# tkkiran/Robust-Conditional-GAN

Hardware: AMD Instinct MI355X
Metric: images/sec G+D train step (CIFAR-10 RCGAN bs=64) (higher is better)
Workload: dtype bf16

## Files before the change

### include/rcgan_hip.h

```cpp
#ifndef RCGAN_HIP_H
#define RCGAN_HIP_H

#include <stddef.h>
#include <stdint.h>

#ifdef __cplusplus
extern "C" {
#endif

#define RCGAN_OK 0
#define RCGAN_EINVALID_ARG (-1)
#define RCGAN_EUNSUPPORTED_SHAPE (-2)
#define RCGAN_EWORKSPACE_TOO_SMALL (-3)
#define RCGAN_EHIP (-4)
#define RCGAN_ERCCL (-5)

#define RCGAN_F32 0
#define RCGAN_BF16 1
#define RCGAN_F16 2

#define RCGAN_ACT_NONE 0
#define RCGAN_ACT_RELU 1
#define RCGAN_ACT_LRELU 2
#define RCGAN_ACT_TANH 3
// ... 24 lines not shown
int rcgan_prof_begin(rcgan_ctx* ctx, int which);
int rcgan_prof_end(rcgan_ctx* ctx, int* launches, double* total_ms, double* total_flops);
int rcgan_prof_executed_flops(rcgan_ctx* ctx, double* executed_flops);
int rcgan_prof_bn_in_launches(rcgan_ctx* ctx, int* launches);
int rcgan_debug_stamps(rcgan_ctx* ctx, void* stamps);
int rcgan_graph_begin(rcgan_ctx* ctx);
int rcgan_graph_end(rcgan_ctx* ctx, int* graph_id);
int rcgan_reserve_scratch(rcgan_ctx* ctx, size_t bytes);
int rcgan_scratch_bytes(rcgan_ctx* ctx, size_t* split_reduction_bytes, size_t* narrow_bytes);
int rcgan_graph_abort(rcgan_ctx* ctx);
int rcgan_graph_launch(rcgan_ctx* ctx, int graph_id);
int rcgan_graph_destroy(rcgan_ctx* ctx, int graph_id);

#define RCGAN_CONV_IN_UPSAMPLE2X 1
#define RCGAN_CONV_IN_RELU 2
#define RCGAN_CONV_ACCUMULATE 4
#define RCGAN_CONV_FORCE_DIRECT 8
#define RCGAN_CONV_OUT_MEANPOOL2 16

#define RCGAN_CONV_RESID_UPSAMPLE2X 32

typedef struct rcgan_conv_desc {
  int n, h, w, cin;
  int cout, kh, kw, stride;
  int dtype;
  int flags;
} rcgan_conv_desc;

size_t rcgan_conv_prepared_bytes(const rcgan_conv_desc* d);
int rcgan_conv_prepare(rcgan_ctx* ctx, const rcgan_conv_desc* d, const float* w_hwio,
                       const float* sigma , void* prepared);

typedef struct rcgan_prepare_item {
  rcgan_conv_desc desc;
  const float* w;
  const float* sigma;
  void* prepared;
} rcgan_prepare_item;
int rcgan_conv_prepare_batch(rcgan_ctx* ctx, const rcgan_prepare_item* items, int n_items);
typedef struct rcgan_embed_desc {
  int v, e_dim, d;
  const float *table, *w_e, *sigma_e , *b_e ;
  float* E;
} rcgan_embed_desc;
int rcgan_conv_prepare_batch_embed(rcgan_ctx* ctx, const rcgan_prepare_item* items, int n_items, const rcgan_embed_desc* e);
typedef struct rcgan_step_inputs_desc {
  int n, dtype;
  const int32_t* images;
  void* x; void* pooled;
  float noise_lo, noise_hi;
  uint64_t seed; void* rng_state;
  float* fill; size_t fill_count;
  const void* fakes; void* fake_slice; int n_slices;
} rcgan_step_inputs_desc;
int rcgan_conv_prepare_batch_riders(rcgan_ctx* ctx, const rcgan_prepare_item* items, int n_items, const rcgan_embed_desc* e,
                                    const rcgan_step_inputs_desc* si);
typedef struct rcgan_frag_item { int item; int ctn, ss; void* fwd; void* bwd; } rcgan_frag_item;
int rcgan_conv_prepare_batch_frags(rcgan_ctx* ctx, const rcgan_prepare_item* items, int n_items, const rcgan_embed_desc* e,
                                   const rcgan_step_inputs_desc* si, const rcgan_frag_item* frags, int n_frags);

size_t rcgan_conv_workspace_bytes(const rcgan_conv_desc* d);
int rcgan_conv_fused_pool_ok(const rcgan_conv_desc* d);
int rcgan_conv_resid_up_ok(const rcgan_conv_desc* d);
int rcgan_conv2d_fwd(rcgan_ctx* ctx, const rcgan_conv_desc* d, const void* x, const void* prepared,
                     const float* bias , void* y);
int rcgan_conv_bn_in_ok(const rcgan_conv_desc* d);
int rcgan_conv2d_fwd_bn(rcgan_ctx* ctx, const rcgan_conv_desc* d, const void* x, const void* prepared, const float* bias, void* y,
                        int segments, const int32_t* labels, const float* gamma, const float* beta, const float* mean, const float* rstd,
                        int act);
int rcgan_conv2d_fwd_bn_residual(rcgan_ctx* ctx, const rcgan_conv_desc* d, const void* x, const void* prepared, const float* bias,
                                 const void* residual, void* y, int segments, const int32_t* labels, const float* gamma, const float* beta,
                                 const float* mean, const float* rstd, int act);
int rcgan_conv2d_fwd_residual(rcgan_ctx* ctx, const rcgan_conv_desc* d, const void* x, const void* prepared,
                              const float* bias , const void* residual , void* y);
int rcgan_conv2d_bwd_data(rcgan_ctx* ctx, const rcgan_conv_desc* d, const void* dy, const void* prepared,
                          const void* x , void* dx, void* ws, size_t ws_bytes);
int rcgan_conv2d_bwd_data_residual(rcgan_ctx* ctx, const rcgan_conv_desc* d, const void* dy, const void* prepared,
                                   const void* x , const void* residual, void* dx, void* ws, size_t ws_bytes);
int rcgan_conv_wgrad_pool_ok(const rcgan_conv_desc* d);
int rcgan_conv2d_bwd_weight(rcgan_ctx* ctx, const rcgan_conv_desc* d, const void* x, const void* dy,
                            float* dw, float* dbias, int accumulate, void* ws, size_t ws_bytes);
int rcgan_conv2d_bwd_weight_group(rcgan_ctx* ctx, int n, const rcgan_conv_desc* descs, const void* const* xs, const void* const* dys,
                                  float* const* dws, float* const* dbiases, int accumulate, void* ws, size_t ws_bytes);

int rcgan_deconv2d_fwd(rcgan_ctx* ctx, const rcgan_conv_desc* d, const void* x, const float* w,
                       const float* bias, void* y);
int rcgan_deconv2d_bwd_data(rcgan_ctx* ctx, const rcgan_conv_desc* d, const void* dy, const float* w, void* dx);
int rcgan_deconv2d_bwd_data_cols(rcgan_ctx* ctx, const rcgan_conv_desc* d, const void* dy, const float* w, void* dx, int n_cols);
int rcgan_deconv2d_bwd_weight(rcgan_ctx* ctx, const rcgan_conv_desc* d, const void* x, const void* dy,
                              float* dw, float* dbias, int accumulate, void* ws, size_t ws_bytes);
size_t rcgan_deconv2d_bwd_weight_concat_bytes(const rcgan_conv_desc* d, int n_cols);
int rcgan_deconv2d_bwd_weight_concat(rcgan_ctx* ctx, const rcgan_conv_desc* d, const void* x, const void* dy, int n_cols, const float* yb,
                                     float* dw, float* dbias, int accumulate, void* ws, size_t ws_bytes);

int rcgan_linear_fwd(rcgan_ctx* ctx, int m, int k, int n, int dtype, const void* x, const float* w,
                     const float* sigma, const float* bias, void* y);
int rcgan_linear_bwd_data(rcgan_ctx* ctx, int m, int k, int n, int dtype, const void* dy, const float* w,
                          const float* sigma, void* dx, int accumulate);
int rcgan_linear_bwd_weight(rcgan_ctx* ctx, int m, int k, int n, int dtype, const void* x, const void* dy,
                            float* dw, float* dbias, int accumulate, void* ws, size_t ws_bytes);
size_t rcgan_linear_workspace_bytes(int m, int k, int n);

size_t rcgan_bn_workspace_bytes(int rows, int c);
size_t rcgan_bn_workspace_bytes_labels(int rows, int c, int n_labels);
int rcgan_bn_stats(rcgan_ctx* ctx, int rows, int c, int dtype, const void* x, float eps,
                   float* mean, float* rstd, float* moving_mean, float* moving_var, float decay,
                   void* ws, size_t ws_bytes);
int rcgan_bn_apply_fwd(rcgan_ctx* ctx, int n, int rows_per_sample, int c, int n_labels, int dtype, const void* x,
                       const int32_t* labels, const float* gamma, const float* beta,
                       const float* mean, const float* rstd, int act, void* y, void* ws, size_t ws_bytes);
int rcgan_bn_fwd_segments(rcgan_ctx* ctx, int nseg, int n_per_seg, int rows_per_sample, int c, int n_labels, int dtype,
                          const void* x, const int32_t* labels, const float* gamma, const float* beta, float eps, int act,
                          float* mean, float* rstd, void* y, void* ws, size_t ws_bytes);
int rcgan_bn_bwd(rcgan_ctx* ctx, int n, int rows_per_sample, int c, int n_labels, int dtype,
                 const void* x, const void* y, const void* dy, const int32_t* labels,
                 const float* gamma, const float* mean, const float* rstd, int act,
                 void* dx, int accumulate_dx, float* dgamma, float* dbeta, int accumulate, void* ws, size_t ws_bytes);
int rcgan_bn_bwd2(rcgan_ctx* ctx, int n, int rows_per_sample, int c, int n_labels, int dtype, const void* x, const void* y,
                  const void* dy, const int32_t* labels, const float* gamma, const float* beta, const float* mean, const float* rstd,
                  int act, void* dx, int accumulate_dx, float* dgamma, float* dbeta, int accumulate, void* ws, size_t ws_bytes);
int rcgan_bn_infer(rcgan_ctx* ctx, int rows, int c, int dtype, const void* x, const float* gamma,
                   const float* beta, const float* moving_mean, const float* moving_var, float eps,
                   int act, void* y);
int rcgan_bn_infer_bwd(rcgan_ctx* ctx, int rows, int c, int dtype, const void* y, const void* dy, const float* gamma,
                       const float* moving_var, float eps, int act, void* dx, int accumulate);

typedef struct rcgan_sn_item {
  const float* w;
  float* u;
  float* sigma;
  float* save;
  int k, c, update;
} rcgan_sn_item;
size_t rcgan_sn_save_floats(int k, int c);
int rcgan_sn_power_iter(rcgan_ctx* ctx, const rcgan_sn_item* items, int n_items);
typedef struct rcgan_sn_bwd_item {
  const float* w; const float* dwbar; float* dw; float* save ; int k, c, accumulate;
} rcgan_sn_bwd_item;
int rcgan_sn_bwd(rcgan_ctx* ctx, const rcgan_sn_bwd_item* items, int n_items);
typedef struct rcgan_sn_adam {
  float* w; float* g; float* m; float* v; size_t count;
  float* hyper;
  float beta1, beta2, eps, clip, grad_scale;
  int n_ranges; const size_t* ranges;
} rcgan_sn_adam;
int rcgan_sn_bwd_adam(rcgan_ctx* ctx, const rcgan_sn_bwd_item* items, int n_items, const rcgan_sn_adam* opt);

int rcgan_act_fwd(rcgan_ctx* ctx, size_t count, int dtype, int act, const void* x, void* y);
int rcgan_act_bwd(rcgan_ctx* ctx, size_t count, int dtype, int act, const void* x_or_y, const void* dy,
                  void* dx, int accumulate);
int rcgan_add(rcgan_ctx* ctx, size_t count, int dtype, const void* a, const void* b, void* y);
int rcgan_axpby(rcgan_ctx* ctx, size_t count, int dtype, float alpha, const void* a, float beta, void* y);
int rcgan_cast(rcgan_ctx* ctx, size_t count, int src_dtype, const void* src, int dst_dtype, void* dst);
int rcgan_meanpool2_fwd(rcgan_ctx* ctx, int n, int h, int w, int c, int dtype, const void* x, void* y);
int rcgan_meanpool2_bwd(rcgan_ctx* ctx, int n, int h, int w, int c, int dtype, const void* dy, void* dx, int accumulate);
int rcgan_upsample2_fwd(rcgan_ctx* ctx, int n, int h, int w, int c, int dtype, const void* x, void* y);
int rcgan_upsample2_bwd(rcgan_ctx* ctx, int n, int h, int w, int c, int dtype, const void* dy, void* dx, int accumulate);
int rcgan_pad_channels(rcgan_ctx* ctx, size_t rows, int c, int before, int after, int dtype, const void* x, void* y);
int rcgan_concat_channels_fwd(rcgan_ctx* ctx, int n, int hw, int c1, int c2, int dtype, const void* x,
                              const float* yb, void* y);
int rcgan_concat_channels_bwd(rcgan_ctx* ctx, int n, int hw, int c1, int c2, int dtype, const void* dy, void* dx);
int rcgan_tile_rows_fwd(rcgan_ctx* ctx, size_t count, int reps, int dtype, const void* x, void* y);
int rcgan_tile_rows_bwd(rcgan_ctx* ctx, size_t count, int reps, int dtype, const void* dy, void* dx, int accumulate);
int rcgan_transpose_f32(rcgan_ctx* ctx, int rows, int cols, const float* x, float* y, int accumulate);
int rcgan_preprocess_cifar(rcgan_ctx* ctx, int n, const int32_t* images_chw, const float* noise_chw,
                           int dtype, void* y_nhwc);
// ... 34 lines not shown
int rcgan_conv_rf_prepare(rcgan_ctx* ctx, int n, const rcgan_conv_desc* descs, const void* const* prepared, void* const* frags);
int rcgan_fragments_prepare(rcgan_ctx* ctx, const void* const* trunk_prepared, void* trunk_frag, int n, const rcgan_conv_desc* descs,
                            const void* const* prepared, void* const* frags);
int rcgan_conv2d_rf(rcgan_ctx* ctx, const rcgan_conv_desc* d, int backward, const void* x, const void* frag, const float* bias,
                    const void* mask_x, const void* residual, void* y);
typedef struct {
  int n, d, v, e_dim;
  int rows_a, kind_a, kind_b;
  float weight;
  const int32_t* labels_a; const float* wts_a; float* dwts_a;
  const int32_t* labels_b; const float* wts_b; float* dwts_b;
  const void* x; void* dx;
  int x_dtype, hw, act;
  const float* E_pre;
  void* defer_ws;
  size_t defer_ws_bytes;
} rcgan_head_desc;
int rcgan_proj_head_fwd_bwd(rcgan_ctx* ctx, const rcgan_head_desc* hd, const float* feat, const float* w_out, const float* sigma_out,
                            const float* b_out, const float* table, const float* w_e, const float* sigma_e, const float* b_e,
                            float* loss_acc, float* logits, float* dfeat, float* dw_out, float* db_out, float* dtable, float* dw_e,
                            float* db_e, void* ws, size_t ws_bytes);
int rcgan_head_flush(rcgan_ctx* ctx);
int rcgan_bce_onehot_fwd_bwd(rcgan_ctx* ctx, int rows, int cols, const float* x, const int32_t* labels,
                             float weight, float* loss_acc, float* dx);
int rcgan_recover_mse_fwd_bwd(rcgan_ctx* ctx, int r, int ydim, int pix, int dtype, const void* gen, const void* actual,
                              const float* yrec, float* loss, void* dgen, float* dyrec, void* ws, size_t ws_bytes);
int rcgan_softmax_rows_fwd(rcgan_ctx* ctx, int rows, int cols, const float* logits, float* p);
int rcgan_softmax_rows_bwd(rcgan_ctx* ctx, int rows, int cols, const float* p, const float* dp, float* dlogits,
                           int accumulate);

size_t rcgan_softmax_xent_workspace_bytes(int rows);
int rcgan_softmax_xent_fwd_bwd(rcgan_ctx* ctx, int rows, int cols, const float* logits, const int32_t* labels, float weight,
                               float* loss_acc, float* n_correct_acc, float* dlogits, void* ws, size_t ws_bytes);
int rcgan_shortcut_a_fwd(rcgan_ctx* ctx, int n, int h, int w, int c, int dtype, const void* x, void* y);
int rcgan_shortcut_a_bwd(rcgan_ctx* ctx, int n, int h, int w, int c, int dtype, const void* dy, void* dx, int accumulate);
int rcgan_sgd_momentum(rcgan_ctx* ctx, size_t count, size_t decay_count, float* w, const float* g, float* accum, const float* hyper,
                       float momentum, float weight_decay, int nesterov, float grad_scale);
int rcgan_augment_cifar(rcgan_ctx* ctx, int n, int n_images, const uint8_t* images_chw_u8, const int32_t* labels_all,
                        const int32_t* index, const int32_t* shift_flip, int pad, int dtype, void* y_nhwc, int32_t* labels_out);

int rcgan_adam_tf(rcgan_ctx* ctx, size_t count, float* w, const float* g, float* m, float* v,
                  const float* hyper, float beta1, float beta2, float eps, float clip, float grad_scale);
int rcgan_adam_tf_host(rcgan_ctx* ctx, size_t count, float* w, const float* g, float* m, float* v,
                       float lr, float t, float beta1, float beta2, float eps, float clip, float grad_scale);
int rcgan_fill_f32(rcgan_ctx* ctx, size_t count, float* p, float value);
int rcgan_copy_words(rcgan_ctx* ctx, size_t count, const void* src, void* dst);

int rcgan_conv_stats_ok(const rcgan_conv_desc* d);
size_t rcgan_conv_stats_bytes(const rcgan_conv_desc* d);
int rcgan_conv2d_fwd_stats(rcgan_ctx* ctx, const rcgan_conv_desc* d, const void* x, const void* prepared, const float* bias,
                           const void* residual, void* y, float* tile_sums);
int rcgan_bn_stats_from_tiles(rcgan_ctx* ctx, const rcgan_conv_desc* d, int nseg, float eps, const float* tile_sums, float* mean, float* rstd);
int rcgan_bn_apply_segments(rcgan_ctx* ctx, int nseg, int n_per_seg, int rows_per_sample, int c, int n_labels, int dtype, const void* x,
                            const int32_t* labels, const float* gamma, const float* beta, const float* mean, const float* rstd, int act,
                            void* y, void* ws, size_t ws_bytes);

int rcgan_set_grad_scale(rcgan_ctx* ctx, float host_scale, const float* dev_scale);

#define RCGAN_F32_PRECISION_HIGHEST 0
#define RCGAN_F32_PRECISION_HIGH 1
int rcgan_set_f32_matmul_precision(rcgan_ctx* ctx, int precision);
int rcgan_grad_finite_check(rcgan_ctx* ctx, size_t count, const float* g, float* ls_state);
int rcgan_adam_tf_dyn(rcgan_ctx* ctx, size_t count, float* w, const float* g, float* m, float* v, float lr, const float* t_dev,
                      float beta1, float beta2, float eps, float clip, float grad_scale, const float* ls_state);
int rcgan_loss_scale_update(rcgan_ctx* ctx, float* ls_state, float* t_dev0, float* t_dev1, float growth_interval, float min_scale,
                            float max_scale);

#define RCGAN_COMM_ID_BYTES 128
int rcgan_comm_unique_id(void* id_out);
int rcgan_comm_init(rcgan_ctx* ctx, const void* id, int world, int rank);
int rcgan_comm_init_stub(rcgan_ctx* ctx, int world);
int rcgan_comm_destroy(rcgan_ctx* ctx);
int rcgan_comm_world(rcgan_ctx* ctx);
int rcgan_allreduce_sum(rcgan_ctx* ctx, float* buf, size_t count);
int rcgan_allreduce_sum_buckets(rcgan_ctx* ctx, int n, float* const* bufs, const size_t* counts);
int rcgan_allreduce_sum_async(rcgan_ctx* ctx, float* buf, size_t count);
int rcgan_allreduce_join(rcgan_ctx* ctx);
int rcgan_comm_count(rcgan_ctx* ctx, int* ranks);
size_t rcgan_allreduce_bf16_scratch_bytes(int n, const size_t* counts);
int rcgan_allreduce_sum_bf16_buckets(rcgan_ctx* ctx, int n, float* const* bufs, const size_t* counts, void* scratch16, size_t scratch_bytes);
int rcgan_comm_stub_model(rcgan_ctx* ctx, double bus_gbps, double latency_us);
const char* rcgan_comm_load_error(void);
int rcgan_set2_f32(rcgan_ctx* ctx, float* p, float a, float b);

int rcgan_selftest(rcgan_ctx* ctx);
#define RCGAN_QUERY_TR_READ 0
int rcgan_query(rcgan_ctx* ctx, int what);

#ifdef __cplusplus
}
#endif
#endif
```

### robust-conditional-gan_amd/_lib.py

```python
import ctypes as C
import os

_HERE = os.path.dirname(os.path.abspath(__file__))
LIB_PATH = os.environ.get("RCGAN_LIB_PATH") or os.path.join(_HERE, "librcgan_hip.so")
LIB_PATH_F16 = os.environ.get("RCGAN_LIB_PATH_F16") or os.path.join(_HERE, "librcgan_hip_f16.so")

F32, BF16, F16 = 0, 1, 2
ACT_NONE, ACT_RELU, ACT_LRELU, ACT_TANH, ACT_SIGMOID = 0, 1, 2, 3, 4
CONV_IN_UPSAMPLE2X, CONV_IN_RELU, CONV_ACCUMULATE, CONV_FORCE_DIRECT, CONV_OUT_MEANPOOL2, CONV_RESID_UPSAMPLE2X = 1, 2, 4, 8, 16, 32
LOSS_HINGE_REAL, LOSS_HINGE_FAKE, LOSS_NEG_MEAN, LOSS_CE_ONES, LOSS_CE_ZEROS = 0, 1, 2, 3, 4
QUERY_TR_READ = 0
F32_PRECISION_HIGHEST, F32_PRECISION_HIGH = 0, 1
F32_PRECISIONS = {"highest": F32_PRECISION_HIGHEST, "high": F32_PRECISION_HIGH}

RCGAN_EHIP, RCGAN_ERCCL = -4, -5
EINVALID_ARG, EUNSUPPORTED_SHAPE = -1, -2
ERRORS = {-1: "RCGAN_EINVALID_ARG", -2: "RCGAN_EUNSUPPORTED_SHAPE", -3: "RCGAN_EWORKSPACE_TOO_SMALL",
          -4: "RCGAN_EHIP", -5: "RCGAN_ERCCL"}


def source_hash():
    import glob
    import hashlib
    h = hashlib.sha256()
    files = sorted(glob.glob(os.path.join(_HERE, "csrc", "*.hip")) + glob.glob(os.path.join(_HERE, "csrc", "*.h")) +
                   glob.glob(os.path.join(os.path.dirname(_HERE), "include", "*.h")))
    for f in files:
        h.update(os.path.basename(f).encode())
        with open(f, "rb") as fh:
            h.update(fh.read())
    return h.hexdigest()[:16]


class RcganError(RuntimeError):
    def __init__(self, code, msg):
        super().__init__("%s (%d): %s" % (ERRORS.get(code, "RCGAN_E?"), code, msg))
        self.code = code


class ConvDesc(C.Structure):
    _fields_ = [("n", C.c_int), ("h", C.c_int), ("w", C.c_int), ("cin", C.c_int),
                ("cout", C.c_int), ("kh", C.c_int), ("kw", C.c_int), ("stride", C.c_int),
                ("dtype", C.c_int), ("flags", C.c_int)]


class PrepareItem(C.Structure):
    _fields_ = [("desc", ConvDesc), ("w", C.c_void_p), ("sigma", C.c_void_p), ("prepared", C.c_void_p)]


class FragItem(C.Structure):
    _fields_ = [("item", C.c_int), ("ctn", C.c_int), ("ss", C.c_int), ("fwd", C.c_void_p), ("bwd", C.c_void_p)]


class HeadDesc(C.Structure):
    _fields_ = [("n", C.c_int), ("d", C.c_int), ("v", C.c_int), ("e_dim", C.c_int),
                ("rows_a", C.c_int), ("kind_a", C.c_int), ("kind_b", C.c_int), ("weight", C.c_float),
                ("labels_a", C.c_void_p), ("wts_a", C.c_void_p), ("dwts_a", C.c_void_p),
                ("labels_b", C.c_void_p), ("wts_b", C.c_void_p), ("dwts_b", C.c_void_p),
                ("x", C.c_void_p), ("dx", C.c_void_p), ("x_dtype", C.c_int), ("hw", C.c_int), ("act", C.c_int),
                ("E_pre", C.c_void_p), ("defer_ws", C.c_void_p), ("defer_ws_bytes", C.c_size_t)]


class EmbedDesc(C.Structure):
    _fields_ = [("v", C.c_int), ("e_dim", C.c_int), ("d", C.c_int),
                ("table", C.c_void_p), ("w_e", C.c_void_p), ("sigma_e", C.c_void_p), ("b_e", C.c_void_p), ("E", C.c_void_p)]


class StepInputsDesc(C.Structure):
    _fields_ = [("n", C.c_int), ("dtype", C.c_int), ("images", C.c_void_p), ("x", C.c_void_p), ("pooled", C.c_void_p),
                ("noise_lo", C.c_float), ("noise_hi", C.c_float), ("seed", C.c_uint64), ("rng_state", C.c_void_p),
                ("fill", C.c_void_p), ("fill_count", C.c_size_t),
                ("fakes", C.c_void_p), ("fake_slice", C.c_void_p), ("n_slices", C.c_int)]


class SnItem(C.Structure):
    _fields_ = [("w", C.c_void_p), ("u", C.c_void_p), ("sigma", C.c_void_p), ("save", C.c_void_p),
                ("k", C.c_int), ("c", C.c_int), ("update", C.c_int)]


class SnBwdItem(C.Structure):
    _fields_ = [("w", C.c_void_p), ("dwbar", C.c_void_p), ("dw", C.c_void_p), ("save", C.c_void_p),
                ("k", C.c_int), ("c", C.c_int), ("accumulate", C.c_int)]


LABELS_NARROW = 16
MAX_CLASSES = 1024
SN_MAX_RANGES = 48


class SnAdam(C.Structure):
    _fields_ = [("w", C.c_void_p), ("g", C.c_void_p), ("m", C.c_void_p), ("v", C.c_void_p), ("count", C.c_size_t),
                ("hyper", C.c_void_p), ("beta1", C.c_float), ("beta2", C.c_float), ("eps", C.c_float), ("clip", C.c_float),
                ("grad_scale", C.c_float), ("n_ranges", C.c_int), ("ranges", C.POINTER(C.c_size_t))]


P, I, F, SZ = C.c_void_p, C.c_int, C.c_float, C.c_size_t
DP = C.POINTER(ConvDesc)

SIGNATURES = {
    "rcgan_create": (I, [C.POINTER(P), I, P]),
    "rcgan_destroy": (I, [P]),
    "rcgan_last_error": (C.c_char_p, [P]),
    "rcgan_version": (C.c_char_p, []),
    "rcgan_half_dtype": (I, []),
    "rcgan_crc32c": (C.c_uint, [C.c_uint, P, SZ]),
    "rcgan_set_stream": (I, [P, P]),
    "rcgan_side_begin": (I, [P]),
    "rcgan_side_end": (I, [P]),
    "rcgan_side_join": (I, [P]),
    "rcgan_stream_sync": (I, [P]),
    "rcgan_event_record": (I, [P, I]),
    "rcgan_event_elapsed_ms": (I, [P, I, I, C.POINTER(F)]),
    "rcgan_debug_stamps": (I, [P, P]),
    "rcgan_prof_begin": (I, [P, I]),
    "rcgan_prof_end": (I, [P, C.POINTER(I), C.POINTER(C.c_double), C.POINTER(C.c_double)]),
    "rcgan_prof_executed_flops": (I, [P, C.POINTER(C.c_double)]),
    "rcgan_prof_bn_in_launches": (I, [P, C.POINTER(I)]),
    "rcgan_graph_begin": (I, [P]),
    "rcgan_reserve_scratch": (I, [P, C.c_size_t]),
    "rcgan_scratch_bytes": (I, [P, C.POINTER(C.c_size_t), C.POINTER(C.c_size_t)]),
    "rcgan_graph_end": (I, [P, C.POINTER(I)]),
    "rcgan_graph_abort": (I, [P]),
    "rcgan_graph_launch": (I, [P, I]),
    "rcgan_graph_destroy": (I, [P, I]),
    "rcgan_conv_prepared_bytes": (SZ, [DP]),
    "rcgan_conv_prepare": (I, [P, DP, P, P, P]),
    "rcgan_conv_prepare_batch": (I, [P, C.POINTER(PrepareItem), I]),
    "rcgan_conv_prepare_batch_embed": (I, [P, C.POINTER(PrepareItem), I, C.POINTER(EmbedDesc)]),
    "rcgan_conv_prepare_batch_riders": (I, [P, C.POINTER(PrepareItem), I, C.POINTER(EmbedDesc), C.POINTER(StepInputsDesc)]),
    "rcgan_conv_prepare_batch_frags": (I, [P, C.POINTER(PrepareItem), I, C.POINTER(EmbedDesc), C.POINTER(StepInputsDesc), C.POINTER(FragItem), I]),
    "rcgan_conv_workspace_bytes": (SZ, [DP]),
    "rcgan_conv2d_fwd": (I, [P, DP, P, P, P, P]),
    "rcgan_conv_bn_in_ok": (I, [DP]),
    "rcgan_conv2d_fwd_bn": (I, [P, DP, P, P, P, P, I, P, P, P, P, P, I]),
    "rcgan_conv2d_fwd_bn_residual": (I, [P, DP, P, P, P, P, P, I, P, P, P, P, P, I]),
    "rcgan_conv_fused_pool_ok": (I, [DP]),
    "rcgan_conv_resid_up_ok": (I, [DP]),
    "rcgan_conv_wgrad_pool_ok": (I, [DP]),
    "rcgan_conv2d_fwd_residual": (I, [P, DP, P, P, P, P, P]),
    "rcgan_conv2d_bwd_data": (I, [P, DP, P, P, P, P, P, SZ]),
    "rcgan_conv2d_bwd_data_residual": (I, [P, DP, P, P, P, P, P, P, SZ]),
    "rcgan_conv2d_bwd_weight": (I, [P, DP, P, P, P, P, I, P, SZ]),
    "rcgan_conv2d_bwd_weight_group": (I, [P, I, P, P, P, P, P, I, P, SZ]),
    "rcgan_deconv2d_fwd": (I, [P, DP, P, P, P, P]),
    "rcgan_deconv2d_bwd_data": (I, [P, DP, P, P, P]),
    "rcgan_deconv2d_bwd_data_cols": (I, [P, DP, P, P, P, I]),
    "rcgan_deconv2d_bwd_weight": (I, [P, DP, P, P, P, P, I, P, SZ]),
    "rcgan_deconv2d_bwd_weight_concat_bytes": (SZ, [DP, I]),
    "rcgan_deconv2d_bwd_weight_concat": (I, [P, DP, P, P, I, P, P, P, I, P, SZ]),
    "rcgan_linear_fwd": (I, [P, I, I, I, I, P, P, P, P, P]),
    "rcgan_linear_bwd_data": (I, [P, I, I, I, I, P, P, P, P, I]),
    "rcgan_linear_bwd_weight": (I, [P, I, I, I, I, P, P, P, P, I, P, SZ]),
    "rcgan_linear_workspace_bytes": (SZ, [I, I, I]),
    "rcgan_bn_workspace_bytes": (SZ, [I, I]),
    "rcgan_bn_workspace_bytes_labels": (SZ, [I, I, I]),
    "rcgan_bn_stats": (I, [P, I, I, I, P, F, P, P, P, P, F, P, SZ]),
    "rcgan_bn_apply_fwd": (I, [P, I, I, I, I, I, P, P, P, P, P, P, I, P, P, SZ]),
    "rcgan_bn_fwd_segments": (I, [P, I, I, I, I, I, I, P, P, P, P, F, I, P, P, P, P, SZ]),
    "rcgan_bn_bwd": (I, [P, I, I, I, I, I, P, P, P, P, P, P, P, I, P, I, P, P, I, P, SZ]),
    "rcgan_bn_bwd2": (I, [P, I, I, I, I, I, P, P, P, P, P, P, P, P, I, P, I, P, P, I, P, SZ]),
    "rcgan_bn_infer": (I, [P, I, I, I, P, P, P, P, P, F, I, P]),
    "rcgan_bn_infer_bwd": (I, [P, I, I, I, P, P, P, P, F, I, P, I]),
    "rcgan_sn_save_floats": (SZ, [I, I]),
    "rcgan_sn_power_iter": (I, [P, C.POINTER(SnItem), I]),
    "rcgan_sn_bwd": (I, [P, C.POINTER(SnBwdItem), I]),
    "rcgan_sn_bwd_adam": (I, [P, C.POINTER(SnBwdItem), I, C.POINTER(SnAdam)]),
    "rcgan_act_fwd": (I, [P, SZ, I, I, P, P]),
    "rcgan_act_bwd": (I, [P, SZ, I, I, P, P, P, I]),
    "rcgan_add": (I, [P, SZ, I, P, P, P]),
    "rcgan_axpby": (I, [P, SZ, I, F, P, F, P]),
    "rcgan_cast": (I, [P, SZ, I, P, I, P]),
    "rcgan_meanpool2_fwd": (I, [P, I, I, I, I, I, P, P]),
    "rcgan_meanpool2_bwd": (I, [P, I, I, I, I, I, P, P, I]),
    "rcgan_upsample2_fwd": (I, [P, I, I, I, I, I, P, P]),
    "rcgan_upsample2_bwd": (I, [P, I, I, I, I, I, P, P, I]),
    "rcgan_pad_channels": (I, [P, SZ, I, I, I, I, P, P]),
    "rcgan_concat_channels_fwd": (I, [P, I, I, I, I, I, P, P, P]),
    "rcgan_concat_channels_bwd": (I, [P, I, I, I, I, I, P, P]),
    "rcgan_tile_rows_fwd": (I, [P, SZ, I, I, P, P]),
    "rcgan_tile_rows_bwd": (I, [P, SZ, I, I, P, P, I]),
    "rcgan_transpose_f32": (I, [P, I, I, P, P, I]),
    "rcgan_preprocess_cifar": (I, [P, I, P, P, I, P]),
    "rcgan_rng_fill": (I, [P, SZ, I, I, F, F, C.c_uint64, P, P]),
    "rcgan_act_meanhw_fwd": (I, [P, I, I, I, I, I, P, P]),
    "rcgan_act_meanhw_bwd": (I, [P, I, I, I, I, I, P, P, P]),
    "rcgan_gather_rows": (I, [P, I, I, P, P, P]),
    "rcgan_scatter_add_rows": (I, [P, I, I, I, P, P, P, I]),
    "rcgan_proj_logit_fwd": (I, [P, I, I, P, P, P, P]),
    "rcgan_proj_logit_bwd": (I, [P, I, I, P, P, P, P, P, P, I]),
    "rcgan_proj_logit_all_fwd": (I, [P, I, I, I, P, P, P, P]),
    "rcgan_proj_logit_all_bwd": (I, [P, I, I, I, P, P, P, P, P, P, I]),
    "rcgan_loss_fwd_bwd": (I, [P, I, I, I, P, P, F, P, P, P]),
    "rcgan_bce_onehot_fwd_bwd": (I, [P, I, I, P, P, F, P, P]),
    "rcgan_dtrunk": (I, [P, I, I, P, P, P, P, P]),
    "rcgan_dtrunk_pooled": (I, [P, I, I, P, P, P, P, P, P, P, P]),
    "rcgan_dtrunk_prepare": (I, [P, P, P]),
    "rcgan_conv_rf_ok": (I, [C.POINTER(ConvDesc)]),
    "rcgan_conv_rf_fragment_bytes": (SZ, [C.POINTER(ConvDesc)]),
    "rcgan_conv_rf_prepare": (I, [P, I, C.POINTER(ConvDesc), P, P]),
    "rcgan_fragments_prepare": (I, [P, P, P, I, C.POINTER(ConvDesc), P, P]),
    "rcgan_conv2d_rf": (I, [P, C.POINTER(ConvDesc), I, P, P, P, P, P, P]),
    "rcgan_dtrunk_fragment_bytes": (SZ, []),
    "rcgan_head_flush": (I, [P]),
    "rcgan_proj_head_fwd_bwd": (I, [P, C.POINTER(HeadDesc)] + [P] * 16 + [P, SZ]),
    "rcgan_recover_mse_fwd_bwd": (I, [P, I, I, I, I, P, P, P, P, P, P, P, SZ]),
    "rcgan_softmax_rows_fwd": (I, [P, I, I, P, P]),
    "rcgan_softmax_rows_bwd": (I, [P, I, I, P, P, P, I]),
    "rcgan_softmax_xent_workspace_bytes": (SZ, [I]),
    "rcgan_softmax_xent_fwd_bwd": (I, [P, I, I, P, P, F, P, P, P, P, SZ]),
    "rcgan_shortcut_a_fwd": (I, [P, I, I, I, I, I, P, P]),
    "rcgan_shortcut_a_bwd": (I, [P, I, I, I, I, I, P, P, I]),
    "rcgan_sgd_momentum": (I, [P, SZ, SZ, P, P, P, P, F, F, I, F]),
    "rcgan_augment_cifar": (I, [P, I, I, P, P, P, P, I, I, P, P]),
    "rcgan_adam_tf": (I, [P, SZ, P, P, P, P, P, F, F, F, F, F]),
    "rcgan_adam_tf_host": (I, [P, SZ, P, P, P, P, F, F, F, F, F, F, F]),
    "rcgan_fill_f32": (I, [P, SZ, P, F]),
    "rcgan_copy_words": (I, [P, SZ, P, P]),
    "rcgan_conv_stats_ok": (I, [DP]),
    "rcgan_conv_stats_bytes": (SZ, [DP]),
    "rcgan_conv2d_fwd_stats": (I, [P, DP, P, P, P, P, P, P]),
    "rcgan_bn_stats_from_tiles": (I, [P, DP, I, F, P, P, P]),
    "rcgan_bn_apply_segments": (I, [P, I, I, I, I, I, I, P, P, P, P, P, P, I, P, P, SZ]),
    "rcgan_comm_unique_id": (I, [P]),
    "rcgan_comm_init": (I, [P, P, I, I]),
    "rcgan_comm_init_stub": (I, [P, I]),
    "rcgan_comm_destroy": (I, [P]),
    "rcgan_comm_world": (I, [P]),
    "rcgan_allreduce_sum": (I, [P, P, SZ]),
    "rcgan_allreduce_sum_buckets": (I, [P, I, P, P]),
    "rcgan_allreduce_sum_async": (I, [P, P, SZ]),
    "rcgan_allreduce_join": (I, [P]),
    "rcgan_comm_count": (I, [P, P]),
    "rcgan_allreduce_bf16_scratch_bytes": (SZ, [I, P]),
    "rcgan_allreduce_sum_bf16_buckets": (I, [P, I, P, P, P, SZ]),
    "rcgan_comm_stub_model": (I, [P, C.c_double, C.c_double]),
    "rcgan_comm_load_error": (C.c_char_p, []),
    "rcgan_set2_f32": (I, [P, P, F, F]),
    "rcgan_set_grad_scale": (I, [P, F, P]),
    "rcgan_set_f32_matmul_precision": (I, [P, I]),
    "rcgan_grad_finite_check": (I, [P, SZ, P, P]),
    "rcgan_adam_tf_dyn": (I, [P, SZ, P, P, P, P, F, P, F, F, F, F, F, P]),
    "rcgan_loss_scale_update": (I, [P, P, P, P, F, F, F]),
    "rcgan_selftest": (I, [P]),
    "rcgan_query": (I, [P, I]),
}

_libs = {}


def load(half="bf16"):
    if half in _libs:
        return _libs[half]
    path = LIB_PATH_F16 if half == "f16" else LIB_PATH
    if not os.path.exists(path):
        raise RuntimeError(
            "%s is missing (%s): build it with robust-conditional-gan_amd/csrc/build.sh "
            "or __graft_entry__.build(); there is no CPU fallback" % (os.path.basename(path), path))
    import torch
    lib = C.CDLL(path)
    for name, (res, args) in SIGNATURES.items():
        fn = getattr(lib, name)
        fn.restype = res
        fn.argtypes = args
    want = F16 if half == "f16" else BF16
    if lib.rcgan_half_dtype() != want:
        raise RuntimeError("%s was built for 16-bit dtype %d, expected %d" % (path, lib.rcgan_half_dtype(), want))
    _libs[half] = lib
    return lib
```

### robust-conditional-gan_amd/cifar.py

```python
import ctypes as C
import os

import warnings

import numpy as np
import torch

from . import _lib as L
from . import ops as O
from .ops_cifar import NO_OPS, Conv2D, Linear, cond_batchnorm, embed_y, spectral_normed_weight
from .runtime import DT, Context, ParamGroup, check_f32_matmul_precision
from .variables import Graph, scoped, variable_scope

Z_DIM = 128
DIM_G = 128
DIM_D = 128
VOCAB_SIZE = 10
EMBEDDING_DIM = 300
IMG_SIZE = 32
IMG_DIM = 3
OUTPUT_DIM = 3072
N_CRITIC = 5
GEN_BS_MULTIPLE = 2
ALGORITHMS = ("rcgan", "rcgan-u", "biased", "unbiased")
# ... 286 lines not shown
    O.proj_head(g.ctx, features, w_out, b_out, table, w_e, b_e, parts, weight, loss_acc, logits=logits, E_pre=getattr(g, "head_E", None))


def perm_classifier(x, perm_type='linear'):
    ctx = _ctx()
    with variable_scope("Discriminator"):
        x = O.cast(ctx, O.reshape(ctx, x, (-1, OUTPUT_DIM)), L.F32)
        if perm_type == 'linear':
            return Linear(x, OUTPUT_DIM, _n_classes(), 'D.d_perm_classifier_h1', spectral_normed=True, biases=True)
        elif perm_type == '2layer':
            h = Linear(x, OUTPUT_DIM, 128, 'D.d_perm_classifier_h1', spectral_normed=True, biases=True)
            return Linear(h, 128, _n_classes(), 'D.d_perm_classifier_h2', spectral_normed=True, biases=True)
        raise ValueError('Unknown perm_type {}'.format(perm_type))


class CifarRCGAN:

    def __init__(self, algorithm="rcgan", alpha=0.6, batch_size=64, lr=2e-4, dtype="bf16", seed=0,
                 perm_classifier=False, perm_multiplier=1.0, perm_type="linear",
                 confuse_init=False, confuse_init_diag=0.2, confuse_multiplier=1.0, confuse_lr_decay=False,
                 device=0, use_graphs=True, device_rng=True, arena_bytes=None, world_size=1, rank=0,
                 variables=None, loss_scale=None, dynamic_loss_scale=None, loss_scale_growth_interval=2000, comm=None,
                 grad_bucket_dtype=None, stub_model=None, f32_matmul_precision="highest", n_classes=VOCAB_SIZE):
        if algorithm not in ALGORITHMS:
            raise ValueError("Unknown algorithm %s" % algorithm)
        self.K = check_n_classes(n_classes)
        self.f32_matmul_precision = check_f32_matmul_precision(f32_matmul_precision, dtype)
        self.alg, self.alpha, self.B, self.lr = algorithm, alpha, int(batch_size), lr
        self.perm, self.perm_mult, self.perm_type = perm_classifier, perm_multiplier, perm_type
        self.confuse_multiplier, self.confuse_lr_decay = confuse_multiplier, confuse_lr_decay
        self.world, self.rank = world_size, rank
        self.use_graphs, self.device_rng = use_graphs, device_rng
        self.fused_head = os.environ.get("RCGAN_FUSED_HEAD", "1") == "1" and 2 * int(batch_size) <= O.HEAD_MAX_N
        self.ride_inputs = os.environ.get("RCGAN_RIDE_INPUTS", "1") == "1"
        if arena_bytes is None:
            arena_bytes = int(2.5e6 * 4 * self.B * (4 if dtype == "f32" else 2)) + (1 << 30)
        self.ctx = Context(device, dtype, arena_bytes=arena_bytes)
        ctx = self.ctx
        ctx.set_f32_matmul_precision(self.f32_matmul_precision)
        self.loss_scale = float(loss_scale) if loss_scale is not None else (1024.0 if ctx.act_dtype == L.F16 else 1.0)
        self.dynamic_ls = (ctx.act_dtype == L.F16) if dynamic_loss_scale is None else bool(dynamic_loss_scale)
        self.ls_growth_interval = float(loss_scale_growth_interval)
        if self.dynamic_ls:
            self.ls_state = torch.tensor([self.loss_scale, 0.0, 0.0, 0.0], dtype=torch.float32, device=ctx.device)
            ctx.check(ctx.lib.rcgan_set_grad_scale(ctx.h, 1.0, C.c_void_p(self.ls_state.data_ptr())))
        else:
            self.ls_state = None
            ctx.check(ctx.lib.rcgan_set_grad_scale(ctx.h, self.loss_scale, None))
        if variables is None:
            variables = create_variables(seed, algorithm, perm_classifier, perm_type, confuse_init, confuse_init_diag, self.K)
        gs, ds, cs, U = variables
        self.PG, self.PD = ParamGroup(ctx, gs), ParamGroup(ctx, ds, sn_scratch=True)
        self.PC = ParamGroup(ctx, cs) if cs else None
        self.groups = [self.PG, self.PD] + ([self.PC] if self.PC else [])
        self.state = {}
        for k, v in U.items():
            t = ctx.persistent((v.size,), L.F32)
            ctx.view(t).copy_(torch.from_numpy(np.ascontiguousarray(v.reshape(-1))))
            self.state[k] = t
        self.graph = Graph(ctx, self.groups, self.state)
        self.graph.n_classes = self.K
        self.comm_kind = None
        self.dp_active = self.world > 1 or comm == "rccl-self"
        if self.dp_active:
            from . import dp
            self.comm_kind = comm or "rccl"
            if self.comm_kind not in ("rccl", "stub", "rccl-self") or (self.comm_kind == "rccl-self" and self.world != 1):
                raise ValueError("Unknown comm %s for world_size %d" % (comm, self.world))
            dp.init_comm(ctx, self.world, self.rank, stub=(self.comm_kind == "stub"))
            if stub_model is not None:
                ctx.check(ctx.lib.rcgan_comm_stub_model(ctx.h, float(stub_model[0]), float(stub_model[1])))
        self.grad_bucket_dtype = grad_bucket_dtype or os.environ.get("RCGAN_DP_BUCKET_DTYPE", "f32")
        if self.grad_bucket_dtype not in ("f32", "bf16"):
            raise ValueError("Unknown gradient bucket dtype %s" % self.grad_bucket_dtype)
        self._bucket16 = None
        self.dp_overlap = self.dp_active and self.grad_bucket_dtype == "f32" and os.environ.get("RCGAN_DP_OVERLAP", "0") == "1"
        self._early_lo = {id(self.PD): self.PD.offsets["Discriminator/D.Block.3.Conv1/Filters"],
                          id(self.PG): self.PG.offsets["Generator/G.Block.2.Shortcut/Filters"]}
        self.dp_adam_in_graph = self.dp_active and not self.dynamic_ls and os.environ.get("RCGAN_DP_GRAPH_ADAM", "1") == "1"
        self.graph_adam = self.dp_adam_in_graph or (not self.dp_active and not self.dynamic_ls and
                                                    os.environ.get("RCGAN_GRAPH_ADAM", "0") == "1")
        self.fused_tail = (not self.dp_active and not self.dynamic_ls and not self.graph_adam
                           and os.environ.get("RCGAN_SN_ADAM", "1") == "1")
        self._tail_fused = {}
        B = self.B
        f32, i32, act = L.F32, "i32", ctx.act_dtype
        P = ctx.persistent
        self.feed_layout = {
            "d": [("images", (B, OUTPUT_DIM), i32), ("labels", (B,), i32), ("labels_random", (B,), i32), ("labels_biased", (B,), i32),
                  ("inv_weights", (B, self.K), f32), ("labels_all", (2 * B,), i32)],
            "g": [("labels_random_G", (2 * B,), i32), ("labels_biased_G", (2 * B,), i32)],
            "gf": [("labels_random_all", (N_CRITIC * B,), i32)]}
        self.feed, self.inp = {}, {}
        self._feed_ring = {}
        for key, fields in self.feed_layout.items():
            words = sum(int(np.prod(shp)) for _, shp, _ in fields)
            slab = torch.zeros(words, dtype=torch.int32, device=ctx.device)
            self.feed[key] = slab
            off = 0
            for name, shp, dt in fields:
                self.inp[name] = DT(slab.data_ptr() + 4 * off, shp, dt, slab, name)
                off += int(np.prod(shp))
        words_d = self.feed["d"].numel()
        self.feed["d5"] = torch.zeros(N_CRITIC * words_d, dtype=torch.int32, device=ctx.device)
        self._d_slot_views = []
        for k in range(N_CRITIC):
            off, views = k * words_d, {}
            for name, shp, dt in self.feed_layout["d"]:
                views[name] = DT(self.feed["d5"].data_ptr() + 4 * off, shp, dt, self.feed["d5"], name)
                off += int(np.prod(shp))
            self._d_slot_views.append(views)
        self.critic_graph = os.environ.get("RCGAN_CRITIC_GRAPH", "1") == "1"
        self.inp.update(noise=P((B, OUTPUT_DIM), f32), z=P((B, Z_DIM), act), z_G=P((2 * B, Z_DIM), act),
                        z_all=P((N_CRITIC * B, Z_DIM), act),
                        arange=P((self.K,), i32), C_const=P((self.K, self.K), f32))
        ctx.view(self.inp["arange"]).copy_(torch.arange(self.K, dtype=torch.int32))
        ctx.view(self.inp["C_const"]).copy_(torch.from_numpy(C_ALPHA(alpha, self.K).astype(np.float32)))
        self.fakes_all = P((N_CRITIC * B, OUTPUT_DIM), act)
        self.x_all = P((2 * B, OUTPUT_DIM), act)
        self._fakes_left = 0
        self.loss_d = self.PD.scalar(0)
        self.loss_g = self.PG.scalar(0)
        self.rng_state = torch.zeros(2, dtype=torch.int64, device=ctx.device)
        self.overlap_gf = os.environ.get("RCGAN_OVERLAP_GF", "0") == "1"
        self.ctx2 = None
        if self.overlap_gf:
            self.ctx2 = Context(device, dtype, arena_bytes=int(2.5e6 * self.B * (4 if dtype == "f32" else 2)) + (256 << 20), ws_bytes=256 << 20)
            ctx.also_close = [self.ctx2]
            ctx.check(self.ctx2.lib.rcgan_set_grad_scale(self.ctx2.h, 1.0, None))
            self.ctx2.set_f32_matmul_precision(self.f32_matmul_precision)
            self.graph2 = Graph(self.ctx2, [ParamGroup.alias(self.ctx2, self.PG)], {})
            self.graph2.persist = self.graph.persist
            self.rng_state_gf = torch.zeros(2, dtype=torch.int64, device=ctx.device)
            self._gf_done = [torch.cuda.Event() for _ in range(N_CRITIC)]
            self._gf_pending = [False] * N_CRITIC
            torch.cuda.set_device(ctx.device)
        self.slice_ctr = torch.zeros(4, dtype=torch.int32, device=ctx.device)
        self._slice_mirror = 0
        self.seed = seed
        self._graphs = {}
        self.head_logits = None
        self.iteration = 0
        self._pg_prepared_version = -1
        torch.cuda.synchronize()

    def set_inputs(self, **arrays):
        ctx = self.ctx
        with torch.cuda.stream(ctx.stream):
            for k, a in arrays.items():
                dst = ctx.view(self.inp[k])
                src = torch.from_numpy(np.ascontiguousarray(np.asarray(a)))
                dst.copy_(src.reshape(dst.shape).to(dst.dtype).pin_memory(), non_blocking=True)

    def pack_feed(self, key, **arrays):
        parts = []
        for name, shp, dt in self.feed_layout[key]:
            a = np.ascontiguousarray(np.asarray(arrays[name]).reshape(shp))
            parts.append(a.astype(np.float32).view(np.int32).reshape(-1) if dt == L.F32 else a.astype(np.int32).reshape(-1))
        return np.concatenate(parts)

    def feed_host(self, key, **arrays):
        steps = arrays.pop("_steps", None)
        ring = self._feed_ring.setdefault(key, {"slots": [], "events": [], "next": 0})
        words = self.feed[key].numel()
        if not ring["slots"]:
            ring["slots"] = [torch.empty(words, dtype=torch.int32).pin_memory() for _ in range(8)]
# ... 145 lines not shown
        else:
            fake = Generator(B, inp["labels_random"], inp["z"], out=fake_dst)
        w = 1.0
        if self.fused_head:
            feat = Discriminator(x_all, None, update_collection=None, _head=False)
            lab_r, lab_f = inp["labels_all"].rows(0, B), inp["labels_all"].rows(B, 2 * B)
            if self.alg == "rcgan-u":
                y_conf = O.gather_rows(ctx, self.confusion_matrix(), inp["labels_random"], B)
                parts = [(B, L.LOSS_HINGE_REAL, inp["labels"], None), (B, L.LOSS_HINGE_FAKE, None, y_conf)]
            elif self.alg == "unbiased":
                parts = [(B, L.LOSS_HINGE_REAL, None, inp["inv_weights"]), (B, L.LOSS_HINGE_FAKE, inp["labels_random"], None)]
            else:
                parts = [(B, L.LOSS_HINGE_REAL, lab_r, None), (B, L.LOSS_HINGE_FAKE, lab_f, None)]
            Discriminator_head(feat, parts, w, self.loss_d, update_collection=None, logits=self.head_logits)
        elif self.alg == "rcgan-u":
            feat_a, wgan_a = Discriminator(x_all, None, update_collection=None)
            feat, wgan = O.rows(ctx, feat_a, 0, B), O.rows(ctx, wgan_a, 0, B)
            feat_f, wgan_f = O.rows(ctx, feat_a, B, 2 * B), O.rows(ctx, wgan_a, B, 2 * B)
            emb = Discriminator_projection(inp["labels"], update_collection=None)
            disc_real = O.proj_logit(ctx, feat, wgan, emb)
            E = Discriminator_projection(inp["arange"], update_collection=None)
            disc_fake = O.proj_logit_all(ctx, feat_f, wgan_f, E)
            y_conf = O.gather_rows(ctx, self.confusion_matrix(), inp["labels_random"], B)
            O.loss_term(ctx, L.LOSS_HINGE_FAKE, disc_fake, w, self.loss_d, wts=y_conf)
            O.loss_term(ctx, L.LOSS_HINGE_REAL, disc_real, w, self.loss_d)
        else:
            feat, wgan = Discriminator(x_all, None, update_collection=None)
            if self.alg in ("biased", "rcgan"):
                emb = Discriminator_projection(inp["labels_all"], update_collection=None)
                disc_all = O.proj_logit(ctx, feat, wgan, emb)
                O.loss_term(ctx, L.LOSS_HINGE_REAL, O.rows(ctx, disc_all, 0, B), w, self.loss_d)
                O.loss_term(ctx, L.LOSS_HINGE_FAKE, O.rows(ctx, disc_all, B, 2 * B), w, self.loss_d)
            else:
                E = Discriminator_projection(inp["arange"], update_collection=None)
                feat_r, wgan_r = O.rows(ctx, feat, 0, B), O.rows(ctx, wgan, 0, B)
                feat_f, wgan_f = O.rows(ctx, feat, B, 2 * B), O.rows(ctx, wgan, B, 2 * B)
                disc_real_all = O.proj_logit_all(ctx, feat_r, wgan_r, E)
                O.loss_term(ctx, L.LOSS_HINGE_REAL, disc_real_all, w, self.loss_d, wts=inp["inv_weights"])
                emb_f = Discriminator_projection(inp["labels_random"], update_collection=None)
                disc_fake = O.proj_logit(ctx, feat_f, wgan_f, emb_f)
                O.loss_term(ctx, L.LOSS_HINGE_FAKE, disc_fake, w, self.loss_d)
        if self.perm:
            logits = perm_classifier(real, self.perm_type)
            O.bce_onehot_term(ctx, logits, inp["labels"], 1.0, self.loss_d)
        ctx.backward()
        fused = bool(ctx.sn_adam and ctx.sn_adam.get("done"))
        ctx.sn_adam = None
        self._dp_finish([self.PD])
        return fused

    def _d_step_body(self, fakes_ready):
        self._tail_fused[fakes_ready] = self._d_body(fakes_ready)

    def _g_body(self):
        ctx, g, B, inp = self.ctx, self.graph, self.B, self.inp
        n = GEN_BS_MULTIPLE * B
        self._refresh_generator_filters()
        ctx.new_step()
        g.begin_step({0, 2} if self.PC is not None else {0})
        ctx.sn_adam = None
        g.early_g = self._dp_early(self.PG) if (self.dp_overlap and ctx.recording) else None
        self.PG.zero_grad()
        if self.PC is not None:
            self.PC.zero_grad()
        if self.device_rng:
            self._rng(inp["z_G"], 1, 0.0, 1.0)
        g.prefetch_sn(self._sn_entries(False, True))
        self._prepare_all((self.PG, self.PD), head_update=NO_OPS)
        fake = Generator(n, inp["labels_random_G"], inp["z_G"])
        lab = inp["labels_random_G"] if self.alg in ("biased", "unbiased") else inp["labels_biased_G"]
        if self.fused_head:
            feat = Discriminator(fake, lab, update_collection=NO_OPS, _head=False)
            if self.alg == "rcgan-u":
                y_conf = O.gather_rows(ctx, self.confusion_matrix(), inp["labels_random_G"], n)
                parts = [(n, L.LOSS_NEG_MEAN, None, y_conf)]
            else:
                parts = [(n, L.LOSS_NEG_MEAN, lab, None)]
            Discriminator_head(feat, parts, 1.0, self.loss_g, update_collection=NO_OPS, logits=self.head_logits)
        else:
            self._g_head_unfused(fake, lab, n)
        if self.perm:
            logits = perm_classifier(fake, self.perm_type)
            O.bce_onehot_term(ctx, logits, inp["labels_random_G"], self.perm_mult, self.loss_g)
        ctx.backward()
        self._dp_finish([self.PG] + ([self.PC] if self.PC is not None else []))

    def _g_head_unfused(self, fake, lab, n):
        ctx, inp = self.ctx, self.inp
        feat, wgan = Discriminator(fake, lab, update_collection=NO_OPS)
        if self.alg == "rcgan-u":
            E = Discriminator_projection(inp["arange"], update_collection=None)
            disc_fake = O.proj_logit_all(ctx, feat, wgan, E)
            y_conf = O.gather_rows(ctx, self.confusion_matrix(), inp["labels_random_G"], n)
            O.loss_term(ctx, L.LOSS_NEG_MEAN, disc_fake, 1.0, self.loss_g, wts=y_conf)
        else:
            emb = Discriminator_projection(lab, update_collection=None)
            disc_fake = O.proj_logit(ctx, feat, wgan, emb)
            O.loss_term(ctx, L.LOSS_NEG_MEAN, disc_fake, 1.0, self.loss_g)

    def _run(self, key, body, ctx=None):
        ctx = ctx or self.ctx
        if not self.use_graphs:
            body()
            return
        if key not in self._graphs:
            body()
            ctx.sync()
            ctx.graph_begin()
            try:
                body()
                gid = ctx.graph_end()
            except L.RcganError as e:
                ctx.graph_abort()
                if not (self.dp_active and e.code == L.RCGAN_ERCCL):
                    raise
                warnings.warn("step %r: the all-reduce could not be captured (%s); running it uncaptured" % (key, e))
                gid = None
            except BaseException:
                ctx.graph_abort()
                raise
            self._graphs[key] = gid
            return
        if self._graphs[key] is None:
            body()
            return
        ctx.graph_launch(self._graphs[key])

    def _dp_early(self, grp):
        ctx, lo = self.ctx, self._early_lo[id(grp)]
        state = {"sent": False}
        grp._dp_early_state = state

        def fire():
            ctx.flush_wgrads()
            for bw in ctx.sn_partial:
                bw(lambda name: name in grp.offsets and grp.offsets[name] >= lo)
            ctx.check(ctx.lib.rcgan_allreduce_sum_async(ctx.h, C.c_void_p(grp.grad.data_ptr() + 4 * lo), grp.count - lo))
            state["sent"] = True
        return fire

    def _dp_finish(self, groups):
        ctx = self.ctx
        if not ctx.recording:
            return
        if not self.dp_active:
            if self.graph_adam:
                for grp in groups:
                    grp.adam_captured(0.0, 0.9, grad_scale=1.0 / (self.world * self.loss_scale))
            return
        ptrs, counts = [], []
        for grp in groups:
            st = getattr(grp, "_dp_early_state", None)
            hi = self._early_lo[id(grp)] if (st is not None and st["sent"]) else grp.count
            grp._dp_early_state = None
            if hi > 0:
                ptrs.append(grp.grad.data_ptr())
                counts.append(hi)
        n = len(ptrs)
        if self.grad_bucket_dtype == "bf16":
            cnt = (C.c_size_t * n)(*counts)
            need = ctx.lib.rcgan_allreduce_bf16_scratch_bytes(n, cnt)
            if self._bucket16 is None:
                allc = [g.count for g in self.groups]
                self._bucket16 = torch.empty(ctx.lib.rcgan_allreduce_bf16_scratch_bytes(len(allc), (C.c_size_t * len(allc))(*allc)),
                                             dtype=torch.uint8, device=ctx.device)
            assert need <= self._bucket16.numel()
            ctx.check(ctx.lib.rcgan_allreduce_sum_bf16_buckets(ctx.h, n, (C.c_void_p * n)(*ptrs), cnt, C.c_void_p(self._bucket16.data_ptr()),
                                                               self._bucket16.numel()))
        else:
            ctx.check(ctx.lib.rcgan_allreduce_sum_buckets(ctx.h, n, (C.c_void_p * n)(*ptrs), (C.c_size_t * n)(*counts)))
        if self.dp_overlap:
            ctx.check(ctx.lib.rcgan_allreduce_join(ctx.h))
        if self.dp_adam_in_graph:
            for grp in groups:
                grp.adam_captured(0.0, 0.9, grad_scale=1.0 / (self.world * self.loss_scale))

    def _optimise_or_publish(self, steps):
        if self.graph_adam:
            for grp, _ in steps:
                grp.version += 1
            return
        self._optimise(steps)

    def _pre_step(self, steps):
        if self.fused_tail:
            for grp, lr in steps:
                if grp is self.PD and (grp.hyper is None or getattr(grp, "_dev_hyper", None) != (float(lr), grp.t)):
                    grp.set_hyper_device(lr, grp.t)
                    grp._dev_hyper = (float(lr), grp.t)
        if self.graph_adam:
            for grp, lr in steps:
                grp.t += 1
                grp.set_hyper_device(lr, grp.t)

    def _gf_body(self):
        ctx, g, B, inp = self.ctx, self.graph, self.B, self.inp
        self._refresh_generator_filters()
        ctx.new_step()
        g.begin_step(set())
        rec, ctx.recording = ctx.recording, False
        try:
            if self.device_rng:
                self._rng(inp["z_all"], 1, 0.0, 1.0)
            self._prepare_all((self.PG,))
            Generator(N_CRITIC * B, inp["labels_random_all"], inp["z_all"], out=self.fakes_all, segments=N_CRITIC)
        finally:
            ctx.recording = rec

    def _gf_chunk_body(self, k):
        ctx2, g2, B, inp = self.ctx2, self.graph2, self.B, self.inp
        ctx2.new_step()
        g2.begin_step(set())
        rec, ctx2.recording = ctx2.recording, False
        try:
            z = inp["z_all"].rows(k * B, (k + 1) * B)
            if self.device_rng:
                ctx2.check(ctx2.lib.rcgan_rng_fill(ctx2.h, z.size, z.dtype, 1, 0.0, 1.0, self.seed * 1000003 + self.rank + 500009,
                                                   C.c_void_p(self.rng_state_gf.data_ptr()), C.c_void_p(z.ptr)))
            Generator(B, inp["labels_random_all"].rows(k * B, (k + 1) * B), z, out=self.fakes_all.rows(k * B, (k + 1) * B))
        finally:
            ctx2.recording = rec

    def _join_gf(self):
        if self.overlap_gf:
            for k in range(N_CRITIC):
                if self._gf_pending[k]:
                    self.ctx.stream.wait_event(self._gf_done[k])
                    self._gf_pending[k] = False

    def _prepare_critic_fakes_overlapped(self):
        s1, s2 = self.ctx.stream, self.ctx2.stream
        self._refresh_generator_filters()
        ev = torch.cuda.Event()
        ev.record(s1)
        s2.wait_event(ev)
        for k in range(N_CRITIC):
            self._run("gf%d" % k, lambda k=k: self._gf_chunk_body(k), ctx=self.ctx2)
            self._gf_done[k].record(s2)
            self._gf_pending[k] = True

    def prepare_critic_fakes(self):
        if self.overlap_gf:
            self._prepare_critic_fakes_overlapped()
        else:
            self._run("gf", self._gf_body)
        self._fakes_left = N_CRITIC
        if self._slice_mirror != 0:
            with torch.cuda.stream(self.ctx.stream):
                self.slice_ctr.zero_()
            self._slice_mirror = 0

    def d_step(self, iteration=None):
        it = self.iteration if iteration is None else iteration
        self._refresh_generator_filters()
        steps = [(self.PD, self.lr * lr_decay(it))]
        self._pre_step(steps)
        if self._fakes_left > 0:
            k = N_CRITIC - self._fakes_left
            self._fakes_left -= 1
            ctx = self.ctx
            if self.overlap_gf and self._gf_pending[k]:
                ctx.stream.wait_event(self._gf_done[k])
                self._gf_pending[k] = False
            if self._rides_inputs():
                assert self._slice_mirror == k, (self._slice_mirror, k)
                self._slice_mirror = (k + 1) % N_CRITIC
            else:
                with torch.cuda.stream(ctx.stream):
                    ctx.view(self.x_all.rows(self.B, 2 * self.B)).copy_(ctx.view(self.fakes_all.rows(k * self.B, (k + 1) * self.B)), non_blocking=True)
            key, fakes_ready = "d_fakes", True
        else:
            key, fakes_ready = "d", False
        self._run(key, lambda: self._d_step_body(fakes_ready))
        if self._tail_fused.get(fakes_ready, False):
            lr = steps[0][1]
            self.PD.t += 1
            self.PD._dev_hyper = (float(lr), self.PD.t)
            self.PD.version += 1
            return
        self._optimise_or_publish(steps)

    def _critic_graph_ok(self):
        return (self.critic_graph and self.fused_tail and self._fakes_left == N_CRITIC and self._rides_inputs() and self._slice_mirror == 0)

    def critic_steps(self, batches, iteration=None):
        it = self.iteration if iteration is None else iteration
        packed = isinstance(batches, torch.Tensor)
        assert (batches.shape[0] if packed else len(batches)) == N_CRITIC
        if not self._critic_graph_ok():
            for k in range(N_CRITIC):
                if packed:
                    self.set_feed("d", batches[k])
                else:
                    self.feed_host("d", **batches[k])
                self.d_step(iteration=it)
            return
        ctx = self.ctx
        if packed:
            src = batches.reshape(-1)
            assert src.is_cuda and src.dtype == torch.int32 and src.is_contiguous() and src.numel() == self.feed["d5"].numel()
            ctx.check(ctx.lib.rcgan_copy_words(ctx.h, src.numel(), C.c_void_p(src.data_ptr()), C.c_void_p(self.feed["d5"].data_ptr())))
        else:
            self.feed_host("d5", _steps=batches)
        self._refresh_generator_filters()
        lr = self.lr * lr_decay(it)
        self._pre_step([(self.PD, lr)])
        self._join_gf()

        def body():
            fused = True
            for k in range(N_CRITIC):
                saved = {n: self.inp[n] for n in self._d_slot_views[k]}
                self.inp.update(self._d_slot_views[k])
                try:
                    fused = self._d_body(True) and fused
                finally:
                    self.inp.update(saved)
            self._tail_fused["d5"] = fused
        self._run("d5", body)
        assert self._tail_fused.get("d5", False), "critic_steps: a step's last launch did not apply the update"
        self._fakes_left = 0
        self.PD.t += N_CRITIC
        self.PD._dev_hyper = (float(lr), self.PD.t)
        self.PD.version += 1

    def g_step(self, iteration=None):
        it = self.iteration if iteration is None else iteration
        self._fakes_left = 0
        self._join_gf()
        self._refresh_generator_filters()
        steps = [(self.PG, self.lr * lr_decay(it))]
        if self.PC is not None:
            steps.append((self.PC, self.lr * self.confuse_multiplier * (lr_decay(it) if self.confuse_lr_decay else 1.0)))
        self._pre_step(steps)
        self._run("g", self._g_body)
        self._optimise_or_publish(steps)
        self._refresh_generator_filters()

    def _optimise(self, steps):
        ctx = self.ctx
        if not self.dynamic_ls:
            for grp, lr in steps:
                grp.t += 1
                grp.set_hyper(lr, grp.t)
                grp.adam(0.0, 0.9, grad_scale=1.0 / (self.world * self.loss_scale))
            return
        for grp, lr in steps:
            grp.t += 1
            grp.finite_check(self.ls_state)
        for grp, lr in steps:
            grp.set_hyper(lr, grp.t)
            grp.adam_dyn(self.ls_state, 0.0, 0.9, grad_scale=1.0 / self.world)
        tds = [C.c_void_p(g.t_dev.data_ptr()) for g, _ in steps] + [None]
        ctx.check(ctx.lib.rcgan_loss_scale_update(ctx.h, C.c_void_p(self.ls_state.data_ptr()), tds[0], tds[1], self.ls_growth_interval,
                                                  1.0, float(1 << 24)))

    def loss_scale_state(self):
        if self.ls_state is None:
            return dict(scale=self.loss_scale, good_steps=None, skipped_steps=0)
        self.ctx.sync()
        s = self.ls_state.cpu().numpy()
        return dict(scale=float(s[0]), good_steps=int(s[1]), skipped_steps=int(s[3]))

    def losses(self):
        ctx = self.ctx
        return float(ctx.download(self.loss_d)[0]), float(ctx.download(self.loss_g)[0])

    def enqueue_losses(self):
        if not hasattr(self, "_loss_ring"):
            self._loss_ring = torch.zeros(1024, 2, dtype=torch.float32).pin_memory()
            self._loss_tickets = 0
        i = self._loss_tickets % 1024
        self._loss_tickets += 1
        ctx = self.ctx
        with torch.cuda.stream(ctx.stream):
            self._loss_ring[i, 0:1].copy_(ctx.view(self.loss_d), non_blocking=True)
            self._loss_ring[i, 1:2].copy_(ctx.view(self.loss_g), non_blocking=True)
        return self._loss_tickets - 1

    def fetch_losses(self, tickets):
        if not tickets:
            return []
        assert self._loss_tickets - min(tickets) <= 1024, "loss ring overrun: fetch at least every 1024 tickets"
        self.ctx.sync()
        return [(float(self._loss_ring[t % 1024, 0]), float(self._loss_ring[t % 1024, 1])) for t in tickets]

    def eval_d_cost(self):
        ctx = self.ctx
        left, self._fakes_left = self._fakes_left, 0
        rec, ctx.recording = ctx.recording, False
        try:
            self._d_body(False)
        finally:
            ctx.recording = rec
            self._fakes_left = left
        return float(ctx.download(self.loss_d)[0])

    def get_params(self):
        out = {}
        for grp in self.groups:
            for n in grp.names:
                out[n] = grp.get(n)
        return out

    def get_grads(self, group):
        scale = self.loss_scale_state()["scale"] * (self.world if self.dp_active else 1)
        return {n: group.get(n, "grad") / np.float32(scale) for n in group.names}

    def get_state(self):
        return {k: self.ctx.download(v).reshape(1, -1) for k, v in self.state.items()}

    def state_dict(self):
        out = {}
        for gname, grp in zip(("Generator", "Discriminator", "confusion"), self.groups):
            for n in grp.names:
                out[n] = grp.get(n)
                out[n + "/Adam"] = grp.get(n, "m")
                out[n + "/Adam_1"] = grp.get(n, "v")
            out["_opt/%s/step" % gname] = np.array([grp.steps_applied()], np.int64)
# ... 72 lines not shown
```

### robust-conditional-gan_amd/csrc/api.hip

```cpp
#include "conv_mfma.h"
#include "small_gemm.h"
#include "step_inputs.h"
#include "conv_image.h"


size_t direct_wgrad_ws_bytes(const rcgan_conv_desc* d);
template <typename T> int direct_fwd(rcgan_ctx*, const rcgan_conv_desc*, const T*, const float*, const float*, const float*, T*, int n_cols = 0);
template <typename T> int direct_dgrad(rcgan_ctx*, const rcgan_conv_desc*, const T*, const float*, const float*, const float*, const T*, T*, int);
template <typename T> int direct_wgrad(rcgan_ctx*, const rcgan_conv_desc*, const T*, const T*, float*, float*, int, void*, size_t);
template <typename T> int direct_wgrad_cols(rcgan_ctx*, const rcgan_conv_desc*, const T*, const T*, int, const float*, float*, int, void*, size_t);
size_t direct_wgrad_cols_ws_bytes(const rcgan_conv_desc* d, int c1);
template <typename T> int colsum_launch(rcgan_ctx*, const T*, long, int, float*, int, float*);
template <typename T> int linear_fwd(rcgan_ctx*, long, long, long, const T*, const float*, const float*, const float*, T*);
template <typename T> int linear_dgrad(rcgan_ctx*, long, long, long, const T*, const float*, const float*, T*, int);
template <typename T> int linear_wgrad(rcgan_ctx*, long, long, long, const T*, const T*, float*, float*, int, void*, size_t);
size_t linear_wgrad_ws_bytes(long m, long k, long n);
template <typename T> int sumpool2_masked_launch(rcgan_ctx*, int, int, int, int, const T*, const T*, T*, int);
int small_fwd_kind(const rcgan_conv_desc* d);
int small_dgrad_kind(const rcgan_conv_desc* d);
int small_wgrad_kind(const rcgan_conv_desc* d);
size_t small_wgrad_ws_bytes(const rcgan_conv_desc* d);
template <typename T> int small_fwd(rcgan_ctx*, const rcgan_conv_desc*, int, const T*, const float*, const float*, T*);
template <typename T> int small_dgrad(rcgan_ctx*, const rcgan_conv_desc*, int, const T*, const float*, T*, int);
template <typename T> int small_wgrad(rcgan_ctx*, const rcgan_conv_desc*, int, const T*, const T*, float*, float*, int, void*, size_t);

__global__ void slab_reduce2_kernel(const float* slab, long stride, float* out, long count, float* bias_out, int nbias, int nz,
                                    int accumulate) {
  long i = (long)blockIdx.x * blockDim.x + threadIdx.x;
  if (i >= count + nbias) return;
  float s = 0.f;
#pragma unroll 4
  for (int z = 0; z < nz; ++z) s += slab[(long)z * stride + i];
  float* o = i < count ? out + i : bias_out + (i - count);
  if (accumulate) s += *o;
  *o = s;
}

#define REDUCE_GROUP_MAX 16
struct SlabReduceGroup {
  struct Item {
    const float* slab; long stride; float* out; long count; float* bias_out; int nbias, nz, accumulate;
    long bias_off;
    int orient, Cb, Cs;
    int sub;
    long cc;
    int bias_parts;
    int vec4;
  } it[REDUCE_GROUP_MAX];
};
__device__ __forceinline__ float4 f4add(float4 a, float4 b) { return make_float4(a.x + b.x, a.y + b.y, a.z + b.z, a.w + b.w); }
__global__ void slab_reduce2_group_kernel(SlabReduceGroup g) {
  const SlabReduceGroup::Item& r = g.it[blockIdx.y];
  long i = (long)blockIdx.x * blockDim.x + threadIdx.x;
  if (r.vec4) {
    const long nv = r.count >> 2;
    if (i < nv) {
      const long e = i << 2;
      float4 s = make_float4(0.f, 0.f, 0.f, 0.f);
      if (r.sub) {
        const int tap = (int)(e / r.cc), kh = tap / 3, kw = tap - kh * 3;
        const long rem = e - (long)tap * r.cc;
        long c4[4];
#pragma unroll
        for (int q = 0; q < 4; ++q) {
          const int pa = q >> 1, pb = q & 1;
          const int sa = ((r.sub == 1) == (pa == 0)) ? (kh >= 1) : (kh >= 2);
          const int sb = ((r.sub == 1) == (pb == 0)) ? (kw >= 1) : (kw >= 2);
          c4[q] = (long)(q * 4 + sa * 2 + sb) * r.cc + rem;
        }
        int z = 0;
        for (; z + 2 <= r.nz; z += 2) {
          float4 v[2][4];
#pragma unroll
          for (int u = 0; u < 2; ++u)
#pragma unroll
            for (int q = 0; q < 4; ++q) v[u][q] = *(const float4*)(r.slab + (long)(z + u) * r.stride + c4[q]);
#pragma unroll
          for (int u = 0; u < 2; ++u) s = f4add(s, f4add(f4add(v[u][0], v[u][1]), f4add(v[u][2], v[u][3])));
        }
        for (; z < r.nz; ++z) {
          const float* sl = r.slab + (long)z * r.stride;
          s = f4add(s, f4add(f4add(*(const float4*)(sl + c4[0]), *(const float4*)(sl + c4[1])), f4add(*(const float4*)(sl + c4[2]), *(const float4*)(sl + c4[3]))));
        }
        if (r.sub == 2) { s.x *= 0.25f; s.y *= 0.25f; s.z *= 0.25f; s.w *= 0.25f; }
      } else {
        int z = 0;
        for (; z + 8 <= r.nz; z += 8) {
          float4 v[8];
#pragma unroll
          for (int u = 0; u < 8; ++u) v[u] = *(const float4*)(r.slab + (long)(z + u) * r.stride + e);
#pragma unroll
          for (int u = 0; u < 8; ++u) s = f4add(s, v[u]);
        }
#pragma unroll 4
        for (; z < r.nz; ++z) s = f4add(s, *(const float4*)(r.slab + (long)z * r.stride + e));
      }
      float4* o = (float4*)(r.out + e);
      if (r.accumulate) s = f4add(s, *o);
      *o = s;
      return;
    }
    i = r.count + (i - nv);
  }
  if (i >= r.count + r.nbias) return;
  const long si = i < r.count ? i : r.bias_off + (i - r.count);
  float s = 0.f;
  if (r.sub && i < r.count) {
    const int tap = (int)(i / r.cc), kh = tap / 3, kw = tap - kh * 3;
    const long rem = i - (long)tap * r.cc;
    long c4[4];
#pragma unroll
    for (int q = 0; q < 4; ++q) {
      const int pa = q >> 1, pb = q & 1;
      const int sa = ((r.sub == 1) == (pa == 0)) ? (kh >= 1) : (kh >= 2);
      const int sb = ((r.sub == 1) == (pb == 0)) ? (kw >= 1) : (kw >= 2);
      c4[q] = (long)(q * 4 + sa * 2 + sb) * r.cc + rem;
    }
    int z = 0;
    for (; z + 4 <= r.nz; z += 4) {
      float v[4][4];
#pragma unroll
      for (int u = 0; u < 4; ++u)
#pragma unroll
        for (int q = 0; q < 4; ++q) v[u][q] = r.slab[(long)(z + u) * r.stride + c4[q]];
#pragma unroll
      for (int u = 0; u < 4; ++u) s += (v[u][0] + v[u][1]) + (v[u][2] + v[u][3]);
    }
    for (; z < r.nz; ++z) {
      const float* sl = r.slab + (long)z * r.stride;
      s += (sl[c4[0]] + sl[c4[1]]) + (sl[c4[2]] + sl[c4[3]]);
    }
    if (r.sub == 2) s *= 0.25f;
  } else {
    int z = 0;
    for (; z + 16 <= r.nz; z += 16) {
      float v[16];
#pragma unroll
      for (int u = 0; u < 16; ++u) v[u] = r.slab[(long)(z + u) * r.stride + si];
#pragma unroll
      for (int u = 0; u < 16; ++u) s += v[u];
    }
#pragma unroll 4
    for (; z < r.nz; ++z) s += r.slab[(long)z * r.stride + si];
    if (i >= r.count && r.bias_parts == 2) {
#pragma unroll 4
      for (z = 0; z < r.nz; ++z) s += r.slab[(long)z * r.stride + si + r.nbias];
    }
  }
  float* o;
  if (i >= r.count) o = r.bias_out + (i - r.count);
  else if (r.orient == 0) o = r.out + i;
  else {
    const int k = (int)(i / r.Cb), n = (int)(i - (long)k * r.Cb);
    const int t = k / r.Cs, c = k - t * r.Cs;
    o = r.out + ((long)t * r.Cb + n) * r.Cs + c;
  }
  if (r.accumulate) s += *o;
  *o = s;
}

struct AdamDyn { const float* ls; const float* tdev; };

__global__ void adam_tf_kernel(size_t count, float* w, const float* g, float* m, float* v, const float* hyper, float lr_v, float t_v,
                               float beta1, float beta2, float eps, float clip, float grad_scale, AdamDyn dyn) {
  if (dyn.ls) {
    if (dyn.ls[2] != 0.f) return;
    grad_scale /= dyn.ls[0];
    t_v = dyn.tdev[0] + 1.f;
  }
  const float lr = hyper ? hyper[0] : lr_v, t = hyper ? hyper[1] : t_v;
  const float alpha = lr * sqrtf(1.f - powf(beta2, t)) / (1.f - powf(beta1, t));
  const float omb1 = 1.f - beta1, omb2 = 1.f - beta2;
  for (size_t i = (size_t)blockIdx.x * blockDim.x + threadIdx.x; i < count; i += (size_t)gridDim.x * blockDim.x) {
    float gi = g[i] * grad_scale;
    float mi = m[i] + (gi - m[i]) * omb1;
    float vi = v[i] + (gi * gi - v[i]) * omb2;
    float wi = w[i] - (mi * alpha) / (sqrtf(vi) + eps);
    if (clip > 0.f) wi = fminf(fmaxf(wi, -clip), clip);
    m[i] = mi; v[i] = vi; w[i] = wi;
  }
}

__global__ void adam_tf_vec4_kernel(size_t count4, float4* w, const float4* g, float4* m, float4* v, const float* hyper, float lr_v, float t_v,
                                    float beta1, float beta2, float eps, float clip, float grad_scale, AdamDyn dyn) {
  if (dyn.ls) {
    if (dyn.ls[2] != 0.f) return;
    grad_scale /= dyn.ls[0];
    t_v = dyn.tdev[0] + 1.f;
  }
  const float lr = hyper ? hyper[0] : lr_v, t = hyper ? hyper[1] : t_v;
  const float alpha = lr * sqrtf(1.f - powf(beta2, t)) / (1.f - powf(beta1, t));
  const float omb1 = 1.f - beta1, omb2 = 1.f - beta2;
  for (size_t i = (size_t)blockIdx.x * blockDim.x + threadIdx.x; i < count4; i += (size_t)gridDim.x * blockDim.x) {
    const float4 g4 = g[i], m4 = m[i], v4 = v[i], w4 = w[i];
    const float gs[4] = {g4.x, g4.y, g4.z, g4.w}, ms[4] = {m4.x, m4.y, m4.z, m4.w}, vs[4] = {v4.x, v4.y, v4.z, v4.w}, ws[4] = {w4.x, w4.y, w4.z, w4.w};
    float mo[4], vo[4], wo[4];
#pragma unroll
    for (int q = 0; q < 4; ++q) {
      const float gi = gs[q] * grad_scale;
      mo[q] = ms[q] + (gi - ms[q]) * omb1;
      vo[q] = vs[q] + (gi * gi - vs[q]) * omb2;
      wo[q] = ws[q] - (mo[q] * alpha) / (sqrtf(vo[q]) + eps);
      if (clip > 0.f) wo[q] = fminf(fmaxf(wo[q], -clip), clip);
    }
    m[i] = make_float4(mo[0], mo[1], mo[2], mo[3]);
    v[i] = make_float4(vo[0], vo[1], vo[2], vo[3]);
    w[i] = make_float4(wo[0], wo[1], wo[2], wo[3]);
  }
}

__global__ void set2_kernel(float* p, float a, float b) { p[0] = a; p[1] = b; }

__global__ void grad_finite_check_kernel(size_t count, const float* g, float* ls) {
  bool bad = false;
  const size_t n4 = count / 4, stride = (size_t)gridDim.x * blockDim.x, tid = (size_t)blockIdx.x * blockDim.x + threadIdx.x;
  for (size_t i = tid; i < n4; i += stride) {
    const float4 q = ((const float4*)g)[i];
    const float z = (q.x - q.x) + (q.y - q.y) + (q.z - q.z) + (q.w - q.w);
    bad |= !(z == 0.f);
  }
  for (size_t i = n4 * 4 + tid; i < count; i += stride) bad |= !((g[i] - g[i]) == 0.f);
  if (bad) ls[2] = 1.f;
}

__global__ void loss_scale_update_kernel(float* ls, float* t0, float* t1, float interval, float min_scale, float max_scale) {
  if (ls[2] != 0.f) {
    ls[0] = fmaxf(ls[0] * 0.5f, min_scale);
    ls[1] = 0.f; ls[2] = 0.f; ls[3] += 1.f;
  } else {
    if (t0) t0[0] += 1.f;
    if (t1) t1[0] += 1.f;
    ls[1] += 1.f;
    if (ls[1] >= interval) { if (ls[0] < max_scale) ls[0] = fminf(ls[0] * 2.f, max_scale); ls[1] = 0.f; }
  }
}

static void adam_launch(rcgan_ctx* ctx, size_t count, float* w, const float* g, float* m, float* v, const float* hyper, float lr, float t,
                        float beta1, float beta2, float eps, float clip, float grad_scale, AdamDyn dyn = {nullptr, nullptr}) {
  const bool vec = count % 4 == 0 && (((size_t)w | (size_t)g | (size_t)m | (size_t)v) & 15) == 0;
  if (vec) {
    size_t blocks = (count / 4 + 255) / 256;
    if (blocks > 8192) blocks = 8192;
    hipLaunchKernelGGL(adam_tf_vec4_kernel, dim3((int)blocks), dim3(256), 0, ctx->stream, count / 4, (float4*)w, (const float4*)g, (float4*)m,
                       (float4*)v, hyper, lr, t, beta1, beta2, eps, clip, grad_scale, dyn);
  } else {
    size_t blocks = (count + 255) / 256;
    if (blocks > 4096) blocks = 4096;
    hipLaunchKernelGGL(adam_tf_kernel, dim3((int)blocks), dim3(256), 0, ctx->stream, count, w, g, m, v, hyper, lr, t, beta1, beta2, eps, clip,
                       grad_scale, dyn);
  }
}

static int g_use_tr = -1;

static int ensure_selftest(rcgan_ctx* ctx) {
  if (g_use_tr >= 0) return RCGAN_OK;
  hipStreamCaptureStatus st = hipStreamCaptureStatusNone;
  (void)hipStreamIsCapturing(ctx->stream, &st);
  if (st != hipStreamCaptureStatusNone) RC_FAIL(ctx, RCGAN_EINVALID_ARG, "first MFMA wgrad call must happen outside graph capture");
  int res[2] = {0, 0};
  int rc = mfma_selftest(ctx, res);
  if (rc) return rc;
  if (res[0] != 0) RC_FAIL(ctx, RCGAN_EHIP, "MFMA 16x16x32 bf16 fragment layout probe failed (%d mismatches)", res[0]);
  g_use_tr = (res[1] == 0) ? 1 : 0;
  const char* e = getenv("RCGAN_NO_TR");
  if (e && e[0] == '1') g_use_tr = 0;
  return RCGAN_OK;
}

extern "C" {

const char* rcgan_version(void) { return RCGAN_HALF_FP16 ? "rcgan_hip 0.1 (gfx950, fp16 build)" : "rcgan_hip 0.1 (gfx950, bf16 build)"; }

int rcgan_create(rcgan_ctx** out, int device, void* stream) {
  if (!out) return RCGAN_EINVALID_ARG;
  int ndev = 0;
  if (hipGetDeviceCount(&ndev) != hipSuccess || ndev <= 0 || device < 0 || device >= ndev) return RCGAN_EHIP;
  if (hipSetDevice(device) != hipSuccess) return RCGAN_EHIP;
  rcgan_ctx* c = new rcgan_ctx();
  c->device = device;
  c->stream = (hipStream_t)stream;
  c->capturing = false;
  c->devtmp = nullptr;
  c->devtmp_bytes = 0;
  c->prof_which = 0;
  c->prof_flops = 0.0; c->prof_flops_exec = 0.0;
  c->main_stream = c->stream; c->side_stream = nullptr; c->fork_ev = nullptr; c->join_ev = nullptr; c->on_side = false;
  if (hipStreamCreateWithFlags(&c->side_stream, hipStreamNonBlocking) != hipSuccess ||
      hipEventCreateWithFlags(&c->fork_ev, hipEventDisableTiming) != hipSuccess ||
      hipEventCreateWithFlags(&c->join_ev, hipEventDisableTiming) != hipSuccess) {
    delete c;
    return RCGAN_EHIP;
  }
  {
// ... 631 lines not shown
  a.M = (long)d->n * a.H * a.W;
  a.lw = ilog2_exact(a.W); a.lh = ilog2_exact(a.H);
  if (a.lw < 0 || a.lh < 0) { a.lw = -1; a.lh = -1; }
  a.slab_stride = (long)a.cells * d->cin * d->cout + d->cout;
  a.want_bias = want_bias ? 1 : 0;
  a.m_chunk = 0;
  *nz = a.sub ? mfma_wgrad_sub_splits(d, a.M) : mfma_wgrad_splits(d, a.M);
  return RCGAN_OK;
}

static SlabReduceGroup::Item wgrad_reduce_item(const rcgan_conv_desc* d, const MfmaWgradArgs& a, float* dw, float* dbias, int nbias, int nz, int accumulate) {
  SlabReduceGroup::Item it = {};
  it.slab = a.slab; it.stride = a.slab_stride; it.out = dw; it.count = (long)d->kh * d->kw * d->cin * d->cout;
  it.bias_out = dbias; it.nbias = nbias; it.nz = nz; it.accumulate = accumulate;
  it.bias_off = (long)a.cells * d->cin * d->cout;
  it.sub = a.sub == 3 ? 0 : a.sub; it.cc = (long)d->cin * d->cout;
  it.bias_parts = a.slab_stride == it.bias_off + 2L * d->cout ? 2 : 1;
  static const int vec4_on = [] { const char* e = getenv("RCGAN_SLAB_REDUCE_VEC4"); return e ? atoi(e) : 1; }();
  it.vec4 = vec4_on && it.count % 4 == 0 && it.cc % 4 == 0 && a.slab_stride % 4 == 0 && ((size_t)a.slab & 15) == 0 && ((size_t)dw & 15) == 0;
  return it;
}

int rcgan_conv_wgrad_pool_ok(const rcgan_conv_desc* d) {
  return d && (d->flags & RCGAN_CONV_OUT_MEANPOOL2) && mfma_wgrad_sub_kind(d, g_use_tr < 0 ? 1 : g_use_tr) == 2 ? 1 : 0;
}

int rcgan_conv2d_bwd_weight(rcgan_ctx* ctx, const rcgan_conv_desc* d, const void* x, const void* dy, float* dw, float* dbias,
                            int accumulate, void* ws, size_t ws_bytes) {
  int rc = check_desc(ctx, d);
  if (rc) return rc;
  if (mfma_wgrad_eligible(d)) {
    rc = ensure_selftest(ctx);
    if (rc) return rc;
    MfmaWgradArgs a;
    int nz = 0;
    rc = wgrad_pose(ctx, d, x, dy, dbias != nullptr, a, &nz);
    if (rc) return rc;
    a.slab = (float*)ws;
    long cnt = (long)d->kh * d->kw * d->cin * d->cout;
    size_t need = (size_t)nz * a.slab_stride * sizeof(float) + (size_t)(cdiv(a.M, 2048) + 1024) * d->cout * sizeof(float);
    if (ws_bytes < need) RC_FAIL(ctx, RCGAN_EWORKSPACE_TOO_SMALL, "need %zu have %zu", need, ws_bytes);
    bool bias_done = false;
    int nzz = mfma_wgrad_launch(ctx, a, nz, &bias_done, ws_bytes);
    if (nzz < 0) return nzz;
    const int nb = bias_done ? d->cout : 0;
    if (a.sub == 1 || a.sub == 2) {
      SlabReduceGroup g;
      for (int q = 0; q < REDUCE_GROUP_MAX; ++q) g.it[q] = wgrad_reduce_item(d, a, dw, dbias, nb, nzz, accumulate);
      hipLaunchKernelGGL(slab_reduce2_group_kernel, dim3(cdiv(cnt + nb, 256), 1), dim3(256), 0, ctx->stream, g);
    } else {
      hipLaunchKernelGGL(slab_reduce2_kernel, dim3(cdiv(cnt + nb, 256)), dim3(256), 0, ctx->stream, (const float*)a.slab, a.slab_stride, dw, cnt,
                         dbias, nb, nzz, accumulate);
    }
    RC_LAUNCH_CHECK(ctx);
    if (dbias && !bias_done) {
      float* part = (float*)((char*)ws + (size_t)nz * a.slab_stride * sizeof(float));
      rc = colsum_launch<bf16_t>(ctx, (const bf16_t*)dy, a.M, d->cout, dbias, accumulate, part);
      if (rc) return rc;
    }
    return RCGAN_OK;
  }
  if (img_side(d)) return img_wgrad(ctx, d, x, dy, dw, dbias, accumulate, ws, ws_bytes);
  if (int kind = small_wgrad_kind(d)) {
    RC_DISPATCH_DTYPE(ctx, d->dtype, return small_wgrad<T>(ctx, d, kind, (const T*)x, (const T*)dy, dw, dbias, accumulate, ws, ws_bytes));
  }
  RC_DISPATCH_DTYPE(ctx, d->dtype, return direct_wgrad<T>(ctx, d, (const T*)x, (const T*)dy, dw, dbias, accumulate, ws, ws_bytes));
  return RCGAN_OK;
}

static int wgrad_busiest_family(const std::vector<MfmaWgradPlanned>* fam, int nfam, size_t counted, bool skip_empty, bool later_wins_ties) {
  int best_f = -1;
  unsigned best = 0;
  for (int f = 0; f < nfam; ++f) {
    if (skip_empty && fam[f].empty()) continue;
    unsigned tot = 0;
    for (size_t q = 0; q < fam[f].size() && q < counted; ++q) tot += fam[f][q].gx * fam[f][q].gy;
    if (best_f < 0 || (later_wins_ties ? tot >= best : tot > best)) { best = tot; best_f = f; }
  }
  return best_f;
}

int rcgan_conv2d_bwd_weight_group(rcgan_ctx* ctx, int n, const rcgan_conv_desc* descs, const void* const* xs, const void* const* dys,
                                  float* const* dws, float* const* dbiases, int accumulate, void* ws, size_t ws_bytes) {
  RC_REQUIRE(ctx, n >= 0 && (n == 0 || (descs && xs && dys && dws && dbiases)), "null argument");
  static const int target_blocks = [] { const char* e = getenv("RCGAN_WGRAD_GROUP_BLOCKS"); return e ? atoi(e) : 448; }();
  struct Cand { MfmaWgradArgs a; int nz; int takes; };
  std::vector<Cand> cand(n);
  const long w9_minwork = [] { const char* e = getenv("RCGAN_WGRAD9_GROUP_MINWORK"); return e ? atol(e) : 1000000L; }();
  bool wgrad9_group_on = false;
  {
    double w9 = 0;
    for (int i = 0; i < n; ++i) {
      const rcgan_conv_desc* d = descs + i;
      if (check_desc(ctx, d) || !mfma_wgrad_eligible(d) || d->kh != 3) continue;
      w9 += (double)d->n * d->h * d->w * (d->cin / 64) * (d->cout / 128);
    }
    wgrad9_group_on = w9 >= (double)w9_minwork;
  }
  double work = 0, work9[2] = {0, 0};
  for (int i = 0; i < n; ++i) {
    const rcgan_conv_desc* d = descs + i;
    int rc = check_desc(ctx, d);
    if (rc) return rc;
    if (!mfma_wgrad_eligible(d)) continue;
    rc = ensure_selftest(ctx);
    if (rc) return rc;
    MfmaWgradArgs& a = cand[i].a;
    rc = wgrad_pose(ctx, d, xs[i], dys[i], dbiases[i] != nullptr, a, &cand[i].nz);
    if (rc) return rc;
    if (mfma_wgrad9_takes(a) && wgrad9_group_on) {
      cand[i].takes = a.sub ? 3 : 2;
      work9[a.sub ? 1 : 0] += (double)a.M * (a.Cin / 64) * (a.Cout / 128) * (a.sub ? 2 : 1);
    } else if (mfma_wgrad3_takes(a)) {
      cand[i].takes = 1;
      work += (double)a.M * (a.sub == 3 ? 1.0 / 3.0 : (a.sub ? 8 * 2.0 / 3.0 : a.KH)) * (a.Cin / 64) * (a.Cout / 128);
    }
  }
  static const int px_max = [] { const char* e = getenv("RCGAN_WGRAD_GROUP_PXMAX"); return e ? atoi(e) : 6144; }();
  long px = (long)(work / target_blocks);
  px = (px + 63) / 64 * 64;
  if (px < 256) px = 256;
  if (px > px_max) px = px_max;
  static const int target9 = [] { const char* e = getenv("RCGAN_WGRAD9_BLOCKS"); return e ? atoi(e) : 256; }();
  long px9[2] = {0, 0};
  for (int f = 0; f < 2; ++f) {
    px9[f] = ((long)(work9[f] / target9) + 127) / 128 * 128;
    if (px9[f] < 512) px9[f] = 512;
    for (int it = 0; it < 4096 && work9[f] > 0; ++it, px9[f] += 128) {
      long tot = 0;
      for (int i = 0; i < n; ++i)
        if (cand[i].takes == 2 + f) {
          MfmaWgradArgs b = cand[i].a;
          unsigned bgx = 0, bgy = 0;
          if (mfma_wgrad9_plan(b, 1 << 20, &bgx, &bgy, px9[f])) tot += (long)bgx * bgy;
        }
      if (tot <= target9) break;
    }
  }
  std::vector<MfmaWgradPlanned> fam9[4];
  std::vector<MfmaWgradPlanned> fam[3];
  std::vector<MfmaWgradPlanned> late;
  std::vector<SlabReduceGroup::Item> red;
  size_t used = 0;
  ImgWGroup img;
  img.n = 0;
  for (int q = 0; q <= IMG_GROUP_MAX; ++q) img.first[q] = 0;
  static const int img_group = [] { const char* e = getenv("RCGAN_WGRAD_GROUP_IMG"); return e ? atoi(e) : 1; }();
  bool any_group = false;
  for (int i = 0; i < n && img_group; ++i) any_group = any_group || cand[i].takes == 1;
  for (int i = 0; i < n; ++i) {
    const rcgan_conv_desc* d = descs + i;
    bool grouped = false;
    if (any_group && img.n < IMG_GROUP_MAX && img_side(d) && (d->cin <= 3 ? d->cout : d->cin) == 128) {
      ImgWArgs ia;
      int cb = 0, nwg = 0;
      static const int img_wgs = [] { const char* e = getenv("RCGAN_WGRAD_IMG_WGS"); return e ? atoi(e) : 128; }();
      int rc = img_wgrad_plan(ctx, d, xs[i], dys[i], img_wgs, &ia, &cb, &nwg);
      if (rc) return rc;
      const long per = 32L * cb + 32;
      const size_t need = ((size_t)nwg * per * sizeof(float) + 255) / 256 * 256;
      if (used + need <= ws_bytes / 2) {
        ia.slab = (float*)((char*)ws + used);
        used += need;
        const int q = img.n++;
        img.a[q] = ia;
        for (int r = q + 1; r <= IMG_GROUP_MAX; ++r) img.first[r] = img.first[q] + (unsigned)nwg;
        const int side = img_side(d), cs = side == 1 ? d->cin : d->cout, T = d->kh * d->kw;
        SlabReduceGroup::Item it = {};
        it.slab = ia.slab; it.stride = per; it.out = dws[i]; it.count = (long)T * cs * cb; it.nz = nwg; it.accumulate = accumulate;
        it.Cb = cb; it.Cs = cs;
        if (side == 1) {
          it.orient = 0; it.bias_out = dbiases[i]; it.nbias = dbiases[i] ? cb : 0; it.bias_off = 31L * cb;
        } else {
          it.orient = 1; it.bias_out = dbiases[i]; it.nbias = dbiases[i] ? cs : 0; it.bias_off = 32L * cb + (T == 9 ? 4 : 0) * cs;
        }
        red.push_back(it);
        grouped = true;
      }
    }
    if (!grouped && mfma_wgrad_eligible(d)) {
      MfmaWgradPlanned p = {cand[i].a, 0, 0};
      MfmaWgradArgs& a = p.a;
      const int nz = cand[i].nz, takes = cand[i].takes;
      const bool nine = takes >= 2 && mfma_wgrad9_plan(a, 1 << 20, &p.gx, &p.gy, px9[takes - 2]);
      const bool three = !nine && takes && mfma_wgrad3_plan(a, nz, &p.gx, &p.gy, px);
      if (a.sub && !three && !nine) RC_FAIL(ctx, RCGAN_EUNSUPPORTED_SHAPE, "sub-pixel filter gradient needs the three-tap kernel");
      if (nine || three || mfma_wgrad_tap_plan(a, nz, &p.gx, &p.gy)) {
        const size_t need = ((size_t)p.gy * a.slab_stride * sizeof(float) + 255) / 256 * 256;
        if (used + need <= ws_bytes / 2) {
          a.slab = (float*)((char*)ws + used);
          used += need;
          if (nine) fam9[(a.sub ? 2 : 0) + (a.relu_in ? 1 : 0)].push_back(p);
          else if (three && a.sub == 3 && !a.relu_in) late.push_back(p);
          else fam[three ? (a.relu_in ? 1 : 0) : 2].push_back(p);
          red.push_back(wgrad_reduce_item(d, a, dws[i], dbiases[i], dbiases[i] ? d->cout : 0, (int)p.gy, accumulate));
          grouped = true;
        }
      }
    }
    if (!grouped) {
      int rc = rcgan_conv2d_bwd_weight(ctx, d, xs[i], dys[i], dws[i], dbiases[i], accumulate, (char*)ws + ws_bytes / 2, ws_bytes - ws_bytes / 2);
      if (rc) return rc;
    }
  }
  if (!late.empty()) {
    const int f = wgrad_busiest_family(fam, 2, (size_t)-1, false, false);
    fam[f].insert(fam[f].end(), late.begin(), late.end());
  }
  int img_f = -1;
  if (img.n) {
    img_f = wgrad_busiest_family(fam, 3, WGRAD_GROUP_MAX_HOST, true, true);
    RC_REQUIRE(ctx, img_f >= 0, "image-end filter gradients planned without a grouped launch");
  }
  int head_f = -1;
  if (ctx->head_stage == 2) head_f = (img_f == 0 || img_f == 1) ? img_f : wgrad_busiest_family(fam, 2, WGRAD_GROUP_MAX_HOST, true, true);
  for (int f = 0; f < 4; ++f)
    if (!fam9[f].empty()) {
      int rc = mfma_wgrad9_group_launch(ctx, (int)fam9[f].size(), fam9[f].data());
      if (rc) return rc;
    }
  for (int f = 0; f < 3; ++f)
    if (!fam[f].empty()) {
      int rc = mfma_wgrad3_group_launch(ctx, (int)fam[f].size(), fam[f].data(), f == 2 ? 1 : 0, f == img_f ? &img : nullptr, f == head_f);
      if (rc) return rc;
    }
  for (size_t i0 = 0; i0 < red.size(); i0 += REDUCE_GROUP_MAX) {
    SlabReduceGroup g;
    const int m = (int)((red.size() - i0 < REDUCE_GROUP_MAX) ? red.size() - i0 : REDUCE_GROUP_MAX);
    long maxc = 0;
    for (int q = 0; q < m; ++q) {
      g.it[q] = red[i0 + q];
      const long threads = (g.it[q].vec4 ? g.it[q].count / 4 : g.it[q].count) + g.it[q].nbias;
      if (threads > maxc) maxc = threads;
    }
    for (int q = m; q < REDUCE_GROUP_MAX; ++q) g.it[q] = red[i0];
    hipLaunchKernelGGL(slab_reduce2_group_kernel, dim3(cdiv(maxc, 256), m), dim3(256), 0, ctx->stream, g);
    RC_LAUNCH_CHECK(ctx);
  }
  return RCGAN_OK;
}

int rcgan_deconv2d_fwd(rcgan_ctx* ctx, const rcgan_conv_desc* d, const void* x, const float* w, const float* bias, void* y) {
  int rc = check_desc(ctx, d);
  if (rc) return rc;
  RC_DISPATCH_DTYPE(ctx, d->dtype, return direct_dgrad<T>(ctx, d, (const T*)x, w, nullptr, bias, (const T*)nullptr, (T*)y, 0));
  return RCGAN_OK;
}

int rcgan_deconv2d_bwd_data(rcgan_ctx* ctx, const rcgan_conv_desc* d, const void* dy, const float* w, void* dx) {
  return rcgan_deconv2d_bwd_data_cols(ctx, d, dy, w, dx, 0);
}

int rcgan_deconv2d_bwd_data_cols(rcgan_ctx* ctx, const rcgan_conv_desc* d, const void* dy, const float* w, void* dx, int n_cols) {
  int rc = check_desc(ctx, d);
  if (rc) return rc;
  RC_REQUIRE(ctx, n_cols >= 0 && n_cols <= d->cout, "n_cols %d of %d input channels", n_cols, d->cout);
  RC_DISPATCH_DTYPE(ctx, d->dtype, return direct_fwd<T>(ctx, d, (const T*)dy, w, nullptr, nullptr, (T*)dx, n_cols));
  return RCGAN_OK;
}

int rcgan_deconv2d_bwd_weight(rcgan_ctx* ctx, const rcgan_conv_desc* d, const void* x, const void* dy, float* dw, float* dbias,
                              int accumulate, void* ws, size_t ws_bytes) {
  int rc = check_desc(ctx, d);
  if (rc) return rc;
  RC_DISPATCH_DTYPE(ctx, d->dtype, rc = direct_wgrad<T>(ctx, d, (const T*)dy, (const T*)x, dw, nullptr, accumulate, ws, ws_bytes));
  if (rc) return rc;
  if (dbias) {
    int oh, ow, p;
    same_pad(d->h, d->kh, d->stride, &oh, &p);
    same_pad(d->w, d->kw, d->stride, &ow, &p);
    (void)oh; (void)ow;
    long rows = (long)d->n * d->h * d->w;
    size_t need = ((size_t)(cdiv(rows, 2048) + 1024) * d->cin * sizeof(float) + 255) / 256 * 256;
    float* part = (ws != nullptr && ws_bytes >= direct_wgrad_ws_bytes(d) + need) ? (float*)((char*)ws + (ws_bytes - need) / 256 * 256) : nullptr;
    RC_DISPATCH_DTYPE(ctx, d->dtype, rc = colsum_launch<T>(ctx, (const T*)dy, rows, d->cin, dbias, accumulate, part));
    if (rc) return rc;
  }
  return RCGAN_OK;
}

size_t rcgan_deconv2d_bwd_weight_concat_bytes(const rcgan_conv_desc* d, int n_cols) {
  if (!d || n_cols <= 0 || n_cols >= d->cout) return 0;
  const long rows = (long)d->n * d->h * d->w;
  return direct_wgrad_cols_ws_bytes(d, n_cols) + ((size_t)(cdiv(rows, 2048) + 1024) * d->cin * sizeof(float) + 255) / 256 * 256 + 256;
}

int rcgan_deconv2d_bwd_weight_concat(rcgan_ctx* ctx, const rcgan_conv_desc* d, const void* x, const void* dy, int n_cols, const float* yb,
                                     float* dw, float* dbias, int accumulate, void* ws, size_t ws_bytes) {
  int rc = check_desc(ctx, d);
  if (rc) return rc;
  RC_REQUIRE(ctx, n_cols > 0 && n_cols < d->cout && yb != nullptr, "%d real columns of %d, yb %p", n_cols, d->cout, (const void*)yb);
  const size_t need = rcgan_deconv2d_bwd_weight_concat_bytes(d, n_cols);
  if (ws == nullptr || ws_bytes < need) RC_FAIL(ctx, RCGAN_EWORKSPACE_TOO_SMALL, "need %zu have %zu", need, ws_bytes);
  RC_DISPATCH_DTYPE(ctx, d->dtype, rc = direct_wgrad_cols<T>(ctx, d, (const T*)dy, (const T*)x, n_cols, yb, dw, accumulate, ws, ws_bytes));
  if (rc) return rc;
  if (dbias) {
    const long rows = (long)d->n * d->h * d->w;
    const size_t tail = ((size_t)(cdiv(rows, 2048) + 1024) * d->cin * sizeof(float) + 255) / 256 * 256;
    float* part = (float*)((char*)ws + (ws_bytes - tail) / 256 * 256);
    RC_DISPATCH_DTYPE(ctx, d->dtype, rc = colsum_launch<T>(ctx, (const T*)dy, rows, d->cin, dbias, accumulate, part));
    if (rc) return rc;
  }
  return RCGAN_OK;
}

static int check_lin(rcgan_ctx* ctx, int m, int k, int n, int dtype) {
  RC_REQUIRE(ctx, m > 0 && k > 0 && n > 0, "bad linear shape [%d,%d]x[%d,%d]", m, k, k, n);
  RC_REQUIRE(ctx, dtype == RCGAN_F32 || dtype == RCGAN_H16, "bad dtype %d", dtype);
  return RCGAN_OK;
}

size_t rcgan_linear_workspace_bytes(int m, int k, int n) { return linear_wgrad_ws_bytes(m, k, n); }

int rcgan_linear_fwd(rcgan_ctx* ctx, int m, int k, int n, int dtype, const void* x, const float* w, const float* sigma,
                     const float* bias, void* y) {
  int rc = check_lin(ctx, m, k, n, dtype);
  if (rc) return rc;
  RC_DISPATCH_DTYPE(ctx, dtype, return linear_fwd<T>(ctx, m, k, n, (const T*)x, w, sigma, bias, (T*)y));
  return RCGAN_OK;
}

int rcgan_linear_bwd_data(rcgan_ctx* ctx, int m, int k, int n, int dtype, const void* dy, const float* w, const float* sigma,
                          void* dx, int accumulate) {
  int rc = check_lin(ctx, m, k, n, dtype);
  if (rc) return rc;
  RC_DISPATCH_DTYPE(ctx, dtype, return linear_dgrad<T>(ctx, m, k, n, (const T*)dy, w, sigma, (T*)dx, accumulate));
  return RCGAN_OK;
}

int rcgan_linear_bwd_weight(rcgan_ctx* ctx, int m, int k, int n, int dtype, const void* x, const void* dy, float* dw, float* dbias,
                            int accumulate, void* ws, size_t ws_bytes) {
  int rc = check_lin(ctx, m, k, n, dtype);
  if (rc) return rc;
  RC_DISPATCH_DTYPE(ctx, dtype, return linear_wgrad<T>(ctx, m, k, n, (const T*)x, (const T*)dy, dw, dbias, accumulate, ws, ws_bytes));
  return RCGAN_OK;
}

int rcgan_adam_tf(rcgan_ctx* ctx, size_t count, float* w, const float* g, float* m, float* v, const float* hyper, float beta1,
                  float beta2, float eps, float clip, float grad_scale) {
  if (count == 0) return RCGAN_OK;
  RC_REQUIRE(ctx, hyper != nullptr, "null hyper (rcgan_adam_tf_host takes {lr, t} by value)");
  adam_launch(ctx, count, w, g, m, v, hyper, 0.f, 0.f, beta1, beta2, eps, clip, grad_scale);
  RC_LAUNCH_CHECK(ctx);
  return RCGAN_OK;
}

int rcgan_adam_tf_host(rcgan_ctx* ctx, size_t count, float* w, const float* g, float* m, float* v, float lr, float t, float beta1,
                       float beta2, float eps, float clip, float grad_scale) {
  if (count == 0) return RCGAN_OK;
  adam_launch(ctx, count, w, g, m, v, nullptr, lr, t, beta1, beta2, eps, clip, grad_scale);
  RC_LAUNCH_CHECK(ctx);
  return RCGAN_OK;
}

int rcgan_set2_f32(rcgan_ctx* ctx, float* p, float a, float b) {
  RC_REQUIRE(ctx, p != nullptr, "null pointer");
  hipLaunchKernelGGL(set2_kernel, dim3(1), dim3(1), 0, ctx->stream, p, a, b);
  RC_LAUNCH_CHECK(ctx);
  return RCGAN_OK;
}

int rcgan_set_grad_scale(rcgan_ctx* ctx, float host_scale, const float* dev_scale) {
  RC_REQUIRE(ctx, host_scale > 0.f, "grad scale %g", (double)host_scale);
  ctx->gscale_host = host_scale;
  ctx->gscale_dev = dev_scale;
  return RCGAN_OK;
}

int rcgan_grad_finite_check(rcgan_ctx* ctx, size_t count, const float* g, float* ls_state) {
  RC_REQUIRE(ctx, g != nullptr && ls_state != nullptr && ((size_t)g & 15) == 0, "null / misaligned argument");
  if (count == 0) return RCGAN_OK;
  size_t blocks = (count / 4 + 255) / 256;
  if (blocks > 2048) blocks = 2048;
  if (blocks < 1) blocks = 1;
  hipLaunchKernelGGL(grad_finite_check_kernel, dim3((int)blocks), dim3(256), 0, ctx->stream, count, g, ls_state);
  RC_LAUNCH_CHECK(ctx);
  return RCGAN_OK;
}

int rcgan_adam_tf_dyn(rcgan_ctx* ctx, size_t count, float* w, const float* g, float* m, float* v, float lr, const float* t_dev, float beta1,
                      float beta2, float eps, float clip, float grad_scale, const float* ls_state) {
  RC_REQUIRE(ctx, t_dev != nullptr && ls_state != nullptr, "null t_dev / ls_state");
  if (count == 0) return RCGAN_OK;
  adam_launch(ctx, count, w, g, m, v, nullptr, lr, 0.f, beta1, beta2, eps, clip, grad_scale, AdamDyn{ls_state, t_dev});
  RC_LAUNCH_CHECK(ctx);
  return RCGAN_OK;
}

int rcgan_loss_scale_update(rcgan_ctx* ctx, float* ls_state, float* t_dev0, float* t_dev1, float growth_interval, float min_scale,
                            float max_scale) {
  RC_REQUIRE(ctx, ls_state != nullptr && growth_interval >= 1.f && min_scale > 0.f && max_scale >= min_scale, "bad loss-scale arguments");
  hipLaunchKernelGGL(loss_scale_update_kernel, dim3(1), dim3(1), 0, ctx->stream, ls_state, t_dev0, t_dev1, growth_interval, min_scale, max_scale);
  RC_LAUNCH_CHECK(ctx);
  return RCGAN_OK;
}

}
```

### robust-conditional-gan_amd/csrc/common.h

```cpp
#pragma once
#include <hip/hip_runtime.h>
#include <stdint.h>
#include <stdio.h>
#include <stdlib.h>
#include <string.h>
#include <string>
#include <vector>

#include "../../include/rcgan_hip.h"

struct rcgan_ctx {
  int device;
  hipStream_t stream;
  std::string err;
  hipEvent_t events[64];
  bool event_made[64];
  std::vector<hipGraphExec_t> graphs;
  bool capturing;
  void* devtmp;
  size_t devtmp_bytes;
  int prof_which;
  std::vector<hipEvent_t> prof_ev;
  double prof_flops, prof_flops_exec;
  int prof_bn_in = 0;
// ... 103 lines not shown

#if RCGAN_HALF_FP16
__host__ __device__ inline float bf16_to_f32(bf16_t h) { return (float)__builtin_bit_cast(_Float16, h); }
__host__ __device__ inline bf16_t f32_to_bf16(float f) { return __builtin_bit_cast(bf16_t, (_Float16)f); }
#else
__host__ __device__ inline float bf16_to_f32(bf16_t h) {
  uint32_t u = ((uint32_t)h) << 16;
  float f;
#if defined(__HIP_DEVICE_COMPILE__)
  f = __uint_as_float(u);
#else
  memcpy(&f, &u, 4);
#endif
  return f;
}

__host__ __device__ inline bf16_t f32_to_bf16(float f) {
#if defined(__HIP_DEVICE_COMPILE__)
  return __builtin_bit_cast(bf16_t, (__bf16)f);
#else
  uint32_t u;
  memcpy(&u, &f, 4);
  if ((u & 0x7fffffffu) > 0x7f800000u) return (bf16_t)((u >> 16) | 0x40);
  u += 0x7fffu + ((u >> 16) & 1u);
  return (bf16_t)(u >> 16);
#endif
}
#endif

template <typename T> struct Elem;
template <> struct Elem<float> {
  static __device__ __forceinline__ float ld(const float* p) { return *p; }
  static __device__ __forceinline__ void st(float* p, float v) { *p = v; }
};
template <> struct Elem<bf16_t> {
  static __device__ __forceinline__ float ld(const bf16_t* p) { return bf16_to_f32(*p); }
  static __device__ __forceinline__ void st(bf16_t* p, float v) { *p = f32_to_bf16(v); }
};

static inline size_t dtype_size(int dtype) { return dtype == RCGAN_H16 ? 2 : 4; }

#define RC_DISPATCH_DTYPE(ctx, dtype, ...)                              \
  do {                                                                  \
    if ((dtype) == RCGAN_F32) { typedef float T; __VA_ARGS__; }         \
    else if ((dtype) == RCGAN_H16) { typedef bf16_t T; __VA_ARGS__; }   \
    else RC_FAIL(ctx, RCGAN_EINVALID_ARG, "bad dtype %d", (int)(dtype)); \
  } while (0)

__device__ __forceinline__ float wave_sum(float v) {
#pragma unroll
  for (int o = 32; o > 0; o >>= 1) v += __shfl_xor(v, o, 64);
  return v;
}

__device__ __forceinline__ float block_sum256(float v, float* red ) {
  v = wave_sum(v);
  __syncthreads();
  if ((threadIdx.x & 63) == 0) red[threadIdx.x >> 6] = v;
  __syncthreads();
  float r = red[0] + red[1] + red[2] + red[3];
  return r;
}

__device__ __forceinline__ float act_apply(int act, float x) {
  switch (act) {
    case RCGAN_ACT_RELU: return x > 0.f ? x : 0.f;
    case RCGAN_ACT_LRELU: return fmaxf(x, 0.2f * x);
    case RCGAN_ACT_TANH: return tanhf(x);
    case RCGAN_ACT_SIGMOID: return 1.f / (1.f + expf(-x));
    default: return x;
  }
}

__device__ __forceinline__ float act_grad(int act, float s) {
  switch (act) {
    case RCGAN_ACT_RELU: return s > 0.f ? 1.f : 0.f;
    case RCGAN_ACT_LRELU: return s > 0.f ? 1.f : 0.2f;
    case RCGAN_ACT_TANH: return 1.f - s * s;
    case RCGAN_ACT_SIGMOID: return s * (1.f - s);
    default: return 1.f;
  }
}

static inline int cdiv(long a, long b) { return (int)((a + b - 1) / b); }

static inline void same_pad(int in, int k, int s, int* out, int* before) {
  int o = (in + s - 1) / s;
  int tot = (o - 1) * s + k - in;
  if (tot < 0) tot = 0;
  *out = o;
  *before = tot / 2;
}
```

### robust-conditional-gan_amd/csrc/conv_mfma.h

```cpp
#pragma once
#include "common.h"

struct ImgWArgs;
struct ImgWGroup;

struct MfmaConvArgs {
  const bf16_t* in;
  const bf16_t* wt;
  const float* bias;
  const bf16_t* mask;
  const bf16_t* resid;
  int resid_up;
  bf16_t* out;
  const bf16_t* zero;
  int N, H, W, Cin, Cout, KH, KW, PT, PL;
  int up, relu_in, accumulate;
  int cm;
  int lw, lh;
  long M;
  unsigned long long* stamps;
  const bf16_t* wph;
  int phase;
  float* stats;
  const float* bn_mean = nullptr;
  const float* bn_rstd = nullptr;
  const float* bn_gamma = nullptr;
  const float* bn_beta = nullptr;
  const int32_t* bn_labels = nullptr;
  int bn_seg_samples = 1, bn_act = 0;
};

constexpr int MFMA_FORM_PLAIN = 0;
constexpr int MFMA_FORM_PHASE = 1;
constexpr int MFMA_FORM_GATHER = 2;

static inline size_t mfma_prepared_rot(const rcgan_conv_desc* d) { return (size_t)d->kh * d->kw * d->cin * d->cout; }
static inline size_t mfma_prepared_sum_fwd(const rcgan_conv_desc* d) { return 2 * mfma_prepared_rot(d); }
static inline size_t mfma_prepared_sum_bwd(const rcgan_conv_desc* d) { return mfma_prepared_sum_fwd(d) + 16 * (size_t)d->cin * d->cout; }
static inline size_t mfma_prepared_sum_end(const rcgan_conv_desc* d) { return mfma_prepared_sum_bwd(d) + 16 * (size_t)d->cin * d->cout; }

struct MfmaWgradArgs {
  const bf16_t* x;
  const bf16_t* dy;
  float* slab;
  long slab_stride;
  int want_bias;
  const bf16_t* zero;
  int N, H, W, Cin, Cout, KH, KW, PT, PL;
  int up, relu_in, use_tr;
  int lw, lh;
  long M, m_chunk;
  int sub;
  int cells;
};
static inline int wgrad3_rows(const MfmaWgradArgs& a) { return a.sub == 3 ? 1 : (a.sub ? 8 : a.KH); }
static inline int wgrad3_alg_taps(const MfmaWgradArgs& a) { return a.sub == 3 ? 1 : (a.sub ? 36 : a.KH * a.KW); }
static inline int wgrad3_exec_taps(const MfmaWgradArgs& a) { return a.sub == 3 ? 1 : (a.sub ? 16 : a.KH * a.KW); }

struct MfmaWgradPlanned { MfmaWgradArgs a; unsigned gx, gy; };

static inline int ilog2_exact(int v) {
  int l = 0;
  while ((1 << l) < v) ++l;
  return (1 << l) == v ? l : -1;
}

bool mfma_eligible(const rcgan_conv_desc* d);
bool mfma_wgrad_eligible(const rcgan_conv_desc* d);
bool mfma_phase_filters(const rcgan_conv_desc* d);
bool mfma_phase_dgrad_ok(const rcgan_conv_desc* d);
int conv_prepare_phase_launch(rcgan_ctx* ctx, int n, const float* const* ws, const float* const* sigmas, bf16_t* const* outs, const int* cins, const int* couts,
                              const int* kinds);
bool mfma_pool_ok(const rcgan_conv_desc* d);
int mfma_conv_launch(rcgan_ctx* ctx, const MfmaConvArgs& a);
int bn_tile_stats_finish_launch(rcgan_ctx* ctx, const float* part, int c, int nseg, int tiles_per_seg, int ngroups, long group_stride,
                                double count, float eps, float* mean, float* rstd);
bool mfma_conv_is_p8(const MfmaConvArgs& a);
bool mfma_conv8_phase_form(const MfmaConvArgs& a);
int mfma_wgrad_splits(const rcgan_conv_desc* d, long M);
bool mfma_wgrad3_plan(MfmaWgradArgs& a, int nz, unsigned* gx, unsigned* gy, long px_per_block);
bool mfma_wgrad3_takes(const MfmaWgradArgs& a);
int mfma_wgrad_sub_kind(const rcgan_conv_desc* d, int use_tr);
int mfma_wgrad_sub_splits(const rcgan_conv_desc* d, long M);
int mfma_wgrad3_group_launch(rcgan_ctx* ctx, int n, const MfmaWgradPlanned* probs, int family, const ImgWGroup* img, bool carry_head = false);
bool mfma_wgrad_tap_plan(MfmaWgradArgs& a, int nz, unsigned* gx, unsigned* gy);
#define WGRAD9_GROUP_MAX 12
bool mfma_wgrad9_takes(const MfmaWgradArgs& a);
bool mfma_wgrad9_plan(MfmaWgradArgs& a, int nz, unsigned* gx, unsigned* gy, long px_per_block);
int mfma_wgrad9_group_launch(rcgan_ctx* ctx, int n, const MfmaWgradPlanned* probs);
int mfma_wgrad_launch(rcgan_ctx* ctx, MfmaWgradArgs& a, int nz, bool* bias_done, size_t ws_bytes);
int mfma_prepare_launch(rcgan_ctx* ctx, const float* w, const float* sigma, bf16_t* wt, bf16_t* wd, int T, int Cin, int Cout);
int direct_prepare_launch(rcgan_ctx* ctx, const float* w, const float* sigma, float* out, long total);
int mfma_selftest(rcgan_ctx* ctx, int* host_result);
#define WGRAD_GROUP_MAX_HOST 12
int img_side(const rcgan_conv_desc* d);
size_t img_extra_offset(const rcgan_conv_desc* d);
size_t img_extra_bytes(const rcgan_conv_desc* d);
size_t img_wgrad_ws_bytes(const rcgan_conv_desc* d);
int img_prepare_launch(rcgan_ctx* ctx, const rcgan_conv_desc* d, const float* w, const float* sigma, void* prepared);
int img_fwd(rcgan_ctx* ctx, const rcgan_conv_desc* d, const void* x, const void* prepared, const float* bias, void* y);
int img_dgrad(rcgan_ctx* ctx, const rcgan_conv_desc* d, const void* dy, const void* prepared, void* dx, int accumulate);
bool img_fwd_bn_ok(const rcgan_conv_desc* d);
int img_fwd_bn(rcgan_ctx* ctx, const rcgan_conv_desc* d, const void* x, const void* prepared, const float* bias, void* y,
               const float* mean, const float* rstd, const float* gamma, const float* beta, const int32_t* labels, int segments, int act);
int img_wgrad_plan(rcgan_ctx* ctx, const rcgan_conv_desc* d, const void* x, const void* dy, int target_wgs, ImgWArgs* a, int* cb, int* nwg);
int img_wgrad(rcgan_ctx* ctx, const rcgan_conv_desc* d, const void* x, const void* dy, float* dw, float* dbias, int accumulate,
              void* ws, size_t ws_bytes);
int mfma_conv8_launch(rcgan_ctx* ctx, const MfmaConvArgs& a, bool wide, bool halo_patch);
bool mfma_conv8_halo_takes(const MfmaConvArgs& a);
int mfma_conv8_halo_launch(rcgan_ctx* ctx, const MfmaConvArgs& a);
bool mfma_conv8n_halo_takes(const MfmaConvArgs& a);
int mfma_conv8n_halo_launch(rcgan_ctx* ctx, const MfmaConvArgs& a);
int mfma_conv_bn_route(const MfmaConvArgs& a);
struct SmallGemmArgs;
struct StepInputsArgs;
int conv_prepare_batch_launch(rcgan_ctx* ctx, const rcgan_prepare_item* items, int n, const SmallGemmArgs* gemm = nullptr,
                              const StepInputsArgs* inputs = nullptr, const rcgan_frag_item* frags = nullptr, int n_frags = 0);
```

### robust-conditional-gan_amd/csrc/conv_mfma.hip

```cpp
#include <vector>
#include "conv_mfma.h"
#include "small_gemm.h"
#include "step_inputs.h"
#include "mfma_util.h"
#include "conv_image.h"
#include "head_rider.h"

#define LDS_PITCH 72
#define WG_PITCH 144



__device__ __forceinline__ void decode_pix(long m, int H, int W, int lh, int lw, int& n, int& oh, int& ow) {
  if (lw >= 0 && lh >= 0) {
    const unsigned mm = (unsigned)m;
    ow = (int)(mm & (unsigned)(W - 1));
    oh = (int)((mm >> lw) & (unsigned)(H - 1));
    n = (int)(mm >> (lw + lh));
  } else {
    ow = (int)(m % W);
    long t = m / W;
    oh = (int)(t % H);
    n = (int)(t / H);
  }
// ... 965 lines not shown
        const int ci = ci0 + wi * 32 + j * 16 + (lane & 15);
        float4 v = make_float4(acc[t][i][j][0], acc[t][i][j][1], acc[t][i][j][2], acc[t][i][j][3]);
        *(float4*)(slab + ((long)cell * a.Cin + ci) * a.Cout + co) = v;
      }
  }
}


template <int NS, bool RELU>
__global__ __launch_bounds__(256) void conv_mfma_wgrad3_kernel(MfmaWgradArgs a) {
  if (__builtin_expect(a.sub != 0, 0)) wgrad3_body<NS, RELU, true>(a, blockIdx.x, blockIdx.y);
  else wgrad3_body<NS, RELU, false>(a, blockIdx.x, blockIdx.y);
}

#define WGRAD_GROUP_MAX 12
static_assert(WGRAD_GROUP_MAX == WGRAD_GROUP_MAX_HOST, "group size");
struct WgradGroup {
  int n;
  int xcd_runs;
  unsigned first[WGRAD_GROUP_MAX + 1];
  unsigned gx[WGRAD_GROUP_MAX];
  MfmaWgradArgs a[WGRAD_GROUP_MAX];
  ImgWGroup img;
  HeadWgradRider head;
};
static_assert(sizeof(WgradGroup) <= 4096, "kernel argument block");

template <int NS, bool RELU>
__global__ __launch_bounds__(256) void conv_mfma_wgrad3_group_kernel(WgradGroup g) {
  unsigned b = blockIdx.x;
  if (__builtin_expect(b >= g.first[g.n], 0)) {
    extern __shared__ __attribute__((aligned(16))) unsigned char smem_img[];
    const unsigned bb = b - g.first[g.n];
    if (bb >= g.img.first[IMG_GROUP_MAX]) head_wgrad_body(g.head.a, g.head.dEg, (int)(bb - g.img.first[IMG_GROUP_MAX]), (float*)smem_img);
    else img_wgrad_group_body(g.img, bb, smem_img);
    return;
  }
  if (g.xcd_runs) {
    const unsigned t8 = g.first[g.n] >> 3;
    if (b < t8 * 8) b = (b & 7) * t8 + (b >> 3);
  }
  int p = 0;
#pragma unroll
  for (int q = 1; q < WGRAD_GROUP_MAX; ++q)
    if (q < g.n && b >= g.first[q]) p = q;
  const unsigned l = b - g.first[p];
  const unsigned gxp = g.gx[p];
  if (__builtin_expect(g.a[p].sub != 0, 0)) wgrad3_body<NS, RELU, true>(g.a[p], l % gxp, l / gxp);
  else wgrad3_body<NS, RELU, false>(g.a[p], l % gxp, l / gxp);
}

template <int NS>
__global__ __launch_bounds__(256) void conv_mfma_wgrad_glds_group_kernel(WgradGroup g) {
  const unsigned b = blockIdx.x;
  if (__builtin_expect(b >= g.first[g.n], 0)) {
    extern __shared__ __attribute__((aligned(16))) unsigned char smem_img[];
    img_wgrad_group_body(g.img, b - g.first[g.n], smem_img);
    return;
  }
  int p = 0;
#pragma unroll
  for (int q = 1; q < WGRAD_GROUP_MAX; ++q)
    if (q < g.n && b >= g.first[q]) p = q;
  const unsigned l = b - g.first[p];
  const unsigned gxp = g.gx[p];
  wgrad_glds_body<NS>(g.a[p], l % gxp, l / gxp);
}

__global__ void conv_prepare_mfma_kernel(const float* w, const float* sigma, bf16_t* wt, bf16_t* wd, int T, int Cin, int Cout) {
  long idx = (long)blockIdx.x * blockDim.x + threadIdx.x;
  long total = (long)T * Cin * Cout;
  if (idx >= total) return;
  const float inv = sigma ? 1.f / *sigma : 1.f;
  int co = (int)(idx % Cout);
  long r = idx / Cout;
  int ci = (int)(r % Cin);
  int t = (int)(r / Cin);
  bf16_t v = f32_to_bf16(w[idx] * inv);
  wt[(long)co * T * Cin + (long)t * Cin + ci] = v;
  wd[(long)ci * T * Cout + (long)(T - 1 - t) * Cout + co] = v;
}

struct PhasePrepBatch { struct It { const float* w; const float* sigma; bf16_t* wph; int Cin, Cout, kind; } it[8]; };
__device__ __forceinline__ void phase_taps2(int kind, int ph, int a, int& k0, int& k1) {
  if (kind == 0) { k0 = ph == 0 ? (a == 0 ? 0 : 1) : (a == 0 ? 0 : 2); k1 = ph == 0 ? (a == 0 ? 0 : 2) : (a == 0 ? 1 : 2); }
  else {
    const int u = ph == 0 ? (a == 0 ? 3 : 1) : (a == 0 ? 2 : 0);
    k0 = u == 0 ? 0 : (u == 1 ? 0 : (u == 2 ? 1 : 2)); k1 = u == 0 ? 0 : (u == 1 ? 1 : 2);
  }
}
__device__ __forceinline__ void phase_taps4(int kind, int u, int& k0, int& k1) {
  if (kind == 0) { k0 = u == 0 ? 2 : (u == 1 ? 1 : 0); k1 = u == 0 ? 2 : (u == 1 ? 2 : (u == 2 ? 1 : 0)); }
  else { k0 = u == 0 ? 0 : (u == 1 ? 0 : (u == 2 ? 1 : 2)); k1 = u == 0 ? 0 : (u == 1 ? 1 : 2); }
}

__global__ __launch_bounds__(256) void conv_prepare_phase_kernel(PhasePrepBatch b) {
  const PhasePrepBatch::It it = b.it[blockIdx.y];
  const float inv = (it.sigma ? 1.f / *it.sigma : 1.f) * (it.kind == 1 ? 0.25f : 1.f);
  const long total = 16L * it.Cin * it.Cout;
  bf16_t* const phase_l = it.kind == 0 ? it.wph : it.wph + total;
  bf16_t* const gather_l = it.kind == 0 ? it.wph + total : it.wph;
  const bool fwd_is_phase = it.kind == 0;
  const int Op = fwd_is_phase ? it.Cout : it.Cin, Rp = fwd_is_phase ? it.Cin : it.Cout;
  const int Og = fwd_is_phase ? it.Cin : it.Cout, Rg = fwd_is_phase ? it.Cout : it.Cin;
  for (long e = (long)blockIdx.x * blockDim.x + threadIdx.x; e < total; e += (long)gridDim.x * blockDim.x) {
    {
      const long per = (long)Op * 4 * Rp;
      const int phase = (int)(e / per);
      long r = e - phase * per;
      const int o = (int)(r / (4 * Rp));
      r -= (long)o * 4 * Rp;
      const int ab = (int)(r / Rp), rr = (int)(r - (long)ab * Rp);
      int kh0, kh1, kw0, kw1;
      phase_taps2(it.kind, phase >> 1, ab >> 1, kh0, kh1);
      phase_taps2(it.kind, phase & 1, ab & 1, kw0, kw1);
      const int ci = fwd_is_phase ? rr : o, co = fwd_is_phase ? o : rr;
      float s = 0.f;
      for (int kh = kh0; kh <= kh1; ++kh)
        for (int kw = kw0; kw <= kw1; ++kw) s += it.w[(((long)kh * 3 + kw) * it.Cin + ci) * it.Cout + co];
      phase_l[e] = f32_to_bf16(s * inv);
    }
    {
      const int o = (int)(e / (16L * Rg));
      long r = e - (long)o * 16 * Rg;
      const int uv = (int)(r / Rg), rr = (int)(r - (long)uv * Rg);
      int kh0, kh1, kw0, kw1;
      phase_taps4(it.kind, uv >> 2, kh0, kh1);
      phase_taps4(it.kind, uv & 3, kw0, kw1);
      const int ci = fwd_is_phase ? o : rr, co = fwd_is_phase ? rr : o;
      float s = 0.f;
      for (int kh = kh0; kh <= kh1; ++kh)
        for (int kw = kw0; kw <= kw1; ++kw) s += it.w[(((long)kh * 3 + kw) * it.Cin + ci) * it.Cout + co];
      gather_l[e] = f32_to_bf16(s * inv);
    }
  }
}

int conv_prepare_phase_launch(rcgan_ctx* ctx, int n, const float* const* ws, const float* const* sigmas, bf16_t* const* outs, const int* cins, const int* couts,
                              const int* kinds) {
  for (int base = 0; base < n; base += 8) {
    PhasePrepBatch b;
    const int m = n - base < 8 ? n - base : 8;
    long maxel = 0;
    for (int i = 0; i < m; ++i) {
      b.it[i] = {ws[base + i], sigmas[base + i], outs[base + i], cins[base + i], couts[base + i], kinds[base + i]};
      const long el = 16L * cins[base + i] * couts[base + i];
      if (el > maxel) maxel = el;
    }
    int bx = (int)cdiv(maxel, 256 * 8);
    if (bx > 1024) bx = 1024;
    hipLaunchKernelGGL(conv_prepare_phase_kernel, dim3(bx, m), dim3(256), 0, ctx->stream, b);
    RC_LAUNCH_CHECK(ctx);
  }
  return RCGAN_OK;
}

struct PrepItem { const float* w; const float* sigma; void* out; void* extra; int T, Cin, Cout, mfma, img; };
struct FragRow { int item; int ctn, ss; bf16_t* fwd; bf16_t* bwd; };
struct PrepBatch { PrepItem it[48]; PhasePrepBatch::It ph[8]; FragRow fr[12]; int start[72]; int n, rows, frag_row0, nfrag, gemm_row, inputs_row; SmallGemmArgs gemm; StepInputsArgs inputs; };

static_assert(sizeof(PrepBatch) <= 4096, "kernel arguments are limited to 4 KiB");
constexpr int PREP_MAX_ROWS = (int)(sizeof(PrepBatch::it) / sizeof(PrepItem) + sizeof(PrepBatch::ph) / sizeof(PhasePrepBatch::It) +
                                    sizeof(PrepBatch::fr) / sizeof(FragRow)) + 2;
constexpr int PREP_ROW_STEP = 64;
static_assert(PREP_MAX_ROWS <= 2 * PREP_ROW_STEP, "the row search must reach every row a launch can hold");
static_assert(PREP_MAX_ROWS + 1 <= (int)(sizeof(PrepBatch::start) / sizeof(int)), "start[] holds rows + 1 entries");

__device__ __forceinline__ long frag_index(int row, int k, int ctn, int ss, int nsl) {
  const int blk = row / (16 * ctn), ct = (row - blk * 16 * ctn) >> 4, r = row & 15;
  const int ks = k >> 5, sl = ks / ss, s = ks - sl * ss, kc = (k >> 3) & 3, e = k & 7;
  return ((((long)(blk * nsl + sl) * ss + s) * ctn + ct) * 64 + kc * 16 + r) * 8 + e;
}

__device__ __forceinline__ void prepare_fragment_units(const PrepItem& it, const FragRow& fr, bf16_t (*tile)[66], int bid, int nb) {
  const float inv = it.sigma ? 1.f / *it.sigma : 1.f;
  const int nci = it.Cin / 64, nco = it.Cout / 64;
  const int ntiles = it.T * nci * nco;
// ... 752 lines not shown
```

### robust-conditional-gan_amd/csrc/sn.hip

```cpp
#include <algorithm>
#include <utility>
#include <vector>

#include "common.h"

#define SN_MAX_K 4096
#define SN_MAX_C 1024
#define SN_BATCH 24
#define SN_EPS 1e-12f
#define SN_RB 32
#define SN_NT 256
#define SN_NW (SN_NT / 64)
#define SN_MAX_CHUNKS (SN_MAX_K / SN_RB)

struct SnLayout {
  float *a, *v, *dv, *b, *u2, *uin, *db, *s, *pb, *pgw, *pdva;
  int chunks;
};
__host__ __device__ inline int sn_chunks(int k) { return (k + SN_RB - 1) / SN_RB; }
__device__ __forceinline__ SnLayout sn_layout(float* save, int k, int c) {
  SnLayout L;
  L.chunks = sn_chunks(k);
  const int kp = (k + 3) & ~3, cp = (c + 3) & ~3;
  L.a = save; L.v = L.a + kp; L.dv = L.v + kp;
// ... 47 lines not shown
    if (lane == 0 && r < rows) { a_s[r] = s; __hip_atomic_store(L.a + r0 + r, s, __ATOMIC_RELAXED, __HIP_MEMORY_SCOPE_AGENT); }
  }
  __syncthreads();
  for (int j = tid; j < c; j += SN_NT) {
    float s = 0.f;
#pragma unroll 8
    for (int r = 0; r < rows; ++r) s += a_s[r] * w[(long)r * c + j];
    __hip_atomic_store(L.pb + (long)blockIdx.x * c + j, s, __ATOMIC_RELAXED, __HIP_MEMORY_SCOPE_AGENT);
  }
  if (batch.arrive == nullptr) return;
  __shared__ int is_last;
  __shared__ float red[SN_NW];
  asm volatile("s_waitcnt vmcnt(0)" ::: "memory");
  __syncthreads();
  if (tid == 0) {
    unsigned* ctr = batch.arrive + blockIdx.y * 32;
    const unsigned prev = __hip_atomic_fetch_add(ctr, 1u, __ATOMIC_RELAXED, __HIP_MEMORY_SCOPE_AGENT);
    is_last = prev == (unsigned)L.chunks - 1u ? 1 : 0;
    if (is_last) __hip_atomic_store(ctr, 0u, __ATOMIC_RELAXED, __HIP_MEMORY_SCOPE_AGENT);
  }
  __syncthreads();
  if (!is_last) return;
  sn_fwd_finish<true>(it, red);
}

template <bool AGENT>
__device__ __forceinline__ void sn_fwd_finish(const rcgan_sn_item& it, float* red) {
  const int k = it.k, c = it.c;
  const SnLayout L = sn_layout(it.save, k, c);
  const int tid = threadIdx.x;
  auto ld = [&](const float* p) __attribute__((always_inline)) -> float {
    return AGENT ? __hip_atomic_load(p, __ATOMIC_RELAXED, __HIP_MEMORY_SCOPE_AGENT) : *p;
  };
  float na2 = 0.f;
  for (int r = tid; r < k; r += SN_NT) { float a = ld(L.a + r); na2 += a * a; }
  na2 = block_sum_nt(na2, red);
  const float na = sqrtf(na2);
  const float inv_na = 1.f / (na + SN_EPS);
  for (int r = tid; r < k; r += SN_NT) L.v[r] = ld(L.a + r) * inv_na;
  float nb2 = 0.f;
  for (int j = tid; j < c; j += SN_NT) {
    float s = 0.f;
#pragma unroll 12
    for (int q = 0; q < L.chunks; ++q) s += ld(L.pb + (long)q * c + j);
    s *= inv_na;
    L.b[j] = s;
    nb2 += s * s;
  }
  nb2 = block_sum_nt(nb2, red);
  const float nb = sqrtf(nb2);
  const float inv_nb = 1.f / (nb + SN_EPS);
  float sg = 0.f;
  for (int j = tid; j < c; j += SN_NT) {
    float b = L.b[j];
    float u2 = b * inv_nb;
    L.u2[j] = u2;
    L.uin[j] = it.u[j];
    if (it.update) it.u[j] = u2;
    sg += b * u2;
  }
  sg = block_sum_nt(sg, red);
  if (tid == 0) {
    L.s[0] = na; L.s[1] = nb; L.s[2] = sg; L.s[3] = 0.f;
    *it.sigma = sg;
  }
}
__global__ __launch_bounds__(SN_NT) void sn_fwd_finish_kernel(SnBatch batch) {
  __shared__ float red[SN_NW];
  sn_fwd_finish<false>(batch.it[blockIdx.x], red);
}

#define SN_MAX_RANGES 48
struct SnAdam {
  float *w_base, *m_base, *v_base, *g_base;
  const float* hyper;
  float beta1, beta2, eps, clip, grad_scale;
  int riders;
  int n_ranges;
  unsigned lo[SN_MAX_RANGES], hi[SN_MAX_RANGES];
};

__device__ __forceinline__ void sn_adam_elem(float g, float& m, float& v, float& w, float alpha, float omb1, float omb2, float eps, float clip,
                                             float grad_scale) {
  const float gi = g * grad_scale;
  m = m + (gi - m) * omb1;
  v = v + (gi * gi - v) * omb2;
  w = w - (m * alpha) / (sqrtf(v) + eps);
  if (clip > 0.f) w = fminf(fmaxf(w, -clip), clip);
}

__global__ __launch_bounds__(SN_NT) void sn_bwd_p1_kernel(SnBwdBatch batch, float* hyper_inc) {
  __shared__ float q_s[SN_MAX_C];
  __shared__ float red[SN_NW];
  if (hyper_inc != nullptr && blockIdx.x == 0 && blockIdx.y == 0 && threadIdx.x == 0) hyper_inc[1] += 1.f;
  const rcgan_sn_bwd_item it = batch.it[blockIdx.y];
  const int k = it.k, c = it.c;
  const int r0 = blockIdx.x * SN_RB;
  if (r0 >= k) return;
  const int rows = min(SN_RB, k - r0);
  const SnLayout L = sn_layout(it.save, k, c);
  const float* w = it.w + (long)r0 * c;
  const float* g = it.dwbar + (long)r0 * c;
  const int tid = threadIdx.x, lane = tid & 63, wave = tid >> 6;
  constexpr int NR = SN_RB / SN_NW;
  const bool small_c = c <= 128;
  float wr[NR][2], gr[NR][2];
  if (small_c) {
#pragma unroll
    for (int i = 0; i < NR; ++i) {
      const int r = wave + i * SN_NW;
#pragma unroll
      for (int e = 0; e < 2; ++e) {
        const int j = lane + 64 * e;
        const bool ok = r < rows && j < c;
        wr[i][e] = ok ? w[(long)r * c + j] : 0.f;
        gr[i][e] = ok ? g[(long)r * c + j] : 0.f;
      }
    }
  }
  const float nb = L.s[1];
  float s2 = 0.f;
  for (int j = tid; j < c; j += SN_NT) { const float b = L.b[j]; s2 += b * b; }
  s2 = block_sum_nt(s2, red);
  const float inv_nb = 1.f / (nb + SN_EPS);
  const float coef_q = s2 / (nb * (nb + SN_EPS) * (nb + SN_EPS));
  for (int j = tid; j < c; j += SN_NT) {
    const float b = L.b[j];
    const float q = L.u2[j] + b * inv_nb - b * coef_q;
    q_s[j] = q;
    if (blockIdx.x == 0) L.db[j] = q;
  }
  __syncthreads();
  float gw = 0.f, pa = 0.f;
  float part[SN_RB / SN_NW], av[SN_RB / SN_NW];
#pragma unroll
  for (int i = 0; i < SN_RB / SN_NW; ++i) {
    const int r = wave + i * SN_NW;
    float s = 0.f;
    if (small_c) {
      const float q0 = lane < c ? q_s[lane] : 0.f, q1 = lane + 64 < c ? q_s[lane + 64] : 0.f;
      s = wr[i][0] * q0 + wr[i][1] * q1;
      gw += gr[i][0] * wr[i][0] + gr[i][1] * wr[i][1];
    } else if (r < rows) {
      for (int j = lane; j < c; j += 64) {
        const float wv = w[(long)r * c + j];
        s += wv * q_s[j];
        gw += g[(long)r * c + j] * wv;
      }
    }
    part[i] = s;
    av[i] = (lane == 0 && r < rows) ? L.a[r0 + r] : 0.f;
  }
#pragma unroll
  for (int i = 0; i < SN_RB / SN_NW; ++i) {
    const int r = wave + i * SN_NW;
    const float s = wave_sum(part[i]);
    if (lane == 0 && r < rows) { L.dv[r0 + r] = s; pa += s * av[i]; }
  }
  gw = block_sum_nt(gw, red);
  pa = block_sum_nt(lane == 0 ? pa : 0.f, red);
  if (tid == 0) { L.pgw[blockIdx.x] = gw; L.pdva[blockIdx.x] = pa; }
}

template <bool ADAM>
__global__ __launch_bounds__(SN_NT) void sn_bwd_p2_kernel(SnBwdBatch batch, int n_items, SnAdam ad) {
  __shared__ float da_s[SN_RB];
  __shared__ float v_s[SN_RB];
  __shared__ float red[SN_NW];
  const int tid = threadIdx.x;
  float alpha = 0.f, omb1 = 0.f, omb2 = 0.f;
  if (ADAM) {
// ... 227 lines not shown
```

### robust-conditional-gan_amd/ops.py

```python
import ctypes as C
import os

import torch

from . import _lib as L
from .runtime import DT


def _p(t):
    return C.c_void_p(t.ptr) if t is not None else None


def same_pad(n, k, s):
    out = -(-n // s)
    tot = max((out - 1) * s + k - n, 0)
    return out, tot // 2


def zeros_like_grad(ctx, t):
    g = ctx.empty(t.shape, t.dtype)
    ctx.check(ctx.lib.rcgan_fill_f32(ctx.h, (g.nbytes + 3) // 4, g.ptr, 0.0))
    return g


def grad_of(ctx, t):
    if t.grad is None:
        t.grad = ctx.empty(t.shape, t.dtype)
        return t.grad, 0
    if getattr(t.grad, "frozen", False):
        fresh = ctx.empty(t.shape, t.dtype)
        ctx.check(ctx.lib.rcgan_axpby(ctx.h, t.size, t.dtype, 1.0, _p(t.grad), 0.0, _p(fresh)))
        t.grad = fresh
    return t.grad, 1


def _track(ctx, out, *ins):
    out.req = ctx.recording and any(i is not None and i.req for i in ins)
    return out.req


class Weight:

    def __init__(self, ctx, param, sigma=None):
        self.ctx, self.param, self.sigma = ctx, param, sigma
        self._prepared = {}
        self.rf_frag = None
        self.dwbar = None
        self._conv1 = None

    @property
    def req(self):
        return self.param.req

    @staticmethod
    def _key(desc, nbytes):
        resample = (L.CONV_IN_UPSAMPLE2X | L.CONV_OUT_MEANPOOL2) if (desc.kh == 3 and desc.kw == 3) else 0
        return (desc.kh, desc.kw, desc.cin, desc.cout, desc.dtype, desc.stride, desc.flags & (L.CONV_FORCE_DIRECT | resample), nbytes)

    def prepared(self, desc):
        ctx = self.ctx
        nbytes = ctx.lib.rcgan_conv_prepared_bytes(C.byref(desc))
        key = self._key(desc, nbytes)
        if key not in self._prepared:
            buf = DT(ctx.arena.alloc(nbytes), (nbytes,), "u8", ctx.arena.buf)
            ctx.check(ctx.lib.rcgan_conv_prepare(ctx.h, C.byref(desc), _p(self.param), _p(self.sigma), _p(buf)))
            self._prepared[key] = buf
        return self._prepared[key]

    def as_conv1x1(self):
        if self._conv1 is None:
            p = self.param
            pv = DT(p.ptr, (1, 1) + tuple(p.shape), p.dtype, p.base, p.name)
            pv.req, pv.group = p.req, p.group
            if p.grad is not None:
                pv.grad = p.grad.reshape((1, 1) + tuple(p.shape))
            w4 = Weight(self.ctx, pv, self.sigma)
            w4._prepared = self._prepared
            self._conv1 = w4
        return self._conv1

    def grad_target(self):
        if self.sigma is None:
            return self.param.grad
        if self.dwbar is None:
            self.dwbar = DT(self.ctx.arena.alloc(self.param.nbytes), self.param.shape, L.F32, self.ctx.arena.buf)
            self.ctx.check(self.ctx.lib.rcgan_fill_f32(self.ctx.h, self.param.size, self.dwbar.ptr, 0.0))
        return self.dwbar


def prepare_batch(ctx, weights_and_shapes, dtype, persistent=None, embed=None, inputs=None, frags=None):
    todo = []
    index = {}
    for w, k, stride, hw, *rest in weights_and_shapes:
        cin, cout = w.param.shape[-2:]
        desc = L.ConvDesc(1, hw, hw, cin, cout, k, k, stride, dtype, rest[0] if rest else 0)
        nbytes = ctx.lib.rcgan_conv_prepared_bytes(C.byref(desc))
        key = Weight._key(desc, nbytes)
        if persistent is None:
            if key in w._prepared:
                continue
            buf = DT(ctx.arena.alloc(nbytes), (nbytes,), "u8", ctx.arena.buf)
        else:
            slot = persistent.setdefault(w.param.name, {})
            if key not in slot:
                t = torch.empty(int(nbytes), dtype=torch.uint8, device=ctx.device)
                slot[key] = DT(t.data_ptr(), (nbytes,), "u8", t)
            buf = slot[key]
        w._prepared[key] = buf
        index[id(w)] = len(todo)
        todo.append(L.PrepareItem(desc, w.param.ptr, w.sigma.ptr if w.sigma is not None else None, buf.ptr))
    fitems = [(index[id(w)], f, b, ctn, ss, w) for (w, f, b, ctn, ss) in (frags or []) if id(w) in index]
    if todo:
        arr = (L.PrepareItem * len(todo))(*todo)
        if fitems and len(fitems) <= 12:
            ed = si = None
            if embed is not None:
                table, w_e, b_e, E = embed
                v, e_dim = table.shape
                ed = L.EmbedDesc(v, e_dim, w_e.param.shape[-1], table.ptr, w_e.param.ptr, w_e.sigma.ptr if w_e.sigma is not None else None,
                                 b_e.ptr if b_e is not None else None, E.ptr)
            if inputs is not None:
                si = inputs
            fa = (L.FragItem * len(fitems))(*[L.FragItem(i, ctn, ss, f, b) for i, f, b, ctn, ss, _ in fitems])
            ctx.check(ctx.lib.rcgan_conv_prepare_batch_frags(ctx.h, arr, len(todo), C.byref(ed) if ed is not None else None,
                                                             C.byref(si) if si is not None else None, fa, len(fitems)))
            return (embed is not None or inputs is not None), {id(w) for *_, w in fitems}
        if embed is not None or inputs is not None:
            ed = si = None
            if embed is not None:
                table, w_e, b_e, E = embed
                v, e_dim = table.shape
                ed = L.EmbedDesc(v, e_dim, w_e.param.shape[-1], table.ptr, w_e.param.ptr, w_e.sigma.ptr if w_e.sigma is not None else None,
                                 b_e.ptr if b_e is not None else None, E.ptr)
            if inputs is not None:
                si = inputs
            ctx.check(ctx.lib.rcgan_conv_prepare_batch_riders(ctx.h, arr, len(todo), C.byref(ed) if ed is not None else None,
                                                              C.byref(si) if si is not None else None))
            return True if frags is None else (True, set())
        ctx.check(ctx.lib.rcgan_conv_prepare_batch(ctx.h, arr, len(todo)))
    return False if frags is None else (False, set())


RF_CONV = os.environ.get("RCGAN_RF_CONV", "1") != "0"
CONCAT_DIRECT = os.environ.get("RCGAN_CONCAT_DIRECT", "1") != "0"
CONCAT_WGRAD = os.environ.get("RCGAN_CONCAT_WGRAD", "1") != "0"
LINEAR_MFMA = os.environ.get("RCGAN_LINEAR_MFMA", "1") != "0"


FRAG_IN_PREPARE = os.environ.get("RCGAN_FRAG_IN_PREPARE", "0") == "1"


def fragment_requests(ctx, trunk, rf):
    reqs, tf = [], None
    if trunk:
        nb = ctx.lib.rcgan_dtrunk_fragment_bytes()
        tf = DT(ctx.arena.alloc(nb), (nb,), "u8", ctx.arena.buf)
        elems2 = 9 * 128 * 128 * 2
        for i, w in enumerate(trunk):
            reqs.append((w, tf.ptr + i * elems2, tf.ptr + (8 + (7 - i)) * elems2, 2, 36))
    for w, d in rf:
        nb = ctx.lib.rcgan_conv_rf_fragment_bytes(C.byref(d))
        w.rf_frag = DT(ctx.arena.alloc(nb), (nb,), "u8", ctx.arena.buf)
        reqs.append((w, w.rf_frag.ptr, w.rf_frag.ptr + nb // 2, 4, 18))
    return tf, reqs


def fragments_batch(ctx, trunk, rf):
    tp = tf = None
    if trunk:
        tdesc = L.ConvDesc(1, 8, 8, 128, 128, 3, 3, 1, ctx.act_dtype, L.CONV_IN_RELU)
        tp = (C.c_void_p * 8)(*[w.prepared(tdesc).ptr for w in trunk])
        nb = ctx.lib.rcgan_dtrunk_fragment_bytes()
        tf = DT(ctx.arena.alloc(nb), (nb,), "u8", ctx.arena.buf)
    n = len(rf)
    descs = (L.ConvDesc * max(n, 1))(*[d for _, d in rf])
    preps = (C.c_void_p * max(n, 1))(*[w.prepared(d).ptr for w, d in rf])
    frags = []
    for w, d in rf:
        nb = ctx.lib.rcgan_conv_rf_fragment_bytes(C.byref(d))
        w.rf_frag = DT(ctx.arena.alloc(nb), (nb,), "u8", ctx.arena.buf)
        frags.append(w.rf_frag.ptr)
    ctx.check(ctx.lib.rcgan_fragments_prepare(ctx.h, tp, _p(tf), n, descs, preps, (C.c_void_p * max(n, 1))(*frags)))
    return tf


def spectral_norm_batch(ctx, entries):
    n = len(entries)
    if n == 0:
        return []
    items = (L.SnItem * n)()
    weights = []
    saves = []
    for i, (param, u, update) in enumerate(entries):
# ... 917 lines not shown
```

### robust-conditional-gan_amd/runtime.py

```python
import ctypes as C

import os

import numpy as np
import torch

from . import _lib as L

ALIGN = 256


def _np_dtype(code):
    return np.float32 if code == L.F32 else np.uint16


class DT:
    __slots__ = ("ptr", "shape", "dtype", "base", "grad", "req", "name", "frozen", "group", "tile_stats", "pooled", "pool_grad", "concat_src", "concat_labels")

    def __init__(self, ptr, shape, dtype, base=None, name=None):
        self.ptr = int(ptr)
        self.shape = tuple(int(s) for s in shape)
        self.dtype = dtype
        self.base = base
        self.grad = None
# ... 19 lines not shown
        if self.dtype == "u8":
            return 1
        return 4 if self.dtype in (L.F32, "i32") else 2

    @property
    def nbytes(self):
        return self.size * self.itemsize

    def reshape(self, *shape):
        if len(shape) == 1 and isinstance(shape[0], (tuple, list)):
            shape = tuple(shape[0])
        shape = list(shape)
        if -1 in shape:
            known = 1
            for s in shape:
                if s != -1:
                    known *= s
            shape[shape.index(-1)] = self.size // known
        t = DT(self.ptr, shape, self.dtype, self.base, self.name)
        assert t.size == self.size, (self.shape, shape)
        return t

    def rows(self, lo, hi):
        stride = self.size // self.shape[0]
        return DT(self.ptr + lo * stride * self.itemsize, (hi - lo,) + self.shape[1:], self.dtype, self.base, self.name)


class Arena:
    def __init__(self, nbytes, device):
        self.buf = torch.empty(int(nbytes), dtype=torch.uint8, device=device)
        self.base = self.buf.data_ptr()
        self.cap = int(nbytes)
        self.off = 0
        self.peak = 0

    def reset(self):
        self.off = 0

    def alloc(self, nbytes):
        off = (self.off + ALIGN - 1) // ALIGN * ALIGN
        if off + nbytes > self.cap:
            raise MemoryError("activation arena exhausted: need %d more bytes (capacity %d); raise arena_bytes"
                              % (off + nbytes - self.cap, self.cap))
        self.off = off + int(nbytes)
        self.peak = max(self.peak, self.off)
        return self.base + off


def check_f32_matmul_precision(precision, dtype):
    if precision not in L.F32_PRECISIONS:
        raise ValueError("Unknown f32_matmul_precision %r: one of %s" % (precision, ", ".join(sorted(L.F32_PRECISIONS))))
    if precision != "highest" and dtype != "f32":
        raise ValueError("f32_matmul_precision=%r needs dtype='f32' (got %r)" % (precision, dtype))
    return precision


class Context:

    def __init__(self, device=0, dtype="bf16", arena_bytes=6 << 30, ws_bytes=1 << 30):
        if not torch.cuda.is_available():
            raise RuntimeError("no HIP device visible: the RCGAN engine has no CPU fallback")
        if dtype in ("f16", "fp16", L.F16):
            self.act_dtype, self.lib = L.F16, L.load("f16")
        else:
            self.act_dtype, self.lib = (L.BF16 if dtype in ("bf16", L.BF16) else L.F32), L.load()
        self.device = torch.device("cuda", device)
        torch.cuda.set_device(self.device)
        self.stream = torch.cuda.Stream(device=self.device)
        h = C.c_void_p()
        rc = self.lib.rcgan_create(C.byref(h), device, C.c_void_p(self.stream.cuda_stream))
        if rc != 0:
            raise L.RcganError(rc, "rcgan_create failed")
        self.h = h
        self.arena = Arena(arena_bytes, self.device)
        self.ws = torch.empty(int(ws_bytes), dtype=torch.uint8, device=self.device)
        self.ws_ptr, self.ws_bytes = self.ws.data_ptr(), int(ws_bytes)
        self.epoch = 0
        self.overlap = os.environ.get("RCGAN_OVERLAP", "0") == "1"
        self.ws2 = torch.empty(int(ws_bytes), dtype=torch.uint8, device=self.device) if self.overlap else None
        self.ws2_ptr = self.ws2.data_ptr() if self.overlap else 0
        self.tape = []
        self.sn_partial = []
        self.pending_wgrads = []
        self.group_wgrads = os.environ.get("RCGAN_GROUP_WGRAD", "1") == "1"
        self.recording = True
        self.capturing = False
        self._keep = []
        self.check(self.lib.rcgan_selftest(self.h))
        self.uses_tr_read = self.lib.rcgan_query(self.h, L.QUERY_TR_READ)

    def check(self, rc):
        if rc != 0:
            raise L.RcganError(rc, self.lib.rcgan_last_error(self.h).decode())

    def close(self):
        for c in getattr(self, "also_close", []):
            c.close()
        self.also_close = []
        if self.h is not None:
            self.lib.rcgan_destroy(self.h)
            self.h = None

    def empty(self, shape, dtype=None, name=None):
        dtype = self.act_dtype if dtype is None else dtype
        n = 1
        for s in shape:
            n *= int(s)
        isz = 4 if dtype in (L.F32, "i32") else 2
        return DT(self.arena.alloc(max(n, 1) * isz), shape, dtype, self.arena.buf, name)

    def persistent(self, shape, dtype=L.F32, fill=None):
        tdt = {L.F32: torch.float32, L.BF16: torch.bfloat16, L.F16: torch.float16, "i32": torch.int32}[dtype]
        t = torch.empty(tuple(int(s) for s in shape) or (1,), dtype=tdt, device=self.device)
        if fill is not None:
            with torch.cuda.stream(self.stream):
                t.fill_(fill)
        self._keep.append(t)
        return DT(t.data_ptr(), shape, dtype, t)

    def view(self, t):
        tdt = {L.F32: torch.float32, L.BF16: torch.bfloat16, L.F16: torch.float16, "i32": torch.int32}[t.dtype]
        if isinstance(t.base, torch.Tensor):
            base = t.base
            off = t.ptr - base.data_ptr()
            raw = base.view(torch.uint8).reshape(-1)[off:off + t.nbytes]
            return raw.view(tdt).reshape(t.shape if t.shape else (1,))
        raise ValueError("DT has no torch base")

    def upload(self, arr, dtype=None, out=None):
        arr = np.asarray(arr)
        if arr.dtype.kind in "iub":
            dtype = "i32"
            src = torch.from_numpy(np.ascontiguousarray(arr.astype(np.int32)))
        else:
            dtype = self.act_dtype if dtype is None else dtype
            src = torch.from_numpy(np.ascontiguousarray(arr.astype(np.float32)))
        if out is None:
            out = self.empty(arr.shape, dtype)
        with torch.cuda.stream(self.stream):
            self.view(out).copy_(src.reshape(out.shape if out.shape else (1,)), non_blocking=False)
        return out

    def download(self, t):
        with torch.cuda.stream(self.stream):
            v = self.view(t).float() if t.dtype != "i32" else self.view(t)
            out = v.cpu()
        self.stream.synchronize()
        return out.numpy().reshape(t.shape)

    def sync(self):
        self.check(self.lib.rcgan_stream_sync(self.h))

    def set_f32_matmul_precision(self, precision):
        self.check(self.lib.rcgan_set_f32_matmul_precision(self.h, L.F32_PRECISIONS[precision]))
        self.f32_matmul_precision = precision

    def zeros(self, shape, dtype=None):
        t = self.empty(shape, dtype)
        with torch.cuda.stream(self.stream):
            self.view(t).zero_()
        return t

    def record(self, fn):
        if self.recording:
            self.tape.append(fn)

    def backward(self):
        for fn in reversed(self.tape):
            fn()
        self.tape = []
        self.flush_wgrads()

    def defer_wgrad(self, desc, x, dy, dw, dbias):
        self.pending_wgrads.append((desc, x, dy, dw, dbias))

    def flush_wgrads(self):
        pend = self.pending_wgrads
        if pend:
            self.pending_wgrads = []
            n = len(pend)
            descs = (L.ConvDesc * n)(*[p[0] for p in pend])
            arr = lambda k: (C.c_void_p * n)(*[(p[k].ptr if p[k] is not None else None) for p in pend])
            xs, dys, dws, dbs = arr(1), arr(2), arr(3), arr(4)
            self.check(self.lib.rcgan_conv2d_bwd_weight_group(self.h, n, descs, xs, dys, dws, dbs, 1, C.c_void_p(self.ws_ptr), self.ws_bytes))
        self.check(self.lib.rcgan_head_flush(self.h))

    def new_step(self):
        self.check(self.lib.rcgan_head_flush(self.h))
        self.tape = []
        self.sn_partial = []
        self.pending_wgrads = []
        self.arena.reset()
        self.epoch += 1

    def reserve_scratch(self, nbytes):
        self.check(self.lib.rcgan_reserve_scratch(self.h, C.c_size_t(int(nbytes))))

    def graph_begin(self):
        self.check(self.lib.rcgan_graph_begin(self.h))
        self.capturing = True

    def graph_end(self):
        gid = C.c_int(-1)
        self.capturing = False
        self.check(self.lib.rcgan_graph_end(self.h, C.byref(gid)))
        return gid.value

    def graph_abort(self):
        self.capturing = False
        self.check(self.lib.rcgan_graph_abort(self.h))

    def graph_launch(self, gid):
        self.check(self.lib.rcgan_graph_launch(self.h, gid))

    def event_record(self, slot):
        self.check(self.lib.rcgan_event_record(self.h, slot))

    def event_elapsed_ms(self, a, b):
        ms = C.c_float(0)
        self.check(self.lib.rcgan_event_elapsed_ms(self.h, a, b, C.byref(ms)))
        return ms.value


class ParamGroup:

    def __init__(self, ctx, specs, sn_scratch=False):
        self.ctx = ctx
        self.names, self.offsets, self.shapes = [], {}, {}
        off = 0
        for name, shape, _ in specs:
            off = (off + 63) // 64 * 64
            self.names.append(name)
            self.offsets[name] = off
            self.shapes[name] = tuple(shape)
            n = 1
            for s in shape:
                n *= int(s)
            off += n
        self.count = max((off + 63) // 64 * 64, 64)
        dev = ctx.device
        self.value = torch.zeros(self.count, dtype=torch.float32, device=dev)
        self.sn_scratch = bool(sn_scratch)
        self._extra = self.count if sn_scratch else 0
        self.gradbuf = torch.zeros(self.count + self._extra + 64, dtype=torch.float32, device=dev)
        self.grad = self.gradbuf[:self.count]
        self.zero_epoch = -1
        self.m = torch.zeros(self.count, dtype=torch.float32, device=dev)
        self.v = torch.zeros(self.count, dtype=torch.float32, device=dev)
        self._lr, self._t = 0.0, 0.0
        self.t = 0
        self.hyper = None
        self.t_dev = None
        self.version = 0
        host = np.zeros(self.count, np.float32)
        for name, shape, init in specs:
            o = self.offsets[name]
            a = np.asarray(init, np.float32).reshape(-1)
            host[o:o + a.size] = a
        self.value.copy_(torch.from_numpy(host))
        torch.cuda.synchronize()

    @classmethod
    def alias(cls, ctx, other):
        g = cls.__new__(cls)
        g.__dict__.update(other.__dict__)
        g.ctx = ctx
        return g

    def _on_stream(self):
        return torch.cuda.stream(self.ctx.stream)

    def param(self, name):
        o = self.offsets[name] * 4
        p = DT(self.value.data_ptr() + o, self.shapes[name], L.F32, self.value, name)
# ... 89 lines not shown
```

### robust-conditional-gan_amd/variables.py

```python
import contextlib

from . import ops as O

_scope_stack = []


@contextlib.contextmanager
def variable_scope(name):
    _scope_stack.append(name)
    try:
        yield "/".join(_scope_stack)
    finally:
        _scope_stack.pop()


def scoped(name):
    return "/".join(_scope_stack + [name])


class Graph:

    current = None

    def __init__(self, ctx, groups, state):
        self.ctx = ctx
        self.groups = groups
        self.state = state
        self.trainable = set()
        self._params = {}
        self.sn = {}
        self.plain = {}
        self.persist = {}
        self.index = {}
        for gi, g in enumerate(groups):
            for n in g.names:
                self.index[n] = gi

    def begin_step(self, trainable_groups):
        self.trainable = set(trainable_groups)
        self._params = {}
        self.sn = {}
        self.plain = {}
        self.image_pool = None
        self.head_E = None
        self.trunk_frag = None
        self.early_d = None
        self.early_g = None
        Graph.current = self

    def param(self, name):
        if name not in self._params:
            if name not in self.index:
                raise KeyError("Variable %s does not exist (variables are created up-front)" % name)
            gi = self.index[name]
            p = self.groups[gi].param(name)
            p.req = gi in self.trainable
            self._params[name] = p
        return self._params[name]

    def has(self, name):
        return name in self.index

    def prefetch_sn(self, entries):
        ents = [(self.param(pn), self.state[un], upd) for pn, un, upd in entries]
        ws = O.spectral_norm_batch(self.ctx, ents)
        for (pn, _, upd), w in zip(entries, ws):
            self.sn[pn] = (w, upd)

    def sn_weight(self, pname, uname, update):
        if pname not in self.sn:
            self.prefetch_sn([(pname, uname, update)])
        w, upd = self.sn[pname]
        if bool(upd) != bool(update):
            raise ValueError("spectral norm of %s was prefetched with update=%s but used with update=%s" % (pname, upd, update))
        return w

    def prepare_convs(self, names, dtype, embed=None, inputs=None, frags=None):
        ws = []
        for pn, k, stride, hw, *rest in names:
            w = self.sn[pn][0] if pn in self.sn else self.weight(pn)
            ws.append((w, k, stride, hw, *rest))
        return O.prepare_batch(self.ctx, ws, dtype, embed=embed, inputs=inputs, frags=frags)

    def refresh_persistent(self, names, dtype):
        ws = [(O.Weight(self.ctx, self.groups[self.index[pn]].param(pn), None), k, stride, hw, *rest) for pn, k, stride, hw, *rest in names]
        O.prepare_batch(self.ctx, ws, dtype, persistent=self.persist)

    def weight(self, pname):
        if pname not in self.plain:
            w = O.Weight(self.ctx, self.param(pname), None)
            w._prepared.update(self.persist.get(pname, {}))
            self.plain[pname] = w
        return self.plain[pname]
```

Baseline: 58340.

## Fuse generator wgrad slab reduction with Adam update and bf16 weight prepare

Adds a kernel that reduces the generator's grouped weight-gradient slabs and, in the same pass, applies the Adam update and writes the prepared bf16 weight layouts (transposed, phase and gather forms) through LDS tiles. This replaces a separate reduce kernel, the optimiser step, and the weight-prepare refresh for the generator, avoiding extra launches and repeated reads of gradients and weights. It also merges the two hyper-parameter writes into a single kernel. The host now has to track the generator's step count and prepared-weight version itself, and the fused path only runs when there is no data parallelism, no dynamic loss scaling and bf16 activations, so it adds complexity and risks state getting out of sync.

Measured after the change: 58350 (median of 3 runs). About the same (+0.0%).

```diff
diff --git a/include/rcgan_hip.h b/include/rcgan_hip.h
--- a/include/rcgan_hip.h
+++ b/include/rcgan_hip.h
@@ -130,6 +130,15 @@
                             float* dw, float* dbias, int accumulate, void* ws, size_t ws_bytes);
 int rcgan_conv2d_bwd_weight_group(rcgan_ctx* ctx, int n, const rcgan_conv_desc* descs, const void* const* xs, const void* const* dys,
                                   float* const* dws, float* const* dbiases, int accumulate, void* ws, size_t ws_bytes);
+typedef struct rcgan_wgrad_adam {
+  float* w; float* g; float* m; float* v; size_t count;
+  const float* hyper;
+  float beta1, beta2, eps, clip, grad_scale;
+  const rcgan_prepare_item* prep; int n_prep;
+} rcgan_wgrad_adam;
+int rcgan_conv2d_bwd_weight_group_adam(rcgan_ctx* ctx, int n, const rcgan_conv_desc* descs, const void* const* xs, const void* const* dys,
+                                       float* const* dws, float* const* dbiases, int accumulate, void* ws, size_t ws_bytes,
+                                       const rcgan_wgrad_adam* opt, int* fused);
 
 int rcgan_deconv2d_fwd(rcgan_ctx* ctx, const rcgan_conv_desc* d, const void* x, const float* w,
                        const float* bias, void* y);
@@ -330,6 +339,7 @@
 int rcgan_comm_stub_model(rcgan_ctx* ctx, double bus_gbps, double latency_us);
 const char* rcgan_comm_load_error(void);
 int rcgan_set2_f32(rcgan_ctx* ctx, float* p, float a, float b);
+int rcgan_set2x2_f32(rcgan_ctx* ctx, float* p0, float a0, float b0, float* p1, float a1, float b1);
 
 int rcgan_selftest(rcgan_ctx* ctx);
 #define RCGAN_QUERY_TR_READ 0
diff --git a/robust-conditional-gan_amd/_lib.py b/robust-conditional-gan_amd/_lib.py
--- a/robust-conditional-gan_amd/_lib.py
+++ b/robust-conditional-gan_amd/_lib.py
@@ -92,6 +92,12 @@
     _fields_ = [("w", C.c_void_p), ("g", C.c_void_p), ("m", C.c_void_p), ("v", C.c_void_p), ("count", C.c_size_t),
                 ("hyper", C.c_void_p), ("beta1", C.c_float), ("beta2", C.c_float), ("eps", C.c_float), ("clip", C.c_float),
                 ("grad_scale", C.c_float), ("n_ranges", C.c_int), ("ranges", C.POINTER(C.c_size_t))]
+
+
+class WgradAdam(C.Structure):
+    _fields_ = [("w", C.c_void_p), ("g", C.c_void_p), ("m", C.c_void_p), ("v", C.c_void_p), ("count", C.c_size_t),
+                ("hyper", C.c_void_p), ("beta1", C.c_float), ("beta2", C.c_float), ("eps", C.c_float), ("clip", C.c_float),
+                ("grad_scale", C.c_float), ("prep", C.POINTER(PrepareItem)), ("n_prep", C.c_int)]
 
 
 P, I, F, SZ = C.c_void_p, C.c_int, C.c_float, C.c_size_t
@@ -142,6 +148,7 @@
     "rcgan_conv2d_bwd_data_residual": (I, [P, DP, P, P, P, P, P, P, SZ]),
     "rcgan_conv2d_bwd_weight": (I, [P, DP, P, P, P, P, I, P, SZ]),
     "rcgan_conv2d_bwd_weight_group": (I, [P, I, P, P, P, P, P, I, P, SZ]),
+    "rcgan_conv2d_bwd_weight_group_adam": (I, [P, I, P, P, P, P, P, I, P, SZ, C.POINTER(WgradAdam), C.POINTER(I)]),
     "rcgan_deconv2d_fwd": (I, [P, DP, P, P, P, P]),
     "rcgan_deconv2d_bwd_data": (I, [P, DP, P, P, P]),
     "rcgan_deconv2d_bwd_data_cols": (I, [P, DP, P, P, P, I]),
@@ -236,6 +243,7 @@
     "rcgan_comm_stub_model": (I, [P, C.c_double, C.c_double]),
     "rcgan_comm_load_error": (C.c_char_p, []),
     "rcgan_set2_f32": (I, [P, P, F, F]),
+    "rcgan_set2x2_f32": (I, [P, P, F, F, P, F, F]),
     "rcgan_set_grad_scale": (I, [P, F, P]),
     "rcgan_set_f32_matmul_precision": (I, [P, I]),
     "rcgan_grad_finite_check": (I, [P, SZ, P, P]),
diff --git a/robust-conditional-gan_amd/cifar.py b/robust-conditional-gan_amd/cifar.py
--- a/robust-conditional-gan_amd/cifar.py
+++ b/robust-conditional-gan_amd/cifar.py
@@ -392,6 +392,9 @@
                                                     os.environ.get("RCGAN_GRAPH_ADAM", "0") == "1")
         self.fused_tail = (not self.dp_active and not self.dynamic_ls and not self.graph_adam
                            and os.environ.get("RCGAN_SN_ADAM", "1") == "1")
+        self.g_tail = (not self.dp_active and not self.dynamic_ls and not self.graph_adam and ctx.act_dtype != L.F32
+                       and os.environ.get("RCGAN_G_TAIL", "1") == "1")
+        self.g_tail_fused = False
         self._tail_fused = {}
         B = self.B
         f32, i32, act = L.F32, "i32", ctx.act_dtype
@@ -703,8 +706,22 @@
         if self.perm:
             logits = perm_classifier(fake, self.perm_type)
             O.bce_onehot_term(ctx, logits, inp["labels_random_G"], self.perm_mult, self.loss_g)
+        tail = None
+        if self.g_tail and ctx.recording and self.PG.hyper is not None:
+            tail = ctx.wgrad_tail = self._g_tail_request()
         ctx.backward()
+        ctx.wgrad_tail = None
+        if ctx.recording:
+            self.g_tail_fused = bool(tail is not None and tail.get("fused", False))
         self._dp_finish([self.PG] + ([self.PC] if self.PC is not None else []))
+
+    def _g_tail_request(self):
+        pg = self.PG
+        items = self.graph.persistent_items(self._filter_names(pg), self.ctx.act_dtype)
+        arr = (L.PrepareItem * max(len(items), 1))(*items)
+        opt = L.WgradAdam(pg.value.data_ptr(), pg.grad.data_ptr(), pg.m.data_ptr(), pg.v.data_ptr(), pg.count, pg.hyper.data_ptr(),
+                          0.0, 0.9, 1e-8, 0.0, 1.0 / (self.world * self.loss_scale), arr, len(items))
+        return {"opt": opt, "items": arr}
 
     def _g_head_unfused(self, fake, lab, n):
         ctx, inp = self.ctx, self.inp
@@ -813,6 +830,18 @@
             for grp, lr in steps:
                 grp.t += 1
                 grp.set_hyper_device(lr, grp.t)
+        if self.g_tail:
+            for grp, lr in steps:
+                if grp is not self.PG:
+                    continue
+                pd = self.PD
+                pd_stale = self.fused_tail and getattr(pd, "_dev_hyper", None) != (float(lr), pd.t)
+                if pd_stale and pd.hyper is not None and grp.hyper is not None and max(grp.t + 1, pd.t) < (1 << 24):
+                    self.ctx.check(self.ctx.lib.rcgan_set2x2_f32(self.ctx.h, grp.hyper.data_ptr(), float(lr), float(grp.t + 1),
+                                                                 pd.hyper.data_ptr(), float(lr), float(pd.t)))
+                    pd._dev_hyper = (float(lr), pd.t)
+                else:
+                    grp.set_hyper_device(lr, grp.t + 1)
 
     def _gf_body(self):
         ctx, g, B, inp = self.ctx, self.graph, self.B, self.inp
@@ -955,7 +984,13 @@
             steps.append((self.PC, self.lr * self.confuse_multiplier * (lr_decay(it) if self.confuse_lr_decay else 1.0)))
         self._pre_step(steps)
         self._run("g", self._g_body)
-        self._optimise_or_publish(steps)
+        if self.g_tail_fused:
+            self.PG.t += 1
+            self.PG.version += 1
+            self._pg_prepared_version = self.PG.version
+            steps = steps[1:]
+        if steps:
+            self._optimise_or_publish(steps)
         self._refresh_generator_filters()
 
     def _optimise(self, steps):
diff --git a/robust-conditional-gan_amd/csrc/api.hip b/robust-conditional-gan_amd/csrc/api.hip
--- a/robust-conditional-gan_amd/csrc/api.hip
+++ b/robust-conditional-gan_amd/csrc/api.hip
@@ -49,9 +49,19 @@
   } it[REDUCE_GROUP_MAX];
 };
 __device__ __forceinline__ float4 f4add(float4 a, float4 b) { return make_float4(a.x + b.x, a.y + b.y, a.z + b.z, a.w + b.w); }
-__global__ void slab_reduce2_group_kernel(SlabReduceGroup g) {
-  const SlabReduceGroup::Item& r = g.it[blockIdx.y];
-  long i = (long)blockIdx.x * blockDim.x + threadIdx.x;
+struct SlabStore {
+  __device__ __forceinline__ void put4(float* o, float4 s, int accumulate) const {
+    float4* p = (float4*)o;
+    if (accumulate) s = f4add(s, *p);
+    *p = s;
+  }
+  __device__ __forceinline__ void put1(float* o, float s, int accumulate) const {
+    if (accumulate) s += *o;
+    *o = s;
+  }
+};
+template <class Sink>
+__device__ __forceinline__ void slab_reduce_elem(const SlabReduceGroup::Item& r, long i, const Sink& sink) {
   if (r.vec4) {
     const long nv = r.count >> 2;
     if (i < nv) {
@@ -95,9 +105,7 @@
 #pragma unroll 4
         for (; z < r.nz; ++z) s = f4add(s, *(const float4*)(r.slab + (long)z * r.stride + e));
       }
-      float4* o = (float4*)(r.out + e);
-      if (r.accumulate) s = f4add(s, *o);
-      *o = s;
+      sink.put4(r.out + e, s, r.accumulate);
       return;
     }
     i = r.count + (i - nv);
@@ -155,8 +163,10 @@
     const int t = k / r.Cs, c = k - t * r.Cs;
     o = r.out + ((long)t * r.Cb + n) * r.Cs + c;
   }
-  if (r.accumulate) s += *o;
-  *o = s;
+  sink.put1(o, s, r.accumulate);
+}
+__global__ void slab_reduce2_group_kernel(SlabReduceGroup g) {
+  slab_reduce_elem(g.it[blockIdx.y], (long)blockIdx.x * blockDim.x + threadIdx.x, SlabStore());
 }
 
 struct AdamDyn { const float* ls; const float* tdev; };
@@ -209,7 +219,243 @@
   }
 }
 
+#define GTAIL_MAX_RANGES 48
+constexpr int GT_TS = 32;
+struct GTailTile { bf16_t* wt; bf16_t* wph; int T, Cin, Cout, kind; };
+struct GTail {
+  SlabReduceGroup::Item it[REDUCE_GROUP_MAX];
+  GTailTile tile[REDUCE_GROUP_MAX];
+  int start[REDUCE_GROUP_MAX + 2];
+  int n;
+  float *w, *m, *v, *g;
+  const float* hyper;
+  float beta1, beta2, eps, clip, grad_scale;
+  int n_ranges;
+  unsigned lo[GTAIL_MAX_RANGES], hi[GTAIL_MAX_RANGES];
+};
+static_assert(sizeof(GTail) <= 4096, "kernel arguments are limited to 4 KiB");
+
+struct SlabAdam {
+  float *w, *m, *v, *g;
+  float alpha, omb1, omb2, eps, clip, grad_scale;
+  __device__ __forceinline__ void step(float gr, float& mm, float& vv, float& ww) const {
+    adam_tf_elem(gr, mm, vv, ww, alpha, omb1, omb2, eps, clip, grad_scale);
+  }
+  __device__ __forceinline__ void put4(float* o, float4 s, int accumulate) const {
+    const long off = o - g;
+    float4 m4 = *(const float4*)(m + off), v4 = *(const float4*)(v + off), w4 = *(const float4*)(w + off);
+    float4* p = (float4*)o;
+    if (accumulate) s = f4add(s, *p);
+    *p = s;
+    step(s.x, m4.x, v4.x, w4.x);
+    step(s.y, m4.y, v4.y, w4.y);
+    step(s.z, m4.z, v4.z, w4.z);
+    step(s.w, m4.w, v4.w, w4.w);
+    *(float4*)(m + off) = m4; *(float4*)(v + off) = v4; *(float4*)(w + off) = w4;
+  }
+  __device__ __forceinline__ void put1(float* o, float s, int accumulate) const {
+    const long off = o - g;
+    float mm = m[off], vv = v[off], ww = w[off];
+    if (accumulate) s += *o;
+    *o = s;
+    step(s, mm, vv, ww);
+    m[off] = mm; v[off] = vv; w[off] = ww;
+  }
+};
+
+template <int T, int ZU>
+__device__ __forceinline__ void gtail_sum_plain(const float* slab, unsigned rem, long stride, long cc, int& z, int nz, float (&acc)[T]) {
+  for (; z + ZU <= nz; z += ZU) {
+    float v[ZU][T];
+#pragma unroll
+    for (int u = 0; u < ZU; ++u)
+#pragma unroll
+      for (int t = 0; t < T; ++t) v[u][t] = (slab + ((long)(z + u) * stride + (long)t * cc))[rem];
+#pragma unroll
+    for (int u = 0; u < ZU; ++u)
+#pragma unroll
+      for (int t = 0; t < T; ++t) acc[t] += v[u][t];
+  }
+}
+template <int SUB, int ZU>
+__device__ __forceinline__ void gtail_sum_sub(const float* slab, unsigned rem, long stride, long cc, int& z, int nz, float (&acc)[9]) {
+  for (; z + ZU <= nz; z += ZU) {
+    float v[ZU][16];
+#pragma unroll
+    for (int u = 0; u < ZU; ++u)
+#pragma unroll
+      for (int c = 0; c < 16; ++c) v[u][c] = (slab + ((long)(z + u) * stride + (long)c * cc))[rem];
+#pragma unroll
+    for (int u = 0; u < ZU; ++u)
+#pragma unroll
+      for (int tap = 0; tap < 9; ++tap) {
+        const int kh = tap / 3, kw = tap - kh * 3;
+        int c4[4];
+#pragma unroll
+        for (int q = 0; q < 4; ++q) {
+          const int pa = q >> 1, pb = q & 1;
+          const int sa = ((SUB == 1) == (pa == 0)) ? (kh >= 1) : (kh >= 2);
+          const int sb = ((SUB == 1) == (pb == 0)) ? (kw >= 1) : (kw >= 2);
+          c4[q] = q * 4 + sa * 2 + sb;
+        }
+        acc[tap] += (v[u][c4[0]] + v[u][c4[1]]) + (v[u][c4[2]] + v[u][c4[3]]);
+      }
+  }
+}
+
+constexpr int GT_SLOTS = 9 + 16;
+template <int T, int KIND>
+__device__ __forceinline__ void gtail_tile_body(const SlabReduceGroup::Item& r, const GTailTile& tl, const SlabAdam& ad, int tile,
+                                                bf16_t (*lds)[GT_TS][GT_TS + 2]) {
+  constexpr int NP = GT_TS * GT_TS / 256;
+  const int Cin = tl.Cin, Cout = tl.Cout;
+  const int nco = Cout / GT_TS;
+  const int ci0 = (tile / nco) * GT_TS, co0 = (tile - (tile / nco) * nco) * GT_TS;
+  const int lane = threadIdx.x & (GT_TS - 1), g8 = threadIdx.x / GT_TS;
+  const long cc = (long)Cin * Cout;
+  const long ob = r.out - ad.g;
+  bf16_t* const wt = tl.wt;
+  bf16_t* const wd = wt + (long)T * cc;
+  constexpr bool fwd_is_phase = KIND == 0;
+  const long total = 16L * cc;
+  bf16_t* const phase_l = KIND == 0 ? tl.wph : tl.wph + total;
+  bf16_t* const gather_l = KIND == 0 ? tl.wph + total : tl.wph;
+#pragma unroll 1
+  for (int p = 0; p < NP; ++p) {
+    const int cil = g8 + 8 * p;
+    const unsigned rem = (unsigned)(ci0 + cil) * (unsigned)Cout + (unsigned)(co0 + lane);
+    float go[T], mo[T], vo[T], wo[T];
+#pragma unroll
+    for (int t = 0; t < T; ++t) {
+      const long e = ob + (long)t * cc;
+      go[t] = r.accumulate ? (ad.g + e)[rem] : 0.f;
+      mo[t] = (ad.m + e)[rem]; vo[t] = (ad.v + e)[rem]; wo[t] = (ad.w + e)[rem];
+    }
+    float acc[T];
+#pragma unroll
+    for (int t = 0; t < T; ++t) acc[t] = 0.f;
+    int z = 0;
+    if constexpr (T == 9) {
+      if (r.sub == 1) {
+        gtail_sum_sub<1, 2>(r.slab, rem, r.stride, cc, z, r.nz, acc);
+        gtail_sum_sub<1, 1>(r.slab, rem, r.stride, cc, z, r.nz, acc);
+      } else if (r.sub == 2) {
+        gtail_sum_sub<2, 2>(r.slab, rem, r.stride, cc, z, r.nz, acc);
+        gtail_sum_sub<2, 1>(r.slab, rem, r.stride, cc, z, r.nz, acc);
+#pragma unroll
+        for (int t = 0; t < T; ++t) acc[t] *= 0.25f;
+      } else {
+        gtail_sum_plain<T, 3>(r.slab, rem, r.stride, cc, z, r.nz, acc);
+        gtail_sum_plain<T, 1>(r.slab, rem, r.stride, cc, z, r.nz, acc);
+      }
+    } else {
+      gtail_sum_plain<T, 16>(r.slab, rem, r.stride, cc, z, r.nz, acc);
+      gtail_sum_plain<T, 4>(r.slab, rem, r.stride, cc, z, r.nz, acc);
+      gtail_sum_plain<T, 1>(r.slab, rem, r.stride, cc, z, r.nz, acc);
+    }
+#pragma unroll
+    for (int t = 0; t < T; ++t) {
+      const long e = ob + (long)t * cc;
+      float s = acc[t];
+      if (r.accumulate) s += go[t];
+      (ad.g + e)[rem] = s;
+      ad.step(s, mo[t], vo[t], wo[t]);
+      (ad.m + e)[rem] = mo[t]; (ad.v + e)[rem] = vo[t]; (ad.w + e)[rem] = wo[t];
+    }
+    const float inv = 1.f;
+    const unsigned rowd = (unsigned)(ci0 + cil) * (unsigned)(T * Cout) + (unsigned)(co0 + lane);
+#pragma unroll
+    for (int t = 0; t < T; ++t) {
+      const bf16_t h = f32_to_bf16(wo[t] * inv);
+      (wd + (long)(T - 1 - t) * Cout)[rowd] = h;
+      lds[t][cil][lane] = h;
+    }
+    if constexpr (KIND >= 0) {
+      const float pinv = 1.f * (KIND == 1 ? 0.25f : 1.f);
+#pragma unroll
+      for (int cls = 0; cls < 32; ++cls) {
+        const bool is_phase = cls < 16;
+        const int c = cls & 15;
+        int kh0, kh1, kw0, kw1;
+        if (is_phase) { phase_taps2(KIND, c >> 3, (c >> 1) & 1, kh0, kh1); phase_taps2(KIND, (c >> 2) & 1, c & 1, kw0, kw1); }
+        else { phase_taps4(KIND, c >> 2, kh0, kh1); phase_taps4(KIND, c & 3, kw0, kw1); }
+        const bool o_is_co = is_phase ? fwd_is_phase : !fwd_is_phase;
+        float s = 0.f;
+#pragma unroll
+        for (int j = 0; j < 4; ++j) {
+          const int kh = kh0 + (j >> 1), kw = kw0 + (j & 1);
+          const bool on = kh <= kh1 && kw <= kw1;
+          s += on ? wo[on ? kh * 3 + kw : 0] : 0.f;
+        }
+        const bf16_t h = f32_to_bf16(s * pinv);
+        if (o_is_co) lds[9 + c][cil][lane] = h;
+        else {
+          bf16_t* const dst = is_phase ? phase_l + (long)(c >> 2) * Cin * 4 * Cout + (long)(c & 3) * Cout : gather_l + (long)c * Cout;
+          const long ostride = is_phase ? 4L * Cout : 16L * Cout;
+          dst[(unsigned)(ci0 + cil) * (unsigned)ostride + (unsigned)(co0 + lane)] = h;
+        }
+      }
+    }
+  }
+  __syncthreads();
+#pragma unroll 1
+  for (int p = 0; p < NP; ++p) {
+    const int col = g8 + 8 * p;
+#pragma unroll
+    for (int t = 0; t < T; ++t) (wt + (long)t * Cin)[(unsigned)(co0 + col) * (unsigned)(T * Cin) + (unsigned)(ci0 + lane)] = lds[t][lane][col];
+    if constexpr (KIND >= 0) {
+#pragma unroll
+      for (int c = 0; c < 16; ++c) {
+        bf16_t* const dst = fwd_is_phase ? phase_l + (long)(c >> 2) * Cout * 4 * Cin + (long)(c & 3) * Cin : gather_l + (long)c * Cin;
+        const long ostride = fwd_is_phase ? 4L * Cin : 16L * Cin;
+        dst[(unsigned)(co0 + col) * (unsigned)ostride + (unsigned)(ci0 + lane)] = lds[9 + c][lane][col];
+      }
+    }
+  }
+}
+
+__global__ __launch_bounds__(256, 2) void slab_reduce_adam_prepare_kernel(GTail P) {
+  __shared__ bf16_t lds[GT_SLOTS][GT_TS][GT_TS + 2];
+  int row = 0;
+  for (int q = 1; q <= P.n; ++q)
+    if ((int)blockIdx.x >= P.start[q]) row = q;
+  const int bid = (int)blockIdx.x - P.start[row], nb = P.start[row + 1] - P.start[row];
+  const float lr = P.hyper[0], t = P.hyper[1];
+  SlabAdam ad;
+  ad.w = P.w; ad.m = P.m; ad.v = P.v; ad.g = P.g;
+  ad.alpha = lr * sqrtf(1.f - powf(P.beta2, t)) / (1.f - powf(P.beta1, t));
+  ad.omb1 = 1.f - P.beta1; ad.omb2 = 1.f - P.beta2;
+  ad.eps = P.eps; ad.clip = P.clip; ad.grad_scale = P.grad_scale;
+  if (row == P.n) {
+    for (int rg = 0; rg < P.n_ranges; ++rg)
+      for (unsigned o = P.lo[rg] + (unsigned)bid * 256u + threadIdx.x; o < P.hi[rg]; o += (unsigned)nb * 256u) {
+        float mm = P.m[o], vv = P.v[o], ww = P.w[o];
+        ad.step(P.g[o], mm, vv, ww);
+        P.m[o] = mm; P.v[o] = vv; P.w[o] = ww;
+      }
+    return;
+  }
+  const SlabReduceGroup::Item& r = P.it[row];
+  const GTailTile& tl = P.tile[row];
+  if (tl.wt != nullptr) {
+    const int ntile = (tl.Cin / GT_TS) * (tl.Cout / GT_TS);
+    if (bid < ntile) {
+      if (tl.T == 1) gtail_tile_body<1, -1>(r, tl, ad, bid, lds);
+      else if (tl.kind < 0) gtail_tile_body<9, -1>(r, tl, ad, bid, lds);
+      else if (tl.kind == 0) gtail_tile_body<9, 0>(r, tl, ad, bid, lds);
+      else gtail_tile_body<9, 1>(r, tl, ad, bid, lds);
+      return;
+    }
+    const long k = (long)(bid - ntile) * 256 + threadIdx.x;
+    if (k >= r.nbias) return;
+    slab_reduce_elem(r, (r.vec4 ? (r.count >> 2) : r.count) + k, ad);
+    return;
+  }
+  slab_reduce_elem(r, (long)bid * 256 + threadIdx.x, ad);
+}
+
 __global__ void set2_kernel(float* p, float a, float b) { p[0] = a; p[1] = b; }
+__global__ void set2x2_kernel(float* p0, float a0, float b0, float* p1, float a1, float b1) { p0[0] = a0; p0[1] = b0; p1[0] = a1; p1[1] = b1; }
 
 __global__ void grad_finite_check_kernel(size_t count, const float* g, float* ls) {
   bool bad = false;
@@ -1007,7 +1253,91 @@
 
 int rcgan_conv2d_bwd_weight_group(rcgan_ctx* ctx, int n, const rcgan_conv_desc* descs, const void* const* xs, const void* const* dys,
                                   float* const* dws, float* const* dbiases, int accumulate, void* ws, size_t ws_bytes) {
+  return rcgan_conv2d_bwd_weight_group_adam(ctx, n, descs, xs, dys, dws, dbiases, accumulate, ws, ws_bytes, nullptr, nullptr);
+}
+
+static bool g_tail_plan(const std::vector<SlabReduceGroup::Item>& red, const rcgan_wgrad_adam* opt, GTail& P, std::vector<rcgan_prepare_item>& rest,
+                        int* grid) {
+  if (red.empty() || red.size() > REDUCE_GROUP_MAX) return false;
+  if (!opt->w || !opt->g || !opt->m || !opt->v || !opt->hyper || opt->count == 0 || opt->count >= ((size_t)1 << 31)) return false;
+  if ((((size_t)opt->w | (size_t)opt->g | (size_t)opt->m | (size_t)opt->v) & 15) != 0) return false;
+  if (opt->n_prep < 0 || (opt->n_prep > 0 && !opt->prep)) return false;
+  const size_t count = opt->count;
+  std::vector<std::pair<size_t, size_t>> cover;
+  std::vector<char> used(opt->n_prep, 0);
+  P.n = (int)red.size();
+  int at = 0;
+  for (int q = 0; q < P.n; ++q) {
+    const SlabReduceGroup::Item& it = red[q];
+    if (it.out < opt->g || it.count <= 0) return false;
+    const size_t off = (size_t)(it.out - opt->g);
+    if (off >= count || (size_t)it.count > count - off) return false;
+    if (it.vec4 && (off & 3)) return false;
+    cover.push_back({off, off + (size_t)it.count});
+    if (it.nbias > 0) {
+      if (!it.bias_out || it.bias_out < opt->g) return false;
+      const size_t boff = (size_t)(it.bias_out - opt->g);
+      if (boff >= count || (size_t)it.nbias > count - boff) return false;
+      cover.push_back({boff, boff + (size_t)it.nbias});
+    }
+    P.it[q] = it;
+    GTailTile& tl = P.tile[q];
+    tl = GTailTile{nullptr, nullptr, 0, 0, 0, -1};
+    for (int j = 0; j < opt->n_prep && it.orient == 0; ++j) {
+      const rcgan_prepare_item& pi = opt->prep[j];
+      const rcgan_conv_desc& d = pi.desc;
+      if (used[j] || pi.w != opt->w + off || pi.sigma != nullptr || pi.prepared == nullptr) continue;
+      const int T = d.kh * d.kw;
+      if (!(d.kh == d.kw && (T == 1 || T == 9)) || d.cin % GT_TS || d.cout % GT_TS || !mfma_eligible(&d)) continue;
+      if (it.count != (long)T * d.cin * d.cout || (it.sub != 0 && (T != 9 || it.cc != (long)d.cin * d.cout))) continue;
+      tl.wt = (bf16_t*)pi.prepared;
+      tl.T = T; tl.Cin = d.cin; tl.Cout = d.cout;
+      if (mfma_phase_filters(&d)) {
+        tl.kind = (d.flags & RCGAN_CONV_OUT_MEANPOOL2) ? 1 : 0;
+        tl.wph = tl.wt + mfma_prepared_sum_fwd(&d);
+      }
+      used[j] = 1;
+      break;
+    }
+    P.start[q] = at;
+    if (tl.wt) at += (tl.Cin / GT_TS) * (tl.Cout / GT_TS) + cdiv(it.nbias, 256);
+    else at += cdiv((it.vec4 ? it.count / 4 : it.count) + it.nbias, 256);
+  }
+  std::sort(cover.begin(), cover.end());
+  P.n_ranges = 0;
+  size_t pos = 0, loose = 0;
+  for (size_t c = 0; c <= cover.size(); ++c) {
+    const size_t lo = c < cover.size() ? cover[c].first : count, hi = c < cover.size() ? cover[c].second : count;
+    if (lo < pos) return false;
+    if (lo > pos) {
+      if (P.n_ranges == GTAIL_MAX_RANGES) return false;
+      P.lo[P.n_ranges] = (unsigned)pos; P.hi[P.n_ranges] = (unsigned)lo;
+      ++P.n_ranges;
+      loose += lo - pos;
+    }
+    pos = hi;
+  }
+  P.start[P.n] = at;
+  int riders = cdiv((long)loose, 256 * 4);
+  if (riders > 256) riders = 256;
+  at += riders;
+  P.start[P.n + 1] = at;
+  for (int q = P.n; q < REDUCE_GROUP_MAX; ++q) { P.it[q] = red[0]; P.tile[q] = GTailTile{nullptr, nullptr, 0, 0, 0, -1}; }
+  P.w = opt->w; P.m = opt->m; P.v = opt->v; P.g = opt->g; P.hyper = opt->hyper;
+  P.beta1 = opt->beta1; P.beta2 = opt->beta2; P.eps = opt->eps; P.clip = opt->clip; P.grad_scale = opt->grad_scale;
+  rest.clear();
+  for (int j = 0; j < opt->n_prep; ++j)
+    if (!used[j]) rest.push_back(opt->prep[j]);
+  *grid = at;
+  return true;
+}
+
+int rcgan_conv2d_bwd_weight_group_adam(rcgan_ctx* ctx, int n, const rcgan_conv_desc* descs, const void* const* xs, const void* const* dys,
+                                       float* const* dws, float* const* dbiases, int accumulate, void* ws, size_t ws_bytes,
+                                       const rcgan_wgrad_adam* opt, int* fused) {
+  if (fused) *fused = 0;
   RC_REQUIRE(ctx, n >= 0 && (n == 0 || (descs && xs && dys && dws && dbiases)), "null argument");
+  RC_REQUIRE(ctx, (opt == nullptr) == (fused == nullptr), "opt and fused come together");
   static const int target_blocks = [] { const char* e = getenv("RCGAN_WGRAD_GROUP_BLOCKS"); return e ? atoi(e) : 448; }();
   struct Cand { MfmaWgradArgs a; int nz; int takes; };
   std::vector<Cand> cand(n);
@@ -1149,6 +1479,21 @@
       int rc = mfma_wgrad3_group_launch(ctx, (int)fam[f].size(), fam[f].data(), f == 2 ? 1 : 0, f == img_f ? &img : nullptr, f == head_f);
       if (rc) return rc;
     }
+  if (opt) {
+    static GTail tail;
+    std::vector<rcgan_prepare_item> rest;
+    int grid = 0;
+    if (g_tail_plan(red, opt, tail, rest, &grid)) {
+      hipLaunchKernelGGL(slab_reduce_adam_prepare_kernel, dim3(grid), dim3(256), 0, ctx->stream, tail);
+      RC_LAUNCH_CHECK(ctx);
+      if (!rest.empty()) {
+        int rc = conv_prepare_batch_launch(ctx, rest.data(), (int)rest.size());
+        if (rc) return rc;
+      }
+      *fused = 1;
+      return RCGAN_OK;
+    }
+  }
   for (size_t i0 = 0; i0 < red.size(); i0 += REDUCE_GROUP_MAX) {
     SlabReduceGroup g;
     const int m = (int)((red.size() - i0 < REDUCE_GROUP_MAX) ? red.size() - i0 : REDUCE_GROUP_MAX);
@@ -1278,6 +1623,13 @@
   return RCGAN_OK;
 }
 
+int rcgan_set2x2_f32(rcgan_ctx* ctx, float* p0, float a0, float b0, float* p1, float a1, float b1) {
+  RC_REQUIRE(ctx, p0 != nullptr && p1 != nullptr && p0 != p1, "null or repeated pointer");
+  hipLaunchKernelGGL(set2x2_kernel, dim3(1), dim3(1), 0, ctx->stream, p0, a0, b0, p1, a1, b1);
+  RC_LAUNCH_CHECK(ctx);
+  return RCGAN_OK;
+}
+
 int rcgan_set2_f32(rcgan_ctx* ctx, float* p, float a, float b) {
   RC_REQUIRE(ctx, p != nullptr, "null pointer");
   hipLaunchKernelGGL(set2_kernel, dim3(1), dim3(1), 0, ctx->stream, p, a, b);
diff --git a/robust-conditional-gan_amd/csrc/common.h b/robust-conditional-gan_amd/csrc/common.h
--- a/robust-conditional-gan_amd/csrc/common.h
+++ b/robust-conditional-gan_amd/csrc/common.h
@@ -209,6 +209,15 @@
   }
 }
 
+__device__ __forceinline__ void adam_tf_elem(float g, float& m, float& v, float& w, float alpha, float omb1, float omb2, float eps, float clip,
+                                             float grad_scale) {
+  const float gi = g * grad_scale;
+  m = m + (gi - m) * omb1;
+  v = v + (gi * gi - v) * omb2;
+  w = w - (m * alpha) / (sqrtf(v) + eps);
+  if (clip > 0.f) w = fminf(fmaxf(w, -clip), clip);
+}
+
 static inline int cdiv(long a, long b) { return (int)((a + b - 1) / b); }
 
 static inline void same_pad(int in, int k, int s, int* out, int* before) {
diff --git a/robust-conditional-gan_amd/csrc/conv_mfma.h b/robust-conditional-gan_amd/csrc/conv_mfma.h
--- a/robust-conditional-gan_amd/csrc/conv_mfma.h
+++ b/robust-conditional-gan_amd/csrc/conv_mfma.h
@@ -38,6 +38,18 @@
 static inline size_t mfma_prepared_sum_fwd(const rcgan_conv_desc* d) { return 2 * mfma_prepared_rot(d); }
 static inline size_t mfma_prepared_sum_bwd(const rcgan_conv_desc* d) { return mfma_prepared_sum_fwd(d) + 16 * (size_t)d->cin * d->cout; }
 static inline size_t mfma_prepared_sum_end(const rcgan_conv_desc* d) { return mfma_prepared_sum_bwd(d) + 16 * (size_t)d->cin * d->cout; }
+
+__device__ __forceinline__ void phase_taps2(int kind, int ph, int a, int& k0, int& k1) {
+  if (kind == 0) { k0 = ph == 0 ? (a == 0 ? 0 : 1) : (a == 0 ? 0 : 2); k1 = ph == 0 ? (a == 0 ? 0 : 2) : (a == 0 ? 1 : 2); }
+  else {
+    const int u = ph == 0 ? (a == 0 ? 3 : 1) : (a == 0 ? 2 : 0);
+    k0 = u == 0 ? 0 : (u == 1 ? 0 : (u == 2 ? 1 : 2)); k1 = u == 0 ? 0 : (u == 1 ? 1 : 2);
+  }
+}
+__device__ __forceinline__ void phase_taps4(int kind, int u, int& k0, int& k1) {
+  if (kind == 0) { k0 = u == 0 ? 2 : (u == 1 ? 1 : 0); k1 = u == 0 ? 2 : (u == 1 ? 2 : (u == 2 ? 1 : 0)); }
+  else { k0 = u == 0 ? 0 : (u == 1 ? 0 : (u == 2 ? 1 : 2)); k1 = u == 0 ? 0 : (u == 1 ? 1 : 2); }
+}
 
 struct MfmaWgradArgs {
   const bf16_t* x;
diff --git a/robust-conditional-gan_amd/csrc/conv_mfma.hip b/robust-conditional-gan_amd/csrc/conv_mfma.hip
--- a/robust-conditional-gan_amd/csrc/conv_mfma.hip
+++ b/robust-conditional-gan_amd/csrc/conv_mfma.hip
@@ -1071,17 +1071,6 @@
 }
 
 struct PhasePrepBatch { struct It { const float* w; const float* sigma; bf16_t* wph; int Cin, Cout, kind; } it[8]; };
-__device__ __forceinline__ void phase_taps2(int kind, int ph, int a, int& k0, int& k1) {
-  if (kind == 0) { k0 = ph == 0 ? (a == 0 ? 0 : 1) : (a == 0 ? 0 : 2); k1 = ph == 0 ? (a == 0 ? 0 : 2) : (a == 0 ? 1 : 2); }
-  else {
-    const int u = ph == 0 ? (a == 0 ? 3 : 1) : (a == 0 ? 2 : 0);
-    k0 = u == 0 ? 0 : (u == 1 ? 0 : (u == 2 ? 1 : 2)); k1 = u == 0 ? 0 : (u == 1 ? 1 : 2);
-  }
-}
-__device__ __forceinline__ void phase_taps4(int kind, int u, int& k0, int& k1) {
-  if (kind == 0) { k0 = u == 0 ? 2 : (u == 1 ? 1 : 0); k1 = u == 0 ? 2 : (u == 1 ? 2 : (u == 2 ? 1 : 0)); }
-  else { k0 = u == 0 ? 0 : (u == 1 ? 0 : (u == 2 ? 1 : 2)); k1 = u == 0 ? 0 : (u == 1 ? 1 : 2); }
-}
 
 __global__ __launch_bounds__(256) void conv_prepare_phase_kernel(PhasePrepBatch b) {
   const PhasePrepBatch::It it = b.it[blockIdx.y];
diff --git a/robust-conditional-gan_amd/csrc/sn.hip b/robust-conditional-gan_amd/csrc/sn.hip
--- a/robust-conditional-gan_amd/csrc/sn.hip
+++ b/robust-conditional-gan_amd/csrc/sn.hip
@@ -153,11 +153,7 @@
 
 __device__ __forceinline__ void sn_adam_elem(float g, float& m, float& v, float& w, float alpha, float omb1, float omb2, float eps, float clip,
                                              float grad_scale) {
-  const float gi = g * grad_scale;
-  m = m + (gi - m) * omb1;
-  v = v + (gi * gi - v) * omb2;
-  w = w - (m * alpha) / (sqrtf(v) + eps);
-  if (clip > 0.f) w = fminf(fmaxf(w, -clip), clip);
+  adam_tf_elem(g, m, v, w, alpha, omb1, omb2, eps, clip, grad_scale);
 }
 
 __global__ __launch_bounds__(SN_NT) void sn_bwd_p1_kernel(SnBwdBatch batch, float* hyper_inc) {
diff --git a/robust-conditional-gan_amd/ops.py b/robust-conditional-gan_amd/ops.py
--- a/robust-conditional-gan_amd/ops.py
+++ b/robust-conditional-gan_amd/ops.py
@@ -89,6 +89,11 @@
 
 
 def prepare_batch(ctx, weights_and_shapes, dtype, persistent=None, embed=None, inputs=None, frags=None):
+    todo, index = prepare_items(ctx, weights_and_shapes, dtype, persistent)
+    return _prepare_launch(ctx, todo, index, embed, inputs, frags)
+
+
+def prepare_items(ctx, weights_and_shapes, dtype, persistent=None):
     todo = []
     index = {}
     for w, k, stride, hw, *rest in weights_and_shapes:
@@ -109,6 +114,10 @@
         w._prepared[key] = buf
         index[id(w)] = len(todo)
         todo.append(L.PrepareItem(desc, w.param.ptr, w.sigma.ptr if w.sigma is not None else None, buf.ptr))
+    return todo, index
+
+
+def _prepare_launch(ctx, todo, index, embed, inputs, frags):
     fitems = [(index[id(w)], f, b, ctn, ss, w) for (w, f, b, ctn, ss) in (frags or []) if id(w) in index]
     if todo:
         arr = (L.PrepareItem * len(todo))(*todo)
diff --git a/robust-conditional-gan_amd/runtime.py b/robust-conditional-gan_amd/runtime.py
--- a/robust-conditional-gan_amd/runtime.py
+++ b/robust-conditional-gan_amd/runtime.py
@@ -125,6 +125,7 @@
         self.tape = []
         self.sn_partial = []
         self.pending_wgrads = []
+        self.wgrad_tail = None
         self.group_wgrads = os.environ.get("RCGAN_GROUP_WGRAD", "1") == "1"
         self.recording = True
         self.capturing = False
@@ -212,20 +213,29 @@
         for fn in reversed(self.tape):
             fn()
         self.tape = []
-        self.flush_wgrads()
+        self.flush_wgrads(last=True)
 
     def defer_wgrad(self, desc, x, dy, dw, dbias):
         self.pending_wgrads.append((desc, x, dy, dw, dbias))
 
-    def flush_wgrads(self):
+    def flush_wgrads(self, last=False):
         pend = self.pending_wgrads
+        tail = self.wgrad_tail if last else None
+        if last:
+            self.wgrad_tail = None
         if pend:
             self.pending_wgrads = []
             n = len(pend)
             descs = (L.ConvDesc * n)(*[p[0] for p in pend])
             arr = lambda k: (C.c_void_p * n)(*[(p[k].ptr if p[k] is not None else None) for p in pend])
             xs, dys, dws, dbs = arr(1), arr(2), arr(3), arr(4)
-            self.check(self.lib.rcgan_conv2d_bwd_weight_group(self.h, n, descs, xs, dys, dws, dbs, 1, C.c_void_p(self.ws_ptr), self.ws_bytes))
+            if tail is not None:
+                fused = C.c_int(0)
+                self.check(self.lib.rcgan_conv2d_bwd_weight_group_adam(self.h, n, descs, xs, dys, dws, dbs, 1, C.c_void_p(self.ws_ptr), self.ws_bytes,
+                                                                       C.byref(tail["opt"]), C.byref(fused)))
+                tail["fused"] = bool(fused.value)
+            else:
+                self.check(self.lib.rcgan_conv2d_bwd_weight_group(self.h, n, descs, xs, dys, dws, dbs, 1, C.c_void_p(self.ws_ptr), self.ws_bytes))
         self.check(self.lib.rcgan_head_flush(self.h))
 
     def new_step(self):
@@ -233,6 +243,7 @@
         self.tape = []
         self.sn_partial = []
         self.pending_wgrads = []
+        self.wgrad_tail = None
         self.arena.reset()
         self.epoch += 1
 
diff --git a/robust-conditional-gan_amd/variables.py b/robust-conditional-gan_amd/variables.py
--- a/robust-conditional-gan_amd/variables.py
+++ b/robust-conditional-gan_amd/variables.py
@@ -86,6 +86,10 @@
         ws = [(O.Weight(self.ctx, self.groups[self.index[pn]].param(pn), None), k, stride, hw, *rest) for pn, k, stride, hw, *rest in names]
         O.prepare_batch(self.ctx, ws, dtype, persistent=self.persist)
 
+    def persistent_items(self, names, dtype):
+        ws = [(O.Weight(self.ctx, self.groups[self.index[pn]].param(pn), None), k, stride, hw, *rest) for pn, k, stride, hw, *rest in names]
+        return O.prepare_items(self.ctx, ws, dtype, persistent=self.persist)[0]
+
     def weight(self, pname):
         if pname not in self.plain:
             w = O.Weight(self.ctx, self.param(pname), None)
```
